# leoelm/Bayesian_inference_for_NN

Measured on AMD Instinct MI355X. Metric: posterior samples/sec (grad-steps/sec) on MLP 784->200->10, batch 1024, higher is better.
Workload: dtype f32; 1 GPU; SGLD, MLP 784->200->10 (D=159010), synthetic MNIST-shaped 48000x784 fp32 resident in HBM, batch 1024 (last batch of an epoch 896), 1 chain per GPU, device-resident run replayed from hipGraphs; seed=2024, parallelism=independent chains x1 (replicas only, no data-path collective)

## Files before the change

bayesian_inference_for_nn_amd/_lib.py:

```python

from __future__ import annotations

import ctypes as C
import os

from . import _build

ACT = {"linear": 0, "relu": 1, "tanh": 2, "sigmoid": 3, "softmax": 4}
LOSS = {"scce": 0, "mse": 1, "bce": 2}
SWEEP = {"gauss_seidel": 0, "jacobi": 1}
GAMMA_MEDIAN = -1.0
MAX_LANES = 64

STREAM_SGLD, STREAM_BBB, STREAM_HMC, STREAM_INIT, STREAM_PREDICT, STREAM_VADAM, STREAM_BSAM, STREAM_CORRUPT = 0, 1, 2, 3, 4, 5, 6, 7
STREAM_PILCO = 8
STREAM_FSVI = 9
FSVI_MAX_N, FSVI_MAX_D = 1024, 2048
REWARD = {"Cart": 0, "Acb 2 factors": 1}
PILCO_KIND = {"dense": 0, "rbf": 1}


class PyzError(RuntimeError):
    def __init__(self, code, msg):
        super().__init__(f"pyz error {code}: {msg}")
        self.code = code


_p = C.c_void_p
_i32, _i64, _u32, _u64, _f = C.c_int32, C.c_int64, C.c_uint32, C.c_uint64, C.c_float

SIGNATURES = {
    "pyz_version": (C.c_int, []),
    "pyz_last_error": (C.c_char_p, []),
    "pyz_device_count": (C.c_int, []),
    "pyz_mlp_create": (C.c_int, [C.c_int, C.POINTER(_i32), C.POINTER(_i32), C.c_int, C.c_int, C.c_int, C.POINTER(_p)]),
    "pyz_mlp_destroy": (C.c_int, [_p]),
    "pyz_mlp_param_count": (_i64, [_p]),
    "pyz_mlp_workspace_bytes": (_i64, [_p]),
    "pyz_mlp_forward": (C.c_int, [_p, _p, C.c_int, _p, _p, C.c_int, _p, _p]),
    "pyz_mlp_loss_grad": (C.c_int, [_p, _p, C.c_int, _p, _p, _p, C.c_int, _p, _p, _p]),
    "pyz_sgd_step": (C.c_int, [_p, _p, _p, _p, _p, C.c_int, _f, _p, _p]),
    "pyz_swag_step": (C.c_int, [_p, _p, _p, _p, _p, _p, _p, _p, C.c_int, _f, _i64, C.c_int, _p, _p]),
    "pyz_adam_step": (C.c_int, [_p, _p, _p, _p, _p, _p, _p, C.c_int, _f, C.c_double, C.c_double, _i64, _f, _f, _p, _p]),
    "pyz_vadam_perturb": (C.c_int, [_p, _p, _p, _f, _f, _i64, _u64, _p, _p]),
    "pyz_bsam_step": (C.c_int, [_p, _p, _p, _p, _p, _p, _p, C.c_int, _f, C.c_double, C.c_double, _f, _f, _f, _f, _i64, _u64,
                              _p, _p, _p]),
    "pyz_sgld_step": (C.c_int, [_p, _p, _p, _p, _p, _p, _p, C.c_int, _f, _i64, _u64, _p, _p, _p]),
    "pyz_sgld_run": (C.c_int, [_p, _p, _p, _p, _p, _p, _p, C.POINTER(_i32), C.POINTER(_f), C.c_int, _i64, _i64, _u64,
                               _p, C.c_int, _p]),
    "pyz_sgld_chains_step": (C.c_int, [_p, _p, _p, _p, C.c_int, _p, _p, _p, C.c_int, _f, _i64, _u64, _p, _p, _p]),
    "pyz_sgld_chains_run": (C.c_int, [_p, _p, _p, _p, C.c_int, _p, _p, _p, C.POINTER(_i32), C.POINTER(_f), C.c_int, _i64,
                                      _i64, _u64, _p, C.c_int, _p]),
    "pyz_sgld_lanes_step": (C.c_int, [_p, _p, _p, _p, C.c_int, _p, _p, _p, C.c_int, C.POINTER(_f), _i64, _u64, C.c_int, _p, _p,
                                      _p]),
    "pyz_sgld_lanes_run": (C.c_int, [_p, _p, _p, _p, C.c_int, _p, _p, _p, C.POINTER(_i32), C.POINTER(_f), C.c_int, _i64,
                                     _i64, _u64, C.c_int, _p, _p]),
    "pyz_lane_scores": (C.c_int, [_p, _p, C.c_int, _p, _p, C.c_int, _p, _p, _p]),
    "pyz_sgd_run": (C.c_int, [_p, _p, _p, _p, _p, C.POINTER(_i32), C.POINTER(_f), C.c_int, _i64, _p, C.c_int, _p]),
    "pyz_swag_run": (C.c_int, [_p, _p, _p, _p, _p, C.c_int, C.c_int, _p, _p, _p, C.POINTER(_i32), C.POINTER(_f), C.c_int,
                               _i64, _i64, _p, C.c_int, _p]),
    "pyz_sgd_members_step": (C.c_int, [_p, _p, _p, C.c_int, _p, _p, _p, C.c_int, _f, _i64, C.c_int, _p, _p]),
    "pyz_sgd_members_run": (C.c_int, [_p, _p, _p, C.c_int, C.c_int, _p, _p, _p, C.POINTER(_i32), C.POINTER(_f), C.c_int, _i64,
                                      _i64, _p, C.c_int, _p]),
    "pyz_swag_members_step": (C.c_int, [_p, _p, _p, _p, _p, C.c_int, C.c_int, _p, _p, _p, C.c_int, _f, _i64, C.c_int, C.c_int,
                                        _p, _p]),
    "pyz_swag_members_run": (C.c_int, [_p, _p, _p, _p, _p, C.c_int, C.c_int, C.c_int, _p, _p, _p, C.POINTER(_i32),
                                       C.POINTER(_f), C.c_int, _i64, _i64, _p, C.c_int, _p]),
    "pyz_last_run_info": (C.c_int, [_p, C.POINTER(_i32), C.POINTER(_i32), C.POINTER(_i32)]),
    "pyz_sgld_run_info": (C.c_int, [_p, C.POINTER(_i32)]),
    "pyz_check_finite": (C.c_int, [_p, _p]),
    "pyz_probe_begin": (C.c_int, [C.c_int]),
    "pyz_probe_end": (C.c_int, [_p, C.POINTER(_f), C.c_char_p, C.c_int, C.POINTER(C.c_int)]),
    "pyz_bbb_step": (C.c_int, [_p, _p, _p, _p, _p, _p, _p, C.c_int, _f, _f, _f, _f, _p, _p, _i64, _u64, _p, _p, _p]),
    "pyz_bbb_run": (C.c_int, [_p, _p, _p, _p, _p, _p, _p, C.POINTER(_i32), C.POINTER(_f), C.c_int, _f, _f, _f, _p, _p, _i64,
                              _i64, _u64, _p, _p, _p, _p, C.c_int, _p, C.c_int, _p]),
    "pyz_adam_run": (C.c_int, [_p, _p, _p, _p, _p, _p, _p, C.POINTER(_i32), C.POINTER(_f), C.POINTER(_i64), C.c_int, C.c_double,
                               C.c_double, _f, _f, C.c_int, _f, _f, _i64, _i64, _u64, _p, C.c_int, _p]),
    "pyz_bsam_run": (C.c_int, [_p, _p, _p, _p, _p, _p, _p, C.POINTER(_i32), C.POINTER(_f), C.c_int, C.c_double, C.c_double,
                               _f, _f, _f, _f, _i64, _i64, _u64, _p, C.c_int, _p]),
    "pyz_adam_run_info": (C.c_int, [_p, C.POINTER(_i32)]),
    "pyz_hmc_step": (C.c_int, [_p, _p, C.c_int, _p, _p, C.c_int, C.c_int, _f, _f, _f, _f, _p, _p, C.c_int, C.POINTER(_f),
                               _i64, _u64, _p, _p, _p]),
    "pyz_hmc_run": (C.c_int, [_p, _p, C.c_int, _p, _p, C.c_int, C.c_int, _f, _f, _f, _f, _p, _p, C.POINTER(_f), C.c_int, C.c_int,
                              _i64, _i64, _u64, _p, _p, _p, _p, C.c_int, _p, C.c_int, _p]),
    "pyz_hmc_run_info": (C.c_int, [_p, C.POINTER(_i32)]),
    "pyz_svgd_step": (C.c_int, [_p, _p, C.c_int, _p, C.c_int, C.c_int, _p, _p, _p, _p, _p, C.c_int, _f, _f, _i64,
                                C.c_int, _p, _p]),
    "pyz_svgd_gradients": (C.c_int, [_p, _p, C.c_int, _p, _p, _p, C.c_int, _p]),
    "pyz_svgd_sweep": (C.c_int, [_p, _p, C.c_int, _p, C.c_int, C.c_int, _p, _p, _f, _f, _i64, C.c_int, _p, _p]),
    "pyz_svgd_kernel_matrix": (C.c_int, [_p, _p, C.c_int, C.c_int, C.c_int, _f, _p]),
    "pyz_svgd_gram_groups": (C.c_int, [_p, _p, C.c_int, C.c_int, C.c_int, _p, _p]),
    "pyz_svgd_kernel_matrix_groups": (C.c_int, [_p, _p, _p, C.c_int, C.c_int, C.c_int, _f, _p]),
    "pyz_svgd_combine": (C.c_int, [_p, _p, C.c_int, _p, C.c_int, C.c_int, _p, _p, _f, _f, _i64, _p, _p]),
    "pyz_fsvi_check": (C.c_int, [C.c_int, C.POINTER(_i32), C.POINTER(_i32), C.c_int, C.c_int, C.c_int, C.c_int]),
    "pyz_fsvi_step": (C.c_int, [_p, _p, _p, C.c_int, _p, _p, _p, _p, _p, C.c_int, C.c_int, _p, _p, _f, _i64, _u64, _p, _p, _p,
                                _p, _p, _p, _p, _p, _p, _p]),
    "pyz_spd_solve_f64": (C.c_int, [_p, _p, C.c_int, C.c_int, _p, _p]),
    "pyz_predict": (C.c_int, [_p, _p, C.c_int, _p, C.c_int, _p, _p, _p]),
    "pyz_predict_moments": (C.c_int, [_p, _p, C.c_int, _p, C.c_int, _p, _p, _p]),
    "pyz_grid_rows": (C.c_int, [_p, C.c_int, _f, _f, C.c_int, _f, _f, C.c_int, _i64, _i64, _p, _p]),
    "pyz_predict_surface": (C.c_int, [_p, _p, C.c_int, _p, C.c_int, C.c_int, _p, _p, _p, _p, _p, _p]),
    "pyz_input_grad": (C.c_int, [_p, _p, C.c_int, _p, _p, C.c_int, _f, _p, _f, _p, _p, _p]),
    "pyz_corrupt_rows": (C.c_int, [_p, _i64, C.c_int, C.c_int, C.c_int, C.c_int, C.POINTER(_i32), C.c_int, _f, C.c_int, _u64, _p, _p]),
    "pyz_score_rows": (C.c_int, [_p, C.c_int, _i64, C.c_int, _p, C.c_int, _p, _p]),
    "pyz_pilco_create": (C.c_int, [C.c_int, C.POINTER(_i32), C.POINTER(_i32), C.c_int, C.POINTER(_i32), C.POINTER(_i32), C.c_int,
                                   C.c_int, C.POINTER(_p)]),
    "pyz_pilco_create_layers": (C.c_int, [C.c_int, C.POINTER(_i32), C.POINTER(_i32), C.POINTER(_i32), C.POINTER(_f), C.c_int,
                                          C.POINTER(_i32), C.POINTER(_i32), C.c_int, C.c_int, C.POINTER(_p)]),
    "pyz_pilco_destroy": (C.c_int, [_p]),
    "pyz_pilco_workspace_bytes": (_i64, [_p]),
    "pyz_pilco_policy_step": (C.c_int, [_p, _p, _p, _p, _i64, _p, _p, _p, C.c_int, C.c_int, _f, C.c_int, _f, _p, _p, _p, _p,
                                        C.c_int, _p]),
    "pyz_pilco_act": (C.c_int, [_p, _p, _p, C.c_int, _p, _p]),
    "pyz_sample_normal_rows": (C.c_int, [_p, _i64, _i64, _i64, _i64, _p, _p, _u64, _u32, _u32, _p]),
    "pyz_sample_lowrank_rows": (C.c_int, [_p, _i64, _i64, _i64, _i64, _p, _p, _p, C.c_int, _f, _u64, _u32, _u32, _p]),
    "pyz_gather_rows": (C.c_int, [_p, _i64, _i64, _i64, _i64, _p, _i64, _p, _p]),
    "pyz_fill_normal": (C.c_int, [_p, _i64, _u64, _u32, _u32, _f, _f, _p]),
    "pyz_debug_stamps": (C.c_int, [C.POINTER(C.c_uint64), _i64]),
    "pyz_debug_mfma_f64_layout": (C.c_int, [C.POINTER(C.c_int32)]),
    "pyz_bench_dense_kernel": (C.c_int, [_p, C.c_int, C.c_int, _p, C.c_int, _p, _p, C.c_int, _p, C.c_int, _p]),
    "pyz_malloc": (C.c_int, [C.c_size_t, C.POINTER(_p)]),
    "pyz_free": (C.c_int, [_p]),
    "pyz_upload": (C.c_int, [_p, _p, C.c_size_t, _p]),
    "pyz_download": (C.c_int, [_p, _p, C.c_size_t, _p]),
    "pyz_sync": (C.c_int, [_p]),
    "pyz_wait_flags": (C.c_int, [_p, C.c_int, C.c_uint64, C.c_int, _p, _p]),
    "pyz_stem_create": (C.c_int, [C.c_int, C.c_int, C.c_int, C.c_int, C.POINTER(_i32), C.c_int, C.c_int, C.POINTER(_p)]),
    "pyz_stem_destroy": (C.c_int, [_p]),
    "pyz_stem_param_count": (_i64, [_p]),
    "pyz_stem_feature_count": (_i64, [_p]),
    "pyz_stem_workspace_bytes": (_i64, [_p]),
    "pyz_stem_forward": (C.c_int, [_p, _p, _i64, C.c_int, _p, _p, C.c_int, _p, _p]),
    "pyz_stem_backward": (C.c_int, [_p, _p, _i64, C.c_int, _p, _p, C.c_int, _p, _p, _i64, _p]),
    "pyz_convnet_forward": (C.c_int, [_p, _p, _p, C.c_int, _p, _p, C.c_int, _p, _p]),
    "pyz_convnet_loss_grad": (C.c_int, [_p, _p, _p, C.c_int, _p, _p, _p, C.c_int, _p, _p, _p]),
    "pyz_convnet_sgd_step": (C.c_int, [_p, _p, _p, _p, _p, _p, C.c_int, _f, _p, _p]),
    "pyz_convnet_swag_step": (C.c_int, [_p, _p, _p, _p, _p, _p, _p, _p, _p, C.c_int, _f, _i64, C.c_int, _p, _p]),
    "pyz_convnet_predict": (C.c_int, [_p, _p, _p, C.c_int, _p, C.c_int, _p, _p, _p, _p]),
}

E_NAN = -6
LOWRANK_MAX_K = 256


def header_version() -> int:
    import re
    text = open(os.path.join(os.path.dirname(os.path.abspath(__file__)), "..", "include", "pyz.h")).read()
    return int(re.search(r"#define\s+PYZ_VERSION\s+(\d+)", text).group(1))

_lib = None


# ... 42 lines not shown
```

bayesian_inference_for_nn_amd/csrc/pyz_api.hip:

```cpp

#include <algorithm>
#include <climits>
#include <cmath>
#include <cstring>
#include <vector>

#include "pyz_common.h"
#include "pyz_conv.h"
#include "pyz_corrupt.h"
#include "pyz_fsvi.h"
#include "pyz_fused.h"
#include "pyz_gemm.h"
#include "pyz_gemm_ring.h"
#include "pyz_hmc_fused.h"
#include "pyz_hmc_multi.h"
#include "pyz_input_grad.h"
#include "pyz_pilco.h"
#include "pyz_kernels.h"
#include "pyz_predict_moments.h"
#include "pyz_surface.h"
#include "pyz_rng.h"
#include "pyz_sgld_chains.h"
#include "pyz_sgld_lanes.h"
#include "pyz_members.h"
// ... 107 lines not shown
int need_grad2(pyz_mlp *m, int P) {
  return ensure_bytes((void **)&m->grad2, &full(m)->x.grad2_cap, sizeof(float) * (size_t)P * m->D + 64, m);
}
int need_qsave(pyz_mlp *m, int P) {
  return ensure_bytes((void **)&m->qsave, &full(m)->x.qsave_cap, sizeof(float) * (size_t)P * m->D + 64, m);
}
int need_part(pyz_mlp *m, size_t n_doubles) {
  return ensure_bytes((void **)&m->part, &full(m)->x.part_cap, sizeof(double) * n_doubles, m);
}
int need_part2(pyz_mlp *m, size_t n_doubles, bool keep_kernel_matrix = false) {
  if (!keep_kernel_matrix) m->km_valid = false;
  return ensure_bytes((void **)&full(m)->x.part2, &full(m)->x.part2_cap, sizeof(double) * n_doubles, m);
}

int check_call(const pyz_mlp *m, int P, int batch) {
  if (!m) return pyz_fail(PYZ_E_INVALID, "null plan");
  if (batch <= 0 || batch > m->max_batch)
    return pyz_fail(PYZ_E_SHAPE, "batch %d outside [1, %d] of the plan", batch, m->max_batch);
  if (P <= 0 || P > m->max_p)
    return pyz_fail(PYZ_E_SHAPE, "particle count %d outside [1, %d] of the plan", P, m->max_p);
  return PYZ_OK;
}

inline bool aligned16(const void *p) { return (reinterpret_cast<uintptr_t>(p) & 15u) == 0; }

int set_ctl(pyz_mlp *m, int slot, int batch, float lr, long long n, long long row_off, int i, hipStream_t st,
            int slot0 = 0, int n_run = 0) {
  m->pend_on = false;
  PYZ_LAUNCH(k_set_ctl, dim3(1), dim3(1), 0, st, m->ctl + slot, batch, lr, n, row_off, i, slot0, n_run);
  PYZ_LAUNCH_CHECK();
  return PYZ_OK;
}

void set_ctl_lazy(pyz_mlp *m, int batch, float lr, long long n) {
  m->pend = StepCtl{};
  m->pend.batch = batch;
  m->pend.lr = lr;
  m->pend.n = n;
  m->pend_on = true;
}

void flush_ctl(pyz_mlp *m, hipStream_t st) {
  if (!m->pend_on) return;
  m->pend_on = false;
  PYZ_LAUNCH(k_set_ctl, dim3(1), dim3(1), 0, st, m->ctl, m->pend.batch, m->pend.lr, m->pend.n, m->pend.row_off, m->pend.i,
                     m->pend.slot0, 0);
}

DenseArgs forward_args(pyz_mlp *m, int l, const float *theta, long long theta_ps, const float *x, const int32_t *row_idx,
                       const StepCtl *ctl, float *gather_out) {
  DenseArgs g{};
  g.K = m->dims[l];
  g.N = m->dims[l + 1];
  if (l == 0) {
    g.in = x;
    g.in_pstride = 0;
    g.row_idx = row_idx;
    g.gather_out = row_idx ? gather_out : nullptr;
  } else {
    g.in = m->act[l - 1];
    g.in_pstride = (long long)m->max_batch * g.K;
    g.row_idx = nullptr;
  }
  g.lda = g.K;
  g.theta = theta;
  g.theta_pstride = theta_ps;
  g.w_off = m->w_off[l];
  g.out = m->act[l];
  g.out_pstride = (long long)m->max_batch * g.N;
  g.act = m->acts[l];
  g.vec = (g.K % 8 == 0) && aligned16(g.in) ? 1 : 0;
  g.ctl = ctl;
  if (l == 0 && m->pend_on && ctl == m->ctl) {
    g.init = m->pend;
    g.init_on = 1;
    m->pend_on = false;
  }
  return g;
}

void launch_forward(pyz_mlp *m, const float *theta, long long theta_ps, int P, const float *x,
                    const int32_t *row_idx, int grid_batch, const StepCtl *ctl, hipStream_t st,
                    float *gather_out = nullptr, int l_end = -1, const StepCtl *gate = nullptr, int gate_mod = 0,
                    long long x_pstride = 0) {
  if (l_end < 0) l_end = m->L;
  for (int l = 0; l < l_end; ++l) {
    DenseArgs g = forward_args(m, l, theta, theta_ps, x, row_idx, ctl, gather_out);
    if (l == 0) g.in_pstride = x_pstride;
    g.wt = pyz_wt_for(P);
    g.gate = gate;
    g.gate_mod = gate_mod;
    if (pyz_launch_fwd_ring(g, grid_batch, P, st)) continue;
    if (!g.row_idx && !g.init_on && !g.gather_out) g.rows_cap = std::min(grid_batch, m->max_batch);
    pyz_launch_fwd(g, grid_batch, P, st);
  }
}

void launch_loss(pyz_mlp *m, int P, const void *y, const int32_t *row_idx, int grid_batch, const StepCtl *ctl,
                 bool want_delta, hipStream_t st) {
  LossArgs g{};
  const int C = m->dims[m->L];
  g.out_last = m->act[m->L - 1];
  g.pstride = (long long)m->max_batch * C;
  g.C = C;
  g.y = y;
  g.delta = want_delta ? m->delta[m->L - 1] : nullptr;
  g.part = m->part;
  g.nblk = cdiv(m->max_batch, 256);
  g.act_last = m->acts[m->L - 1];
  g.ctl = ctl;
  g.row_idx = row_idx;
  dim3 grid(cdiv(grid_batch, 256), P);
  if ((int)grid.x < g.nblk) g.nblk = grid.x;
  if (m->loss == PYZ_LOSS_SCCE)
    PYZ_LAUNCH(k_loss_scce, grid, dim3(256), 0, st, g);
  else
    PYZ_LAUNCH(k_loss_mse, grid, dim3(256), 0, st, g);
}

inline int loss_nblk(const pyz_mlp *m, int grid_batch) { return std::min(cdiv(m->max_batch, 256), cdiv(grid_batch, 256)); }

struct TailOf {
  long long x_pstride;
  long long grad_pstride;
  float *dfeat;
  int act_feat;
};

void launch_backward(pyz_mlp *m, const float *theta, long long theta_ps, int P, const float *x,
                     const int32_t *row_idx, int grid_batch, const StepCtl *ctl, float *grad, hipStream_t st,
                     float *grad_sq = nullptr, const TailOf *tail = nullptr) {
  for (int l = m->L - 1; l >= 0; --l) {
    const int K = m->dims[l], N = m->dims[l + 1];
    if (l > 0 || tail) {
      DenseArgs g{};
      g.K = K;
      g.N = N;
      g.in = m->delta[l];
      g.in_pstride = (long long)m->max_batch * N;
      g.lda = N;
      g.theta = theta;
      g.theta_pstride = theta_ps;
      g.w_off = m->w_off[l];
      g.out = l > 0 ? m->delta[l - 1] : tail->dfeat;
      g.out_pstride = l > 0 ? (long long)m->max_batch * K : tail->x_pstride;
      g.aux = l > 0 ? m->act[l - 1] : x;
      g.aux_pstride = g.out_pstride;
      g.act = l > 0 ? m->acts[l - 1] : tail->act_feat;
      g.vec = (N % 8 == 0) && (m->w_off[l] % 4 == 0) && (P == 1 || theta_ps % 4 == 0) && aligned16(theta) ? 1 : 0;
      g.ctl = ctl;
      pyz_launch_bwd_data(g, grid_batch, P, st);
    }
    DenseArgs g{};
    g.K = K;
    g.N = N;
    if (l == 0) {
      g.in = x;
      g.in_pstride = tail ? tail->x_pstride : 0;
      g.row_idx = row_idx;
    } else {
      g.in = m->act[l - 1];
      g.in_pstride = (long long)m->max_batch * K;
    }
    g.lda = K;
    g.aux = m->delta[l];
    g.aux_pstride = (long long)m->max_batch * N;
    g.out = grad;
    g.out_pstride = tail ? tail->grad_pstride : m->D;
    g.w_off = m->w_off[l];
// ... 93 lines not shown
                            const StepCtl *ctl, hipStream_t st) {
  for (int l = m->L - 2; l >= 1; --l) {
    const int K = m->dims[l], N = m->dims[l + 1];
    DenseArgs g{};
    g.K = K;
    g.N = N;
    g.in = m->delta[l];
    g.in_pstride = (long long)m->max_batch * N;
    g.lda = N;
    g.theta = theta;
    g.theta_pstride = theta_ps;
    g.w_off = m->w_off[l];
    g.out = m->delta[l - 1];
    g.out_pstride = (long long)m->max_batch * K;
    g.aux = m->act[l - 1];
    g.aux_pstride = (long long)m->max_batch * K;
    g.act = m->acts[l - 1];
    g.vec = (N % 8 == 0) && (m->w_off[l] % 4 == 0) && (P == 1 || theta_ps % 4 == 0) && aligned16(theta) ? 1 : 0;
    g.ctl = ctl;
    pyz_launch_bwd_data(g, grid_batch, P, st);
  }
}

inline int wgrad_tiles(const pyz_mlp *m) {
  int tiles = 0;
  for (int l = 0; l < m->L; ++l) tiles += ((m->dims[l] + 1 + 31) / 32) * ((m->dims[l + 1] + 31) / 32);
  return tiles;
}

int wgrad_layers(pyz_mlp *m, int P, const float *x, const int32_t *row_idx, const StepCtl *ctl, WgradArgs &a,
                 const float *gathered) {
  int tiles = 0;
  a.L = m->L;
  for (int l = 0; l < m->L; ++l) {
    WgradLayer &ly = a.lay[l];
    ly.K = m->dims[l];
    ly.N = m->dims[l + 1];
    if (l == 0) {
      ly.in = (row_idx && gathered) ? gathered : x;
      ly.in_pstride = 0;
      ly.gather = (row_idx && !gathered) ? 1 : 0;
    } else {
      ly.in = m->act[l - 1];
      ly.in_pstride = (long long)m->max_batch * ly.K;
      ly.gather = 0;
    }
    ly.lda = ly.K;
    ly.delta = m->delta[l];
    ly.delta_pstride = (long long)m->max_batch * ly.N;
    ly.w_off = m->w_off[l];
    ly.tile0 = tiles;
    a.tile0[l] = tiles;
    tiles += ((ly.K + 1 + 31) / 32) * ((ly.N + 31) / 32);
  }
  for (int l = m->L; l < PYZ_MAX_LAYERS; ++l) a.tile0[l] = INT_MAX;
  a.row_idx = row_idx;
  a.ctl = ctl;
  a.part = m->part;
  a.nblk = m->cur_nblk;
  a.tiles = tiles;
  a.nonfinite = m->nonfinite;
  a.wt = pyz_wt_for(P);
  return tiles;
}

void launch_wgrad_all(pyz_mlp *m, int P, const float *x, const int32_t *row_idx, int grid_batch, const StepCtl *ctl,
                      WgradArgs &a, hipStream_t st, const float *gathered) {
  const int tiles = wgrad_layers(m, P, x, row_idx, ctl, a, gathered);
  const int S = pyz_pick_waves((long long)tiles * P, (grid_batch + 1) / 2);
  dim3 grid(pyz_pad8((long long)tiles + 1, P), P);
  if (a.prep.src && P == 1) grid.x = (unsigned)(tiles + 1 + std::max(pyz_cu_count() - tiles - 1, 24));
  switch (S) {
    case 1:
      if (a.mode == PYZ_UPD_NONE) PYZ_LAUNCH((k_wgrad_all<1, true>), grid, dim3(64), 0, st, a);
      else PYZ_LAUNCH(k_wgrad_all<1>, grid, dim3(64), 0, st, a);
      break;
    case 2: PYZ_LAUNCH(k_wgrad_all<2>, grid, dim3(128), 2 * 4096, st, a); break;
    case 4: PYZ_LAUNCH(k_wgrad_all<4>, grid, dim3(256), 4 * 4096, st, a); break;
    case 8: PYZ_LAUNCH(k_wgrad_all<8>, grid, dim3(512), 8 * 4096, st, a); break;
    default: PYZ_LAUNCH(k_wgrad_all<16>, grid, dim3(1024), 16 * 4096, st, a); break;
  }
}

void launch_wgrad_adam(pyz_mlp *m, const float *x, const int32_t *row_idx, int grid_batch, const StepCtl *ctl, AdamArgs &a,
                       hipStream_t st, const float *gathered) {
  const int tiles = wgrad_layers(m, 1, x, row_idx, ctl, a.w, gathered);
  const int S = pyz_pick_waves(tiles, (grid_batch + 1) / 2);
  const dim3 grid(tiles + 1);
  switch (S) {
    case 1: PYZ_LAUNCH(k_wgrad_adam<1>, grid, dim3(64), 0, st, a); break;
    case 2: PYZ_LAUNCH(k_wgrad_adam<2>, grid, dim3(128), 2 * 4096, st, a); break;
    case 4: PYZ_LAUNCH(k_wgrad_adam<4>, grid, dim3(256), 4 * 4096, st, a); break;
    case 8: PYZ_LAUNCH(k_wgrad_adam<8>, grid, dim3(512), 8 * 4096, st, a); break;
    default: PYZ_LAUNCH(k_wgrad_adam<16>, grid, dim3(1024), 16 * 4096, st, a); break;
  }
}

void launch_wgrad_bsam(pyz_mlp *m, const float *x, const int32_t *row_idx, int grid_batch, const StepCtl *ctl, int phase,
                       BsamArgs &a, hipStream_t st, const float *gathered) {
  const int tiles = wgrad_layers(m, 1, x, row_idx, ctl, a.w, gathered);
  const int S = pyz_pick_waves(tiles, (grid_batch + 1) / 2);
  const dim3 grid(tiles + 1);
#define PYZ_BSAM_CASE(W, LDS)                                                           \
  if (phase == 0) PYZ_LAUNCH((k_wgrad_bsam<W, 0>), grid, dim3(64 * W), LDS, st, a);     \
  else PYZ_LAUNCH((k_wgrad_bsam<W, 1>), grid, dim3(64 * W), LDS, st, a);                \
  break
  switch (S) {
    case 1: PYZ_BSAM_CASE(1, 0);
    case 2: PYZ_BSAM_CASE(2, 2 * 4096);
    case 4: PYZ_BSAM_CASE(4, 4 * 4096);
    case 8: PYZ_BSAM_CASE(8, 8 * 4096);
    default: PYZ_BSAM_CASE(16, 16 * 4096);
  }
#undef PYZ_BSAM_CASE
}

inline float *batch_buf(pyz_mlp *m, int slot) { return m->xb + (size_t)slot * m->max_batch * m->dims[0]; }

inline bool batch_ahead(const pyz_mlp *m, const int32_t *row_idx) {
  static const int on = pyz_env_int("PYZ_BATCH_AHEAD", 1);
  if (!on || !can_fuse(m) || m->L <= 1 || row_idx == nullptr) return false;
  return on == 2 || wgrad_tiles(m) + 24 <= pyz_cu_count();
}

PrepArgs prep_args(pyz_mlp *m, const float *x, const int32_t *row_idx, int grid_batch, long long row_stride, int dst_slot) {
  PrepArgs p{};
  p.src = x;
  p.dst = batch_buf(m, dst_slot);
  p.row_idx = row_idx;
  p.tab_bs = m->tab_bs;
  p.row_stride = row_stride;
  p.K = p.lda = m->dims[0];
  p.fwd_tiles_n = (m->dims[1] + 31) / 32;
  p.fwd_tiles = ((grid_batch + 31) / 32) * p.fwd_tiles_n;
  return p;
}

int ksplit_for(pyz_mlp *m, const float *theta, long long theta_ps, int P, const float *xc, int grid_batch, const StepCtl *ctl) {
  const int ks_env = pyz_env_int("PYZ_FWD_KSPLIT", 0);
  if (ks_env < 2 || ks_env > 8 || m->L != 2 || P != 1) return 0;
  const int UT = m->dims[1] <= 64 ? 1 : m->dims[1] <= 256 ? 4 : 0, NPc = m->dims[2];
  if (!UT || NPc > 16 || !pyz_env_int("PYZ_HEAD_ROWS", 1)) return 0;
  DenseArgs g = forward_args(m, 0, theta, theta_ps, xc, nullptr, ctl, nullptr);
  if (!pyz_fwd_ring_ksplit_ok(g, grid_batch, P)) return 0;
  if ((long long)((grid_batch + 31) / 32) * ks_env > 2 * pyz_cu_count()) return 0;
  const size_t need = sizeof(float) * (size_t)ks_env * m->max_batch * m->dims[1];
  if (!full(m)->x.fwd_part || full(m)->x.fwd_part_cap < need) return 0;
  return ks_env;
}

void launch_loss_backward(pyz_mlp *m, const float *theta, long long theta_ps, int P, const float *x, const void *y,
                          const int32_t *row_idx, int grid_batch, const StepCtl *ctl, bool want_grad, WgradArgs &upd,
                          hipStream_t st, int ahead_slot = -1, AdamArgs *adam = nullptr) {
  if (can_fuse(m)) {
    if (ahead_slot >= 0) {
      const float *xc = batch_buf(m, ahead_slot);
      const int ks = ksplit_for(m, theta, theta_ps, P, xc, grid_batch, ctl);
      if (ks > 1) {
        DenseArgs g = forward_args(m, 0, theta, theta_ps, xc, nullptr, ctl, nullptr);
        g.wt = pyz_wt_for(P);
        g.k_split = ks;
        g.part_out = static_cast<float *>(full(m)->x.fwd_part);
        g.part_stride = (long long)m->max_batch * g.N;
        pyz_launch_fwd_ring_ksplit(g, grid_batch, st);
      } else {
        launch_forward(m, theta, theta_ps, P, xc, nullptr, grid_batch, ctl, st, nullptr, m->L - 1);
      }
      launch_head(m, theta, theta_ps, P, x, y, row_idx, grid_batch, ctl, want_grad, st, nullptr, 0, ks);
      launch_bwd_data_hidden(m, theta, theta_ps, P, grid_batch, ctl, st);
      launch_wgrad_all(m, P, x, row_idx, grid_batch, ctl, upd, st, xc);
      return;
    }
    static const int use_xb = pyz_env_int("PYZ_GATHER_COPY", 1);
    float *xb = (use_xb && want_grad && row_idx && m->L > 1) ? m->xb : nullptr;
    launch_forward(m, theta, theta_ps, P, x, row_idx, grid_batch, ctl, st, xb, m->L - 1);
    launch_head(m, theta, theta_ps, P, x, y, row_idx, grid_batch, ctl, want_grad, st);
    if (want_grad) {
      launch_bwd_data_hidden(m, theta, theta_ps, P, grid_batch, ctl, st);
      if (adam) launch_wgrad_adam(m, x, row_idx, grid_batch, ctl, *adam, st, xb);
      else launch_wgrad_all(m, P, x, row_idx, grid_batch, ctl, upd, st, xb);
    }
    return;
  }
  flush_ctl(m, st);
  launch_forward(m, theta, theta_ps, P, x, row_idx, grid_batch, ctl, st);
  launch_loss(m, P, y, row_idx, grid_batch, ctl, want_grad, st);
  m->cur_nblk = loss_nblk(m, grid_batch);
  if (want_grad) launch_backward(m, theta, theta_ps, P, x, row_idx, grid_batch, ctl, upd.grad, st, adam ? m->grad2 : nullptr);
}

void launch_bsam_pass(pyz_mlp *m, const float *theta, const float *x, const void *y, const int32_t *row_idx, int grid_batch,
                      int phase, BsamArgs &a, hipStream_t st) {
  static const int use_xb = pyz_env_int("PYZ_GATHER_COPY", 1);
  float *xb = (use_xb && row_idx && m->L > 1) ? m->xb : nullptr;
  launch_forward(m, theta, m->D, 1, x, row_idx, grid_batch, m->ctl, st, xb, m->L - 1);
  launch_head(m, theta, m->D, 1, x, y, row_idx, grid_batch, m->ctl, true, st);
  launch_bwd_data_hidden(m, theta, m->D, 1, grid_batch, m->ctl, st);
  launch_wgrad_bsam(m, x, row_idx, grid_batch, m->ctl, phase, a, st, xb);
}

int check_loss_combo(const pyz_mlp *m) {
  const int last = m->acts[m->L - 1];
  if (m->loss == PYZ_LOSS_SCCE && last != PYZ_ACT_SOFTMAX)
    return pyz_fail(PYZ_E_INVALID, "SparseCategoricalCrossentropy needs a softmax last layer");
  if (m->loss == PYZ_LOSS_MSE && last == PYZ_ACT_SOFTMAX)
    return pyz_fail(PYZ_E_INVALID, "MeanSquaredError on a softmax last layer is not supported");
  if (m->loss == PYZ_LOSS_BCE && (m->dims[m->L] != 1 || last != PYZ_ACT_SIGMOID))
    return pyz_fail(PYZ_E_INVALID, "BinaryCrossentropy needs a last layer of exactly one sigmoid unit");
  return PYZ_OK;
}

AdamScal adam_scalars(float lr, double beta_1, double beta_2, long long epoch, float denom_eps, float decay) {
  AdamScal a;
  a.lr = lr;
  a.b1 = (float)beta_1;
  a.c1 = (float)(1.0 - beta_1);
  a.b2 = (float)beta_2;
  a.c2 = (float)(1.0 - beta_2);
  a.bc1 = (float)(1.0 - std::pow(beta_1, (double)epoch));
  a.bc2 = (float)(1.0 - std::pow(beta_2, (double)epoch));
  a.eps = denom_eps;
  a.decay = decay;
  return a;
}

void launch_delta0(pyz_mlp *m, const float *theta, int P, const float *x, const void *y, int n, hipStream_t st) {
  if (can_fuse(m)) {
    launch_forward(m, theta, m->D, P, x, nullptr, n, m->ctl, st, nullptr, m->L - 1);
    launch_head(m, theta, m->D, P, x, y, nullptr, n, m->ctl, true, st);
    launch_bwd_data_hidden(m, theta, m->D, P, n, m->ctl, st);
    return;
  }
  launch_forward(m, theta, m->D, P, x, nullptr, n, m->ctl, st);
  launch_loss(m, P, y, nullptr, n, m->ctl, true, st);
  m->cur_nblk = loss_nblk(m, n);
  if (m->L > 1) {
    const int l = m->L - 1, K = m->dims[l], N = m->dims[l + 1];
// ... 251 lines not shown
  return for_draw_chunks(net, d_weights, n_samples, d_x, n, m->max_p, st, [&](int s0, int S, const float *) {
    g.S = S;
    g.accumulate = s0 > 0 ? 1 : 0;
    if (!pyz_launch_predict_moments(g, st))
      return pyz_fail(PYZ_E_SHAPE, "a row of %d outputs does not fit the moments kernel's LDS", g.C);
    return PYZ_OK;
  });
}

}

extern "C" {

int pyz_version(void) { return PYZ_VERSION; }

const char *pyz_last_error(void) { return pyz_err_slot().c_str(); }

int pyz_device_count(void) {
  int n = 0;
  if (hipGetDeviceCount(&n) != hipSuccess) return 0;
  return n;
}

int pyz_mlp_create(int n_layers, const int32_t *h_dims, const int32_t *h_acts, int loss, int max_batch,
                   int max_particles, pyz_mlp **out) {
  if (!out || !h_dims || !h_acts) return pyz_fail(PYZ_E_INVALID, "null argument");
  *out = nullptr;
  if (n_layers < 1 || n_layers > PYZ_MAX_LAYERS) return pyz_fail(PYZ_E_INVALID, "n_layers %d outside [1, %d]", n_layers, PYZ_MAX_LAYERS);
  if (max_batch < 1 || max_particles < 1) return pyz_fail(PYZ_E_INVALID, "max_batch and max_particles must be >= 1");
  if (max_particles > 65535) return pyz_fail(PYZ_E_INVALID, "max_particles %d > 65535", max_particles);
  if (loss != PYZ_LOSS_SCCE && loss != PYZ_LOSS_MSE && loss != PYZ_LOSS_BCE) return pyz_fail(PYZ_E_INVALID, "unknown loss %d", loss);
  int ndev = 0;
  if (hipGetDeviceCount(&ndev) != hipSuccess || ndev < 1) return pyz_fail(PYZ_E_NODEV, "no HIP device visible");
  pyz_mlp_full *m = new pyz_mlp_full();
  m->L = n_layers;
  m->loss = loss;
  m->max_batch = max_batch;
  m->max_p = max_particles;
  long long off = 0;
  for (int l = 0; l <= n_layers; ++l) {
    if (h_dims[l] < 1) {
      delete m;
      return pyz_fail(PYZ_E_INVALID, "dims[%d] = %d", l, h_dims[l]);
    }
    m->dims[l] = h_dims[l];
  }
  for (int l = 0; l < n_layers; ++l) {
    const int a = h_acts[l];
    if (a < PYZ_ACT_LINEAR || a > PYZ_ACT_SOFTMAX || (a == PYZ_ACT_SOFTMAX && l != n_layers - 1)) {
      delete m;
      return pyz_fail(PYZ_E_INVALID, "activation %d at layer %d is not supported", a, l);
    }
    m->acts[l] = a;
    m->w_off[l] = off;
    off += (long long)(m->dims[l] + 1) * m->dims[l + 1];
  }
  m->D = off;
  if (loss == PYZ_LOSS_BCE) {
    const int rc = check_loss_combo(m);
    if (rc != PYZ_OK) {
      delete m;
      return rc;
    }
  }
  {
    long long widest = 0;
    for (int l = 0; l <= n_layers; ++l) widest = std::max<long long>(widest, m->dims[l]);
    if ((long long)max_batch * widest * 4 >= (1LL << 31) || off * 4 >= (1LL << 31)) {
      delete m;
      return pyz_fail(PYZ_E_INVALID, "max_batch x widest layer, or the parameter vector, exceeds 2 GiB");
    }
  }
  auto fail = [&](int rc) {
    pyz_mlp_destroy(m);
    return rc;
  };
  for (int l = 0; l < n_layers; ++l) {
    const size_t bytes = sizeof(float) * (size_t)max_particles * max_batch * m->dims[l + 1] + 64;
    if (hipMalloc((void **)&m->act[l], bytes) != hipSuccess || hipMalloc((void **)&m->delta[l], bytes) != hipSuccess)
      return fail(pyz_fail(PYZ_E_OOM, "workspace allocation of %zu bytes failed", bytes));
    m->ws_bytes += 2 * bytes;
  }
  {
    const size_t bytes = 2 * sizeof(float) * (size_t)max_batch * m->dims[0] + 64;
    if (hipMalloc((void **)&m->xb, bytes) != hipSuccess) return fail(pyz_fail(PYZ_E_OOM, "workspace allocation of %zu bytes failed", bytes));
    m->ws_bytes += bytes;
  }
  if (hipMalloc((void **)&m->nonfinite, 64) != hipSuccess || hipMemset(m->nonfinite, 0, 64) != hipSuccess)
    return fail(pyz_fail(PYZ_E_OOM, "counter allocation failed"));
  if (hipMalloc((void **)&m->ctl, 2 * sizeof(StepCtl)) != hipSuccess) return fail(pyz_fail(PYZ_E_OOM, "ctl allocation failed"));
  if (hipMemset(m->ctl, 0, 2 * sizeof(StepCtl)) != hipSuccess) return fail(pyz_fail(PYZ_E_HIP, "ctl memset failed"));
  const size_t scal = sizeof(float) * (size_t)(max_particles * 16 + 64);
  if (hipMalloc((void **)&m->scal, scal) != hipSuccess) return fail(pyz_fail(PYZ_E_OOM, "scalar allocation failed"));
  m->ws_bytes += scal;
  {
    const int rc = need_part(m, (size_t)max_particles * max_batch + 8);
    if (rc != PYZ_OK) return fail(rc);
  }
  if (m->L == 2 && m->dims[1] > 192 && m->dims[1] <= 200 && pyz_env_int("PYZ_FWD_KSPLIT", 0) >= 2) {
    const int rc = ensure_bytes(&m->x.fwd_part, &m->x.fwd_part_cap, sizeof(float) * (size_t)8 * max_batch * m->dims[1], m);
    if (rc != PYZ_OK) return fail(rc);
  }
  {
    const int gs_lds = (int)pyz_svgd_gs_lds_bytes();
    if (hipFuncSetAttribute(reinterpret_cast<const void *>(k_svgd_gs<false>), hipFuncAttributeMaxDynamicSharedMemorySize, gs_lds) != hipSuccess ||
        hipFuncSetAttribute(reinterpret_cast<const void *>(k_svgd_gs<true>), hipFuncAttributeMaxDynamicSharedMemorySize, gs_lds) != hipSuccess)
      return fail(pyz_fail(PYZ_E_HIP, "hipFuncSetAttribute(k_svgd_gs) failed"));
    if (hipFuncSetAttribute(reinterpret_cast<const void *>(k_svgd_gs_resident), hipFuncAttributeMaxDynamicSharedMemorySize,
                            (int)pyz_svgd_gs_res_lds_bytes()) != hipSuccess)
      return fail(pyz_fail(PYZ_E_HIP, "hipFuncSetAttribute(k_svgd_gs_resident) failed"));
    if (hipFuncSetAttribute(reinterpret_cast<const void *>(k_svgd_gs_resident2), hipFuncAttributeMaxDynamicSharedMemorySize,
                            (int)pyz_svgd_gs_res_lds_bytes()) != hipSuccess)
      return fail(pyz_fail(PYZ_E_HIP, "hipFuncSetAttribute(k_svgd_gs_resident2) failed"));
    const int gr_lds = (int)pyz_svgd_gram_lds_bytes();
    if (hipFuncSetAttribute(reinterpret_cast<const void *>(k_svgd_gram_tile<1, false>), hipFuncAttributeMaxDynamicSharedMemorySize, gr_lds) != hipSuccess ||
        hipFuncSetAttribute(reinterpret_cast<const void *>(k_svgd_gram_tile<2, false>), hipFuncAttributeMaxDynamicSharedMemorySize, gr_lds) != hipSuccess ||
        hipFuncSetAttribute(reinterpret_cast<const void *>(k_svgd_gram_tile<4, true>), hipFuncAttributeMaxDynamicSharedMemorySize, gr_lds) != hipSuccess)
      return fail(pyz_fail(PYZ_E_HIP, "hipFuncSetAttribute(k_svgd_gram_tile) failed"));
  }
  *out = m;
  return PYZ_OK;
}

int pyz_mlp_destroy(pyz_mlp *mm) {
  if (!mm) return PYZ_OK;
  pyz_mlp_full *m = full(mm);
  m->graphs.drop();
  m->x.hm_graphs.drop();
  m->x.hmc_run_graphs.drop();
  m->x.adam_graphs.drop();
  for (int l = 0; l < PYZ_MAX_LAYERS; ++l) {
    if (m->act[l]) (void)hipFree(m->act[l]);
    if (m->delta[l]) (void)hipFree(m->delta[l]);
  }
  void *ptrs[] = {m->grad, m->grad2, m->qsave, m->part, m->x.part2, m->scal, m->ctl, m->tab_bs, m->xb, m->x.hm_buf, m->x.hm_res_buf, m->x.gs_res_buf, m->x.fwd_part, m->nonfinite, m->x.hr_buf, m->x.hr_tab, m->x.tab_bc, m->x.fsvi_buf};
  for (void *p : ptrs)
    if (p) (void)hipFree(p);
  if (m->x.tab_host) {
    (void)hipHostFree(m->x.tab_host);
    for (auto &e : m->x.tab_ev) (void)hipEventDestroy(e);
  }
  if (m->x.up_host) {
    (void)hipHostFree(m->x.up_host);
    for (auto &e : m->x.up_ev) (void)hipEventDestroy(e);
  }
  if (m->x.hr_host) {
    (void)hipHostFree(m->x.hr_host);
    for (auto &e : m->x.hr_ev) (void)hipEventDestroy(e);
  }
  if (m->h_pinned) (void)hipHostFree(m->h_pinned);
  delete m;
  return PYZ_OK;
}

int64_t pyz_mlp_param_count(const pyz_mlp *m) { return m ? m->D : -1; }
int64_t pyz_mlp_workspace_bytes(const pyz_mlp *m) { return m ? (int64_t)m->ws_bytes : -1; }

int pyz_mlp_forward(pyz_mlp *m, const float *d_theta, int P, const float *d_x, const int32_t *d_row_idx, int batch,
                    float *d_out, void *stream) {
  int rc = check_call(m, P, batch);
  if (rc) return rc;
  return net_forward(Net{nullptr, m}, d_theta, P, d_x, d_row_idx, batch, d_out, stream);
}

int pyz_mlp_loss_grad(pyz_mlp *m, const float *d_theta, int P, const float *d_x, const void *d_y,
                      const int32_t *d_row_idx, int batch, float *d_grad, float *d_loss, void *stream) {
  int rc = check_call(m, P, batch);
// ... 333 lines not shown
  } else {
    u.mode = PYZ_UPD_NONE;
    u.grad = m->grad;
    u.grad_pstride = m->D;
  }
  launch_loss_backward(m, d_theta, m->D, 1, d_x, d_y, d_row_idx, batch, m->ctl, true, u, st);
  if (!fused)
    PYZ_LAUNCH(k_swag_update, dim3(cdiv(m->D, 256)), dim3(256), 0, st, d_theta, d_mean, d_sq_mean, d_dev_row,
                       m->grad, m->D, update_moments ? 1 : 0, m->ctl, m->part, m->cur_nblk, d_loss, m->nonfinite);
  PYZ_LAUNCH_CHECK();
  return PYZ_OK;
}

struct SwagChain {
  float *dev;
  int k, freq;
};

struct BbbChain {
  float *rho, *w;
  float *w2;
  float alpha, prior_mean, prior_rho;
  const float *pm_vec, *pr_vec;
  pyz_mlp *val;
  const float *val_x;
  const void *val_y;
  int n_val;
  float *val_losses;
};

static int ensure_run_tables(pyz_mlp *m, size_t n_tab, size_t host_entry_bytes, hipStream_t st) {
  pyz_mlp_full *f = full(m);
  if (m->tab_cap < (int)n_tab) {
    const size_t cap = std::max<size_t>(n_tab, 65536);
    if (m->tab_bs) PYZ_HIP(hipFree(m->tab_bs));
    m->tab_bs = nullptr;
    m->tab_lr = nullptr;
    PYZ_HIP(hipMalloc((void **)&m->tab_bs, 8 * cap));
    m->tab_lr = reinterpret_cast<float *>(m->tab_bs + cap);
    m->tab_cap = (int)cap;
    m->graphs.drop();
  }
  if (f->x.tab_host_cap < host_entry_bytes * n_tab) {
    if (f->x.tab_host) {
      PYZ_HIP(hipStreamSynchronize(st));
      PYZ_HIP(hipHostFree(f->x.tab_host));
      f->x.tab_host = nullptr;
    } else {
      for (auto &e : f->x.tab_ev) PYZ_HIP(hipEventCreateWithFlags(&e, hipEventDisableTiming));
    }
    const size_t cap = std::max<size_t>(host_entry_bytes * n_tab, host_entry_bytes * 4096);
    PYZ_HIP(hipHostMalloc(&f->x.tab_host, 2 * cap));
    f->x.tab_host_cap = cap;
    f->x.tab_count = 0;
  }
  return PYZ_OK;
}

static int check_run(const pyz_mlp *m, int n_steps, int64_t slot0, const int32_t *h_batch_sizes, const int64_t *h_epochs = nullptr) {
  if (n_steps <= 0) return pyz_fail(PYZ_E_INVALID, "n_steps must be positive");
  if (slot0 < 0 || slot0 + n_steps > 0x7fffffff) return pyz_fail(PYZ_E_INVALID, "slot0 out of range");
  int bmax = 0;
  for (int s = 0; h_batch_sizes && s < n_steps; ++s) {
    if (h_batch_sizes[s] <= 0 || h_batch_sizes[s] > m->max_batch)
      return pyz_fail(PYZ_E_SHAPE, "batch size %d of step %d outside [1, %d]", h_batch_sizes[s], s, m->max_batch);
    if (h_epochs && h_epochs[s] < 1) return pyz_fail(PYZ_E_INVALID, "epoch %lld of step %d < 1", (long long)h_epochs[s], s);
    bmax = std::max(bmax, h_batch_sizes[s]);
  }
  return bmax;
}

struct RunBc {
  double beta_1, beta_2;
  const int64_t *h_epochs;
  float2 of(int s) const {
    const AdamScal a = adam_scalars(0.0f, beta_1, beta_2, h_epochs[s], 0.0f, 0.0f);
    return make_float2(a.bc1, a.bc2);
  }
};

static int upload_run_tables(pyz_mlp *m, const int32_t *h_batch_sizes, const float *h_lr, int n_steps, int64_t n0, int64_t slot0,
                             const RunBc *bc, const float *d_x, const int32_t *d_row_idx, int ahead_batch, hipStream_t st) {
  Extra &x = full(m)->x;
  int rc;
  const size_t n_tab = (size_t)n_steps + 1;
  if ((rc = ensure_run_tables(m, n_tab, bc ? 16 : 8, st))) return rc;
  if (bc && x.tab_bc_cap < m->tab_cap) {
    if (x.tab_bc) PYZ_HIP(hipFree(x.tab_bc));
    x.tab_bc = nullptr;
    x.tab_bc_cap = 0;
    PYZ_HIP(hipMalloc((void **)&x.tab_bc, sizeof(float2) * (size_t)m->tab_cap));
    x.tab_bc_cap = m->tab_cap;
  }
  const long long row_stride = m->max_batch;
  m->pend_on = false;
  if (n_steps <= PYZ_INLINE_TAB) {
    InlineTabs tabs{};
    InlineBc ibc{};
    for (int s = 0; s < n_steps; ++s) {
      tabs.bs[s] = h_batch_sizes[s];
      tabs.lr[s] = h_lr[s];
    }
    tabs.bs[n_steps] = h_batch_sizes[n_steps - 1];
    tabs.lr[n_steps] = h_lr[n_steps - 1];
    tabs.n = n_steps + 1;
    for (int s = 0; bc && s <= n_steps; ++s) ibc.bc[s] = bc->of(std::min(s, n_steps - 1));
    if (ahead_batch) {
      const PrepArgs pa = prep_args(m, d_x, d_row_idx, ahead_batch, row_stride, 0);
      if (bc) PYZ_LAUNCH(k_run_start_bc, dim3(256), dim3(256), 0, st, m->ctl, tabs, ibc, m->tab_bs, m->tab_lr, x.tab_bc, (long long)n0, slot0 * row_stride, (int)slot0, pa);
      else PYZ_LAUNCH(k_run_start, dim3(256), dim3(256), 0, st, m->ctl, tabs, m->tab_bs, m->tab_lr, (long long)n0, slot0 * row_stride, (int)slot0, pa);
    } else {
      if (bc) PYZ_LAUNCH(k_set_ctl_tabs_bc, dim3(1), dim3(64), 0, st, m->ctl, tabs, ibc, m->tab_bs, m->tab_lr, x.tab_bc, (long long)n0, slot0 * row_stride, (int)slot0);
      else PYZ_LAUNCH(k_set_ctl_tabs, dim3(1), dim3(64), 0, st, m->ctl, tabs, m->tab_bs, m->tab_lr, (long long)n0, slot0 * row_stride, (int)slot0);
    }
    return PYZ_OK;
  }
  const unsigned slot = (unsigned)(x.tab_count & 1);
  if (x.tab_count >= 2) PYZ_HIP(hipEventSynchronize(x.tab_ev[slot]));
  ++x.tab_count;
  int32_t *hb = reinterpret_cast<int32_t *>(static_cast<unsigned char *>(x.tab_host) + slot * x.tab_host_cap);
  float *hl = reinterpret_cast<float *>(hb + n_tab);
  float2 *hc = reinterpret_cast<float2 *>(hl + n_tab);
  std::memcpy(hb, h_batch_sizes, sizeof(int32_t) * n_steps);
  std::memcpy(hl, h_lr, sizeof(float) * n_steps);
  hb[n_steps] = h_batch_sizes[n_steps - 1];
  hl[n_steps] = h_lr[n_steps - 1];
  for (int s = 0; bc && s <= n_steps; ++s) hc[s] = bc->of(std::min(s, n_steps - 1));
  PYZ_HIP(hipMemcpyAsync(m->tab_bs, hb, sizeof(int32_t) * n_tab, hipMemcpyHostToDevice, st));
  PYZ_HIP(hipMemcpyAsync(m->tab_lr, hl, sizeof(float) * n_tab, hipMemcpyHostToDevice, st));
  if (bc) PYZ_HIP(hipMemcpyAsync(x.tab_bc, hc, sizeof(float2) * n_tab, hipMemcpyHostToDevice, st));
  PYZ_HIP(hipEventRecord(x.tab_ev[slot], st));
  if ((rc = set_ctl(m, 0, h_batch_sizes[0], h_lr[0], n0, slot0 * row_stride, 0, st, (int)slot0, n_steps))) return rc;
  if (ahead_batch)
    PYZ_LAUNCH(k_prep_batch, dim3(256), dim3(256), 0, st, prep_args(m, d_x, d_row_idx, ahead_batch, row_stride, 0), m->ctl);
  return PYZ_OK;
}

static void launch_sgld_step(pyz_mlp *m, float *theta, float *mean, float *sq, const float *x, const void *y,
                             const int32_t *row_idx, int grid_batch, int slot, bool chained, long long row_stride,
                             uint64_t seed, const float *unit_noise, float *loss, hipStream_t st, int mode = PYZ_UPD_SGLD,
                             const SwagChain *swag = nullptr, const BbbChain *bbb = nullptr, bool first = true) {
  const StepCtl *ctl = m->ctl + slot;
  if (bbb) {
    const int nblk_sample = cdiv(cdiv(m->D, 4), 256), tiles = wgrad_tiles(m);
    const bool fuse = bbb->w2 != nullptr;
    const size_t kl_stride = (size_t)std::max(nblk_sample, tiles);
    double *kl_cur = full(m)->x.part2 + (fuse ? (size_t)slot * kl_stride : 0);
    double *kl_next = full(m)->x.part2 + (size_t)(slot ^ 1) * kl_stride;
    float *w_cur = (fuse && slot) ? bbb->w2 : bbb->w, *w_next = slot ? bbb->w : bbb->w2;
    const bool sample = !fuse || first;
    if (sample) {
      BbbArgs a{};
      a.mu = theta;
      a.rho = bbb->rho;
      a.w = w_cur;
      a.D = m->D;
      a.alpha = bbb->alpha;
      a.prior_mean = bbb->prior_mean;
      a.prior_rho = bbb->prior_rho;
      a.pm_vec = bbb->pm_vec;
      a.pr_vec = bbb->pr_vec;
      a.seed = seed;
      a.part_kl = kl_cur;
      a.nblk_kl = nblk_sample;
      a.ctl = ctl;
      a.chained = 1;
      PYZ_LAUNCH(k_bbb_sample, dim3(nblk_sample), dim3(256), 0, st, a);
    }
    WgradArgs u{};
    u.mode = PYZ_UPD_BBB;
    u.theta = theta;
    u.mean = bbb->rho;
    u.sq_mean = w_cur;
    u.seed = seed;
    u.alpha = bbb->alpha;
    u.prior_mean = bbb->prior_mean;
    u.prior_rho = bbb->prior_rho;
    u.pm_vec = bbb->pm_vec;
    u.pr_vec = bbb->pr_vec;
    u.bbb_chained = 1;
    u.part_kl = kl_cur;
    u.nblk_kl = sample ? nblk_sample : tiles;
    if (fuse) {
      u.w_next = w_next;
      u.part_kl_next = kl_next;
    }
    u.cost = loss;
    u.next = chained ? m->ctl + (slot ^ 1) : nullptr;
    u.tab_bs = m->tab_bs;
    u.tab_lr = m->tab_lr;
    u.row_stride = row_stride;
    const bool ahead = chained && batch_ahead(m, row_idx);
    if (ahead) u.prep = prep_args(m, x, row_idx, grid_batch, row_stride, slot ^ 1);
    launch_loss_backward(m, w_cur, m->D, 1, x, y, row_idx, grid_batch, ctl, true, u, st, ahead ? slot : -1);
    if (bbb->val) {
      pyz_mlp *v = bbb->val;
      launch_forward(v, w_cur, v->D, 1, bbb->val_x, nullptr, bbb->n_val, v->ctl, st, nullptr, v->L - 1, ctl, 10);
      launch_head(v, w_cur, v->D, 1, bbb->val_x, bbb->val_y, nullptr, bbb->n_val, v->ctl, false, st, ctl, 10);
      PYZ_LAUNCH(k_loss_finalize_gated, dim3(1), dim3(64), 0, st, v->part, v->cur_nblk, v->ctl, bbb->val_losses, v->nonfinite, ctl, 10);
    }
    return;
  }
  if (can_fuse(m)) {
    WgradArgs u{};
    u.mode = mode;
    if (swag) {
      u.swag_freq = swag->freq;
      u.swag_k = swag->k;
      u.dev_base = swag->dev;
      u.dev_stride = m->D;
    }
    u.theta = theta;
    u.mean = mean;
    u.sq_mean = sq;
    u.seed = seed;
    u.unit_noise = unit_noise;
    u.loss = loss;
    u.loss_indexed = chained ? 1 : 0;
    u.next = chained ? m->ctl + (slot ^ 1) : nullptr;
    u.tab_bs = m->tab_bs;
    u.tab_lr = m->tab_lr;
    u.row_stride = row_stride;
    const bool ahead = chained && batch_ahead(m, row_idx);
    if (ahead) u.prep = prep_args(m, x, row_idx, grid_batch, row_stride, slot ^ 1);
    launch_loss_backward(m, theta, m->D, 1, x, y, row_idx, grid_batch, ctl, true, u, st, ahead ? slot : -1);
    return;
  }
  WgradArgs u{};
  u.mode = PYZ_UPD_NONE;
  u.grad = m->grad;
  u.grad_pstride = m->D;
  launch_loss_backward(m, theta, m->D, 1, x, y, row_idx, grid_batch, ctl, true, u, st);
  SgldArgs a{};
  a.theta = theta;
  a.mean = mean;
  a.sq_mean = sq;
  a.grad = m->grad;
  a.D = m->D;
  a.ctl = ctl;
  a.next = chained ? m->ctl + (slot ^ 1) : nullptr;
  a.tab_bs = m->tab_bs;
  a.tab_lr = m->tab_lr;
  a.row_stride = row_stride;
  a.seed = seed;
  a.unit_noise = unit_noise;
  a.part = m->part;
  a.nblk = m->cur_nblk;
  a.loss = loss;
  a.loss_indexed = chained ? 1 : 0;
  a.nonfinite = m->nonfinite;
  PYZ_LAUNCH(k_sgld_update, dim3(cdiv(cdiv(m->D, 4), 256)), dim3(256), 0, st, a);
}

int pyz_sgld_step(pyz_mlp *m, float *d_theta, float *d_mean, float *d_sq_mean, const float *d_x, const void *d_y,
                  const int32_t *d_row_idx, int batch, float lr, int64_t n, uint64_t seed, const float *d_unit_noise,
                  float *d_loss, void *stream) {
  int rc = check_call(m, 1, batch);
  if (rc) return rc;
  if ((rc = check_loss_combo(m))) return rc;
  if (!d_theta || !d_mean || !d_sq_mean || !d_x || !d_y || !d_loss) return pyz_fail(PYZ_E_INVALID, "null device pointer");
  if (n < 0) return pyz_fail(PYZ_E_INVALID, "negative step count");
  if (!can_fuse(m) && (rc = need_grad(m, 1))) return rc;
  hipStream_t st = as_stream(stream);
  set_ctl_lazy(m, batch, lr, n);
  launch_sgld_step(m, d_theta, d_mean, d_sq_mean, d_x, d_y, d_row_idx, batch, 0, false, 0, seed, d_unit_noise, d_loss, st);
  PYZ_LAUNCH_CHECK();
  return PYZ_OK;
}

static int sgld_run_impl(pyz_mlp *m, float *d_theta, float *d_mean, float *d_sq_mean, const float *d_x, const void *d_y,
                         const int32_t *d_row_idx, const int32_t *h_batch_sizes, const float *h_lr, int n_steps,
                         int64_t n0, int64_t slot0, uint64_t seed, float *d_losses, int use_graph, void *stream,
                         int mode = PYZ_UPD_SGLD, const SwagChain *swag = nullptr, const BbbChain *bbb = nullptr) {
  if (!m) return pyz_fail(PYZ_E_INVALID, "null plan");
  if (mode != PYZ_UPD_SGLD && !can_fuse(m))
    return pyz_fail(PYZ_E_INVALID, "the chained SGD / SWAG runs need a last layer of at most 32 units");
  if (mode == PYZ_UPD_SGD) d_mean = d_sq_mean = d_theta;
  int rc = check_loss_combo(m);
  if (rc) return rc;
  if ((rc = check_run(m, n_steps, slot0, nullptr)) < 0) return rc;
  if (!d_theta || !d_mean || !d_sq_mean || !d_x || !d_y || !d_row_idx || !h_batch_sizes || !h_lr || !d_losses)
    return pyz_fail(PYZ_E_INVALID, "null pointer");
  const int bmax = check_run(m, n_steps, slot0, h_batch_sizes);
  if (bmax < 0) return bmax;
  if (!can_fuse(m) && (rc = need_grad(m, 1))) return rc;
  hipStream_t st = as_stream(stream);
  BbbChain bbb_local{};
  if (bbb) {
    static const int fuse_sample = pyz_env_int("PYZ_BBB_FUSE_SAMPLE", 1);
    if ((rc = need_part2(m, 2 * (size_t)std::max(cdiv(cdiv(m->D, 4), 256), wgrad_tiles(m))))) return rc;
    if (fuse_sample) {
      if ((rc = need_grad(m, 1))) return rc;
      bbb_local = *bbb;
      bbb_local.w2 = m->grad;
      bbb = &bbb_local;
    }
    if (bbb->val) {
      pyz_mlp *v = bbb->val;
      if (v->D != m->D || !can_fuse(v) || bbb->n_val < 1 || bbb->n_val > v->max_batch || !bbb->val_x || !bbb->val_y || !bbb->val_losses)
        return pyz_fail(PYZ_E_INVALID, "validation plan / split does not fit the model");
      if ((rc = set_ctl(v, 0, bbb->n_val, 0.0f, 0, 0, 0, st))) return rc;
    }
  }
  const long long row_stride = m->max_batch;
  if ((rc = upload_run_tables(m, h_batch_sizes, h_lr, n_steps, n0, slot0, nullptr, d_x, d_row_idx,
                              batch_ahead(m, d_row_idx) ? bmax : 0, st)))
    return rc;

  int s = 0;
  m->run_graph_steps = m->run_eager_steps = m->run_graph_launches = 0;
  m->graphs.begin_call();
  static const int G = std::min(128, std::max(2, pyz_env_int("PYZ_GRAPH_STEPS", 32) & ~1));
  if (use_graph && st != nullptr && !pyz_probe().on) {
    unsigned long long key = 1469598103934665603ull;
    auto mix = [&](unsigned long long v) { key = (key ^ v) * 1099511628211ull; };
    mix((unsigned long long)(uintptr_t)d_theta); mix((unsigned long long)(uintptr_t)d_mean);
    mix((unsigned long long)(uintptr_t)d_sq_mean); mix((unsigned long long)(uintptr_t)d_x);
    mix((unsigned long long)(uintptr_t)d_y); mix((unsigned long long)(uintptr_t)d_row_idx);
    mix((unsigned long long)(uintptr_t)d_losses); mix(seed); mix((unsigned long long)bmax);
    mix((unsigned long long)(uintptr_t)m->tab_bs); mix((unsigned long long)G); mix((unsigned long long)mode);
    if (swag) { mix((unsigned long long)(uintptr_t)swag->dev); mix((unsigned long long)swag->k); mix((unsigned long long)swag->freq); }
    if (bbb) {
      unsigned fb[3];
      memcpy(&fb[0], &bbb->alpha, 4); memcpy(&fb[1], &bbb->prior_mean, 4); memcpy(&fb[2], &bbb->prior_rho, 4);
      for (unsigned b : fb) mix(b);
      mix((unsigned long long)(uintptr_t)bbb->pm_vec); mix((unsigned long long)(uintptr_t)bbb->pr_vec);
      mix((unsigned long long)(uintptr_t)bbb->val); mix((unsigned long long)(uintptr_t)bbb->val_x); mix((unsigned long long)(uintptr_t)bbb->val_y);
      mix((unsigned long long)bbb->n_val); mix((unsigned long long)(uintptr_t)bbb->val_losses);
      mix((unsigned long long)(uintptr_t)bbb->w2); mix((unsigned long long)(uintptr_t)bbb->rho); mix((unsigned long long)(uintptr_t)full(m)->x.part2);
    }
    m->graphs.rekey(key);
    while (s < n_steps) {
      const int len = std::min(G, n_steps - s);
      const bool rest = len < G;
      rc = m->graphs.launch(len, 0, rest ? 1 : 0, rest ? PYZ_GRAPH_CHUNKS : 1, st, [&] {
        for (int k = 0; k < len; ++k)
          launch_sgld_step(m, d_theta, d_mean, d_sq_mean, d_x, d_y, d_row_idx, bmax, k & 1, true, row_stride, seed,
                           nullptr, d_losses, st, mode, swag, bbb, k == 0);
        return PYZ_OK;
      });
      if (rc) return rc;
      s += len;
      m->run_graph_steps += len;
      ++m->run_graph_launches;
    }
  }
  for (; s < n_steps; ++s) {
    launch_sgld_step(m, d_theta, d_mean, d_sq_mean, d_x, d_y, d_row_idx, bmax, s & 1, true, row_stride, seed, nullptr,
                     d_losses, st, mode, swag, bbb, s == 0);
    ++m->run_eager_steps;
  }
  if (bbb && bbb->w2 && ((n_steps - 1) & 1))
    PYZ_HIP(hipMemcpyAsync(bbb->w, bbb->w2, sizeof(float) * (size_t)m->D, hipMemcpyDeviceToDevice, st));
  PYZ_LAUNCH_CHECK();
  return PYZ_OK;
}

int pyz_sgld_run(pyz_mlp *m, float *d_theta, float *d_mean, float *d_sq_mean, const float *d_x, const void *d_y,
                 const int32_t *d_row_idx, const int32_t *h_batch_sizes, const float *h_lr, int n_steps, int64_t n0,
                 int64_t slot0, uint64_t seed, float *d_losses, int use_graph, void *stream) {
  return sgld_run_impl(m, d_theta, d_mean, d_sq_mean, d_x, d_y, d_row_idx, h_batch_sizes, h_lr, n_steps, n0, slot0, seed,
                       d_losses, use_graph, stream);
}

static int sgld_rows_check(const pyz_mlp *m, bool lanes, const void *theta, const void *mean, const void *sq, int P,
                           const void *x, const void *y, const void *h_lr, const void *losses, int64_t n, int seed_stride,
                           const char *row = nullptr) {
  if (!row) row = lanes ? "lane" : "chain";
  if (P < 1) return pyz_fail(PYZ_E_INVALID, "n_%ss %d: at least one %s", row, P, row);
  if (n < 0) return pyz_fail(PYZ_E_INVALID, "negative step count");
  if (lanes && seed_stride != 0 && seed_stride != 1)
    return pyz_fail(PYZ_E_INVALID, "seed_stride %d: 0 (one noise stream for every lane) or 1 (seed + lane)", seed_stride);
  if (!theta || !mean || !sq || !x || !y || (lanes && !h_lr) || !losses)
    return pyz_fail(PYZ_E_INVALID, lanes ? "null pointer" : "null device pointer");
  if (!m) return pyz_fail(PYZ_E_INVALID, "null plan");
  const int most = lanes ? std::min(m->max_p, PYZ_MAX_LANES) : m->max_p;
  if (P > most)
    return pyz_fail(PYZ_E_SHAPE, "n_%ss %d outside [1, %d] of the plan%s", row, P, most, lanes ? " and the library" : "");
  return check_loss_combo(m);
}

static dim3 sgld_rows_grid(long long groups, int P) {
  const long long per_row = std::max<long long>(1, 8LL * pyz_cu_count() / P);
  return dim3((unsigned)std::min<long long>(cdiv(groups, 256), per_row), (unsigned)P);
}

struct MembersUpdate {
  bool swag;
  float *dev;
  int k;
  int freq;
  int hit, col;
};

static void launch_sgld_rows_step(pyz_mlp *m, float *theta, float *mean, float *sq, int P, const float *x, const void *y,
                                  const int32_t *row_idx, int grid_batch, int slot, bool chained, long long row_stride,
                                  uint64_t seed, const float *lane_lr, int seed_stride, const float *unit_noise, float *loss,
                                  hipStream_t st, const MembersUpdate *members = nullptr) {
  const StepCtl *ctl = m->ctl + slot;
  WgradArgs u{};
  u.mode = PYZ_UPD_NONE;
  u.grad = m->grad;
  u.grad_pstride = m->D;
// ... 1789 lines not shown
    g.out = m->delta[layer - 1];
    g.out_pstride = (long long)m->max_batch * K;
    g.aux = m->act[layer - 1];
    g.aux_pstride = (long long)m->max_batch * K;
    g.act = m->acts[layer - 1];
    g.vec = (N % 8 == 0) && (m->w_off[layer] % 4 == 0) && (P == 1 || m->D % 4 == 0) && aligned16(d_theta) ? 1 : 0;
  } else if (kind == 0) {
    if (layer == 0) {
      g.in = d_x;
      g.in_pstride = 0;
      g.row_idx = d_row_idx;
    } else {
      g.in = m->act[layer - 1];
      g.in_pstride = (long long)m->max_batch * K;
    }
    g.lda = K;
    g.out = m->act[layer];
    g.out_pstride = (long long)m->max_batch * N;
    g.act = m->acts[layer];
    g.vec = (K % 8 == 0) && aligned16(g.in) ? 1 : 0;
  }
  WgradArgs u{};
  u.mode = PYZ_UPD_NONE;
  u.grad = d_grad;
  u.grad_pstride = m->D;
  for (int i = 0; i < iters; ++i) {
    if (kind == 0) {
      if (!pyz_launch_fwd_ring(g, batch, P, st)) pyz_launch_fwd(g, batch, P, st);
    }
    else if (kind == 1) pyz_launch_bwd_data(g, batch, P, st);
    else launch_wgrad_all(m, P, d_x, d_row_idx, batch, m->ctl, u, st, nullptr);
  }
  PYZ_LAUNCH_CHECK();
  return PYZ_OK;
}

int pyz_probe_begin(int max_launches) {
  if (max_launches < 1 || max_launches > (1 << 20)) return pyz_fail(PYZ_E_INVALID, "max_launches outside [1, 2^20]");
  PyzProbe &p = pyz_probe();
  if (p.on) return pyz_fail(PYZ_E_INVALID, "a probe is already open on this thread");
  while ((int)p.ev.size() < 2 * max_launches) {
    hipEvent_t e = nullptr;
    PYZ_HIP(hipEventCreate(&e));
    p.ev.push_back(e);
  }
  p.name.assign((size_t)max_launches, nullptr);
  p.cap = max_launches;
  p.n = 0;
  p.on = true;
  return PYZ_OK;
}

int pyz_probe_end(void *stream, float *h_us, char *h_names, int name_stride, int *h_n) {
  PyzProbe &p = pyz_probe();
  if (!p.on) return pyz_fail(PYZ_E_INVALID, "no probe open on this thread");
  p.on = false;
  if (!h_us || !h_n) return pyz_fail(PYZ_E_INVALID, "null pointer");
  PYZ_HIP(hipStreamSynchronize(as_stream(stream)));
  for (int i = 0; i < p.n; ++i) {
    float ms = 0.0f;
    PYZ_HIP(hipEventElapsedTime(&ms, p.ev[2 * i], p.ev[2 * i + 1]));
    h_us[i] = ms * 1e3f;
    if (h_names && name_stride > 1) {
      const char *nm = p.name[i] ? p.name[i] : "";
      const bool wrapped = nm[0] == '(';
      char *dst = h_names + (size_t)i * name_stride;
      std::snprintf(dst, (size_t)name_stride, "%s", nm + (wrapped ? 1 : 0));
      const size_t len = std::strlen(dst);
      if (wrapped && len > 0 && dst[len - 1] == ')') dst[len - 1] = '\0';
    }
  }
  *h_n = p.n;
  return PYZ_OK;
}

int pyz_last_run_info(const pyz_mlp *m, int32_t *h_graph_steps, int32_t *h_eager_steps, int32_t *h_graph_launches) {
  if (!m) return pyz_fail(PYZ_E_INVALID, "null plan");
  if (h_graph_steps) *h_graph_steps = m->run_graph_steps;
  if (h_eager_steps) *h_eager_steps = m->run_eager_steps;
  if (h_graph_launches) *h_graph_launches = m->run_graph_launches;
  return PYZ_OK;
}

int pyz_sgld_run_info(const pyz_mlp *m, int32_t *h_captures) {
  if (!m) return pyz_fail(PYZ_E_INVALID, "null plan");
  if (h_captures) *h_captures = m->graphs.captures;
  return PYZ_OK;
}

int pyz_check_finite(pyz_mlp *m, void *stream) {
  if (!m) return pyz_fail(PYZ_E_INVALID, "null plan");
  hipStream_t st = as_stream(stream);
  int n = 0;
  PYZ_HIP(hipMemcpyAsync(&n, m->nonfinite, sizeof n, hipMemcpyDeviceToHost, st));
  PYZ_HIP(hipMemsetAsync(m->nonfinite, 0, sizeof n, st));
  PYZ_HIP(hipStreamSynchronize(st));
  if (n > 0) return pyz_fail(PYZ_E_NAN, "%d step(s) since the last check produced a NaN / Inf loss", n);
  return PYZ_OK;
}

int pyz_malloc(size_t bytes, void **d_out) {
  if (!d_out || bytes == 0) return pyz_fail(PYZ_E_INVALID, "bad allocation request");
  *d_out = nullptr;
  PYZ_HIP(hipMalloc(d_out, bytes));
  return PYZ_OK;
}

int pyz_free(void *d_ptr) {
  if (d_ptr) PYZ_HIP(hipFree(d_ptr));
  return PYZ_OK;
}

int pyz_upload(void *d_dst, const void *h_src, size_t bytes, void *stream) {
  if (!d_dst || !h_src) return pyz_fail(PYZ_E_INVALID, "null pointer");
  PYZ_HIP(hipMemcpyAsync(d_dst, h_src, bytes, hipMemcpyHostToDevice, as_stream(stream)));
  PYZ_HIP(hipStreamSynchronize(as_stream(stream)));
  return PYZ_OK;
}

int pyz_download(void *h_dst, const void *d_src, size_t bytes, void *stream) {
  if (!h_dst || !d_src) return pyz_fail(PYZ_E_INVALID, "null pointer");
  PYZ_HIP(hipMemcpyAsync(h_dst, d_src, bytes, hipMemcpyDeviceToHost, as_stream(stream)));
  PYZ_HIP(hipStreamSynchronize(as_stream(stream)));
  return PYZ_OK;
}

int pyz_wait_flags(const uint64_t *d_flags, int n, uint64_t value, int spin_limit, int *d_fail, void *stream) {
  if (!d_flags) return pyz_fail(PYZ_E_INVALID, "null device pointer");
  if (n < 1 || n > 64) return pyz_fail(PYZ_E_INVALID, "flag count %d outside [1, 64]", n);
  PYZ_LAUNCH(k_wait_flags, dim3(1), dim3(64), 0, as_stream(stream), reinterpret_cast<const unsigned long long *>(d_flags), n,
             (unsigned long long)value, spin_limit, d_fail);
  PYZ_LAUNCH_CHECK();
  return PYZ_OK;
}

int pyz_sync(void *stream) {
  PYZ_HIP(hipStreamSynchronize(as_stream(stream)));
  return PYZ_OK;
}

int pyz_debug_mfma_f64_layout(int32_t *h_out512) {
  if (!h_out512) return pyz_fail(PYZ_E_INVALID, "null pointer");
  int *d = nullptr;
  PYZ_HIP(hipMalloc((void **)&d, 512 * sizeof(int)));
  PYZ_LAUNCH(k_probe_mfma_f64, dim3(1), dim3(64), 0, nullptr, d);
  const hipError_t e = hipMemcpy(h_out512, d, 512 * sizeof(int), hipMemcpyDeviceToHost);
  (void)hipFree(d);
  PYZ_HIP(e);
  return PYZ_OK;
}

int pyz_debug_stamps(uint64_t *h_out, int64_t n_words) {
#ifdef PYZ_STAMPS
  const int64_t total = (int64_t)PYZ_STAMP_KERNELS * PYZ_STAMP_BLOCKS * PYZ_STAMP_WAVES * PYZ_STAMP_SLOTS * 2;
  if (!h_out || n_words < total) return pyz_fail(PYZ_E_INVALID, "need %lld words", (long long)total);
  PYZ_HIP(hipDeviceSynchronize());
  PYZ_HIP(hipMemcpyFromSymbol(h_out, HIP_SYMBOL(pyz_dbg_buf), sizeof(unsigned long long) * total));
  return PYZ_OK;
#else
  (void)h_out;
  (void)n_words;
  return pyz_fail(PYZ_E_INVALID, "not a PYZ_STAMPS build");
#endif
}

int pyz_stem_destroy(pyz_stem *s) {
// ... 217 lines not shown
```

bayesian_inference_for_nn_amd/csrc/pyz_common.h:

```cpp
#pragma once

#include <hip/hip_runtime.h>
#include <hip/hip_ext.h>

#include <cstdarg>
#include <cstdint>
#include <cstdio>
#include <string>
#include <vector>

#include "../../include/pyz.h"

#define PYZ_MAX_LAYERS 16

typedef float f32x16 __attribute__((ext_vector_type(16)));
typedef float f32x4 __attribute__((ext_vector_type(4)));

struct StepCtl {
  int32_t batch;
  float lr;
  long long n;
  long long row_off;
  int32_t i;
  int32_t slot0;
// ... 53 lines not shown
  long long n = raw.n, ro = raw.row_off;
  asm volatile("; step scalars" : "+v"(b), "+v"(lr), "+v"(n), "+v"(ro));
  PyzCtlHot c;
  c.batch = __builtin_amdgcn_readfirstlane(b);
  c.lr = __builtin_bit_cast(float, __builtin_amdgcn_readfirstlane(__builtin_bit_cast(int, lr)));
  const unsigned nl = __builtin_amdgcn_readfirstlane((int)(unsigned)n), nh = __builtin_amdgcn_readfirstlane((int)(n >> 32));
  const unsigned rl = __builtin_amdgcn_readfirstlane((int)(unsigned)ro), rh = __builtin_amdgcn_readfirstlane((int)(ro >> 32));
  c.n = (long long)(((unsigned long long)nh << 32) | nl);
  c.row_off = (long long)(((unsigned long long)rh << 32) | rl);
  return c;
}

__device__ __forceinline__ StepCtl pyz_ctl_first(const StepCtl *ctl, const StepCtl &init, const int on) {
  if (on && blockIdx.x == 0 && blockIdx.y == 0 && threadIdx.x == 0) *const_cast<StepCtl *>(ctl) = init;
  int ib = init.batch, ii = init.i, is0 = init.slot0, inr = init.n_run;
  float il = init.lr;
  long long in_ = init.n, iro = init.row_off;
  asm volatile("" : "+s"(ib), "+s"(ii), "+s"(is0), "+s"(il), "+s"(in_), "+s"(iro), "+s"(inr));
  StepCtl c;
  c.batch = on ? ib : ctl->batch;
  c.lr = on ? il : ctl->lr;
  c.n = on ? in_ : ctl->n;
  c.row_off = on ? iro : ctl->row_off;
  c.i = on ? ii : ctl->i;
  c.slot0 = on ? is0 : ctl->slot0;
  c.n_run = on ? inr : ctl->n_run;
  return c;
}

__device__ __forceinline__ void pyz_st(float *p, const float v, const int wt) {
  if (wt)
    asm volatile("global_store_dword %0, %1, off sc1" ::"v"(p), "v"(v) : "memory");
  else
    *p = v;
}

inline std::string &pyz_err_slot() {
  static thread_local std::string s;
  return s;
}

inline int pyz_fail(int code, const char *fmt, ...) {
  char buf[512];
  va_list ap;
  va_start(ap, fmt);
  vsnprintf(buf, sizeof buf, fmt, ap);
  va_end(ap);
  pyz_err_slot() = buf;
  return code;
}

#define PYZ_HIP(call)                                                                        \
  do {                                                                                       \
    hipError_t e_ = (call);                                                                  \
    if (e_ != hipSuccess)                                                                    \
      return pyz_fail(e_ == hipErrorOutOfMemory ? PYZ_E_OOM : PYZ_E_HIP, "%s failed: %s (%s:%d)", \
                      #call, hipGetErrorString(e_), __FILE__, __LINE__);                     \
  } while (0)

#define PYZ_LAUNCH_CHECK()                                                                    \
  do {                                                                                        \
    hipError_t e_ = hipGetLastError();                                                        \
    if (e_ != hipSuccess)                                                                     \
      return pyz_fail(PYZ_E_HIP, "kernel launch failed: %s (%s:%d)", hipGetErrorString(e_),   \
                      __FILE__, __LINE__);                                                    \
  } while (0)

struct PyzProbe {
  std::vector<hipEvent_t> ev;
  std::vector<const char *> name;
  int n = 0, cap = 0;
  bool on = false;
};
inline PyzProbe &pyz_probe() {
  static thread_local PyzProbe p;
  return p;
}
#define PYZ_LAUNCH(kern, grid, block, lds, st, ...)                                                              \
  do {                                                                                                           \
    PyzProbe &pp_ = pyz_probe();                                                                                 \
    if (pp_.on && pp_.n < pp_.cap) {                                                                             \
      hipExtLaunchKernelGGL(kern, grid, block, lds, st, pp_.ev[2 * pp_.n], pp_.ev[2 * pp_.n + 1], 0, __VA_ARGS__); \
      pp_.name[pp_.n++] = #kern;                                                                                 \
    } else {                                                                                                     \
      hipLaunchKernelGGL(kern, grid, block, lds, st, __VA_ARGS__);                                               \
    }                                                                                                            \
  } while (0)

template <int N>
struct PyzGraphCache {
  hipGraph_t graph[N] = {};
  hipGraphExec_t exec[N] = {};
  int len[N] = {};
  unsigned long long sig[N] = {}, use[N] = {};
  unsigned long long clock = 0, key = 0;
  unsigned long long call_clock = 0;
  int captures = 0;

  void drop_slot(int c) {
    if (exec[c]) (void)hipGraphExecDestroy(exec[c]);
    if (graph[c]) (void)hipGraphDestroy(graph[c]);
    exec[c] = nullptr;
    graph[c] = nullptr;
    len[c] = 0;
  }
  void drop() {
    for (int c = 0; c < N; ++c) drop_slot(c);
  }
  void rekey(unsigned long long k) {
    if (key != k) {
      drop();
      key = k;
    }
  }
  void begin_call() {
    captures = 0;
    call_clock = clock;
  }
  template <class Steps>
  int launch(int n, unsigned long long s, int lo, int hi, hipStream_t st, Steps &&steps) {
    int ci = -1, free_slot = -1, lru = -1;
    for (int c = lo; c < hi; ++c) {
      if (!exec[c]) {
        if (free_slot < 0) free_slot = c;
        continue;
      }
      if (len[c] == n && sig[c] == s) ci = c;
      if (lru < 0 || use[c] < use[lru]) lru = c;
    }
    if (ci < 0) {
      ci = free_slot >= 0 ? free_slot : lru;
      if (exec[ci] && use[ci] > call_clock) PYZ_HIP(hipStreamSynchronize(st));
      drop_slot(ci);
      PYZ_HIP(hipStreamBeginCapture(st, hipStreamCaptureModeRelaxed));
      const int rc = steps();
      hipGraph_t gr = nullptr;
      const hipError_t ce = hipStreamEndCapture(st, &gr);
      if (rc || ce != hipSuccess) {
        if (gr) (void)hipGraphDestroy(gr);
        return rc ? rc : pyz_fail(PYZ_E_HIP, "hipStreamEndCapture failed: %s", hipGetErrorString(ce));
      }
      graph[ci] = gr;
      PYZ_HIP(hipGraphInstantiate(&exec[ci], gr, nullptr, nullptr, 0));
      len[ci] = n;
      sig[ci] = s;
      ++captures;
    }
    use[ci] = ++clock;
    PYZ_HIP(hipGraphLaunch(exec[ci], st));
    return PYZ_OK;
  }
};

#define PYZ_GRAPH_CHUNKS 8
struct pyz_mlp {
  int L = 0;
  int dims[PYZ_MAX_LAYERS + 1] = {0};
  int acts[PYZ_MAX_LAYERS] = {0};
  long long w_off[PYZ_MAX_LAYERS] = {0};
  int loss = 0;
  int max_batch = 0, max_p = 0;
  long long D = 0;
  size_t ws_bytes = 0;
  float *act[PYZ_MAX_LAYERS] = {nullptr};
  float *delta[PYZ_MAX_LAYERS] = {nullptr};
  float *xb = nullptr;
  float *grad = nullptr;
  float *grad2 = nullptr;
  float *qsave = nullptr;
  double *part = nullptr;
  int part_len = 0;
  int cur_nblk = 0;
  float *scal = nullptr;
  StepCtl *ctl = nullptr;
  StepCtl pend{};
  bool pend_on = false;
  int32_t *tab_bs = nullptr;
  float *tab_lr = nullptr;
  int tab_cap = 0;
  float *h_pinned = nullptr;
  PyzGraphCache<PYZ_GRAPH_CHUNKS> graphs;
  int run_graph_steps = 0, run_eager_steps = 0, run_graph_launches = 0;
  int *nonfinite = nullptr;
  int grad_owner = 0;
  int grad_rows = 0;
  bool km_valid = false;
  const float *km_all = nullptr;
  int km_total = 0, km_row0 = 0, km_local = 0;
  float km_gamma = 0.0f;
};
```

bayesian_inference_for_nn_amd/csrc/pyz_fused.h:

```cpp
#pragma once

#include <type_traits>

#include "pyz_common.h"
#include "pyz_gemm.h"
#include "pyz_kernels.h"

struct HeadArgs {
  const float *hin;
  long long hin_pstride;
  const float *theta;
  long long theta_pstride;
  long long w_off;
  const StepCtl *ctl;
  const int32_t *row_idx;
  const StepCtl *gate;
  const void *y;
  double *part;
  int lda;
  int K, N;
  int loss;
  int gather_hin;
  int gate_mod;
  int init_on;
// ... 383 lines not shown
        d2[c] = c < N ? sc * e * pyz_act_grad(o, act) : 0.0f;
        outv[c] = o;
      }
      lm = a / (float)N;
    }
#pragma unroll
    for (int c = 0; c < NP; ++c) {
      my_d = (l == c) ? d2[c] : my_d;
      my_o = (l == c) ? outv[c] : my_o;
    }
  }
  PYZ_STAMP(1, 3);
  if (l < N) {
    if (g.out_last) pyz_st(g.out_last + p * g.last_pstride + (long long)m * N + l, my_o, g.wt);
    if (g.delta_last) pyz_st(g.delta_last + p * g.last_pstride + (long long)m * N + l, my_d, g.wt);
  }
  if (l == 0) g.part[p * g.nblk + m] = (double)lm;
  PYZ_STAMP(1, 4);
  if (!g.delta_prev) return;
  float *op = g.delta_prev + p * g.prev_pstride + (long long)m * K;
  const int actp = g.act_prev;
#pragma unroll
  for (int t = 0; t < UT; ++t) {
    const int u = l + 64 * t;
    float a = 0.0f;
#pragma unroll
    for (int c = 0; c < NP; ++c) a = fmaf(d2[c], wv[t][c], a);
    if (u < K) pyz_st(op + u, a * pyz_act_grad(hv[t], actp), g.wt);
  }
  PYZ_STAMP(1, 5);
}

template <int UT, int NP, int RW = 1, bool HP = false>
__global__ void __launch_bounds__(256) k_head_rows(HeadArgs g) {
  PYZ_STAMP(1, 0);
  const int w = pyz_wave_id(), l = threadIdx.x & 63;
  asm volatile("; arguments in one trip" ::"s"(g.hin), "s"(g.hin_pstride), "s"(g.theta), "s"(g.theta_pstride), "s"(g.w_off),
               "s"(g.ctl), "s"(g.row_idx), "s"(g.gate), "s"(g.y), "s"(g.part), "s"(g.lda), "s"(g.K), "s"(g.N), "s"(g.loss),
               "s"(g.gather_hin), "s"(g.gate_mod), "s"(g.init_on), "s"(g.nblk), "s"(g.act_last), "s"(g.act_prev), "s"(g.vec),
               "s"(g.wt));
  if (g.gate && g.gate->n % g.gate_mod == 0) return;
  StepCtl ctl;
  if (g.init_on) {
    asm volatile("; the step scalars by value" ::: "memory");
    ctl = pyz_ctl_first(g.ctl, g.init, 1);
  } else {
    const PyzCtlHot c = pyz_ctl_arrived(pyz_ctl_request(g.ctl));
    ctl.batch = c.batch;
    ctl.row_off = c.row_off;
  }
  const int batch = ctl.batch, p = blockIdx.y;
  const int m0 = (blockIdx.x * 4 + w) * RW;
  if (m0 >= batch) {
    if (l < RW && m0 + l < g.nblk) g.part[p * g.nblk + m0 + l] = 0.0;
    return;
  }
  PyzHeadW<UT, NP> W;
  if (RW == 1) {
    pyz_head_row<UT, NP, false, HP>(g, batch, ctl.row_off, p, m0, l, W);
    return;
  }
  pyz_head_load_w<UT, NP>(g, p, l, W);
#pragma unroll 1
  for (int rr = 0; rr < RW; ++rr) {
    const int m = m0 + rr;
    if (m >= batch) {
      if (l == 0 && m < g.nblk) g.part[p * g.nblk + m] = 0.0;
      continue;
    }
    pyz_head_row<UT, NP, true>(g, batch, ctl.row_off, p, m, l, W);
  }
}

struct PrepArgs {
  const float *src;
  float *dst;
  const int32_t *row_idx;
  const int32_t *tab_bs;
  long long row_stride;
  int K, lda;
  int fwd_tiles, fwd_tiles_n;
};

__device__ __forceinline__ void pyz_copy_rows(const PrepArgs &g, const int32_t *idx, const int ra, const int rb) {
  const int K = g.K, nt = blockDim.x, t = threadIdx.x;
  if (ra >= rb) return;
  if ((K & 3) == 0 && (g.lda & 3) == 0 && ((reinterpret_cast<uintptr_t>(g.src) | reinterpret_cast<uintptr_t>(g.dst)) & 15) == 0) {
    const int K4 = K >> 2, total = (rb - ra) * K4;
    for (int e0 = t; e0 < total; e0 += 4 * nt) {
      float4 v[4];
#pragma unroll
      for (int u = 0; u < 4; ++u) {
        const int e = min(e0 + u * nt, total - 1), m = ra + e / K4, c = e % K4;
        v[u] = *reinterpret_cast<const float4 *>(g.src + (long long)idx[m] * g.lda + 4 * c);
      }
#pragma unroll
      for (int u = 0; u < 4; ++u) {
        const int e = e0 + u * nt;
        if (e < total) {
          float *d = g.dst + (long long)(ra + e / K4) * K + 4 * (e % K4);
          const f32x4 vv = {v[u].x, v[u].y, v[u].z, v[u].w};
          asm volatile("global_store_dwordx4 %0, %1, off sc1" ::"v"(d), "v"(vv) : "memory");
        }
      }
    }
    return;
  }
  const int total = (rb - ra) * K;
  for (int e = t; e < total; e += nt) {
    const int m = ra + e / K, c = e % K;
    g.dst[(long long)m * K + c] = g.src[(long long)idx[m] * g.lda + c];
  }
}

__device__ __forceinline__ void pyz_prep_rows(const PrepArgs &g, const int32_t *idx, const int nb, const int j, const int cnt,
                                              const int bid) {
  int ra, rb;
  if (cnt >= 8 && g.fwd_tiles >= 8) {
    const int x = bid & 7, q = g.fwd_tiles >> 3, r = g.fwd_tiles & 7;
    const int t0 = x < r ? x * (q + 1) : r * (q + 1) + (x - r) * q, t1 = t0 + (x < r ? q + 1 : q);
    const int b0 = (t0 + g.fwd_tiles_n - 1) / g.fwd_tiles_n, b1 = (t1 + g.fwd_tiles_n - 1) / g.fwd_tiles_n;
    const int r0 = min(32 * b0, nb), r1 = x == 7 ? nb : min(32 * b1, nb);
    const int id0 = bid - j;
    const int first = id0 + ((x - (id0 & 7)) & 7);
    const int mine = (bid - first) >> 3, all = (id0 + cnt - 1 - first) / 8 + 1;
    const int per = (r1 - r0 + all - 1) / all;
    ra = r0 + mine * per;
    rb = min(ra + per, r1);
  } else {
    const int per = (nb + cnt - 1) / cnt;
    ra = j * per;
    rb = min(ra + per, nb);
  }
  pyz_copy_rows(g, idx, ra, rb);
}

__global__ void k_prep_batch(PrepArgs g, const StepCtl *ctl) {
  pyz_prep_rows(g, g.row_idx + ctl->row_off, ctl->batch, (int)blockIdx.x, (int)gridDim.x, (int)blockIdx.x);
}

__global__ void k_run_start(StepCtl *ctl, InlineTabs t, int32_t *tab_bs, float *tab_lr, long long n, long long row_off,
                            int slot0, PrepArgs g) {
  if (blockIdx.x == 0) {
    const int e = threadIdx.x;
    if (e < t.n) {
      tab_bs[e] = t.bs[e];
      tab_lr[e] = t.lr[e];
    }
    if (e == 0) {
      ctl->batch = t.bs[0];
      ctl->lr = t.lr[0];
      ctl->n = n;
      ctl->row_off = row_off;
      ctl->i = 0;
      ctl->slot0 = slot0;
      ctl->n_run = t.n - 1;
    }
  }
  pyz_prep_rows(g, g.row_idx + row_off, t.bs[0], (int)blockIdx.x, (int)gridDim.x, (int)blockIdx.x);
}

__global__ void k_run_start_bc(StepCtl *ctl, InlineTabs t, InlineBc b, int32_t *tab_bs, float *tab_lr, float2 *tab_bc,
                               long long n, long long row_off, int slot0, PrepArgs g) {
  if (blockIdx.x == 0) {
    const int e = threadIdx.x;
    if (e < t.n) {
      tab_bs[e] = t.bs[e];
      tab_lr[e] = t.lr[e];
      tab_bc[e] = b.bc[e];
    }
    if (e == 0) {
      ctl->batch = t.bs[0];
      ctl->lr = t.lr[0];
      ctl->n = n;
      ctl->row_off = row_off;
      ctl->i = 0;
      ctl->slot0 = slot0;
      ctl->n_run = t.n - 1;
    }
  }
  pyz_prep_rows(g, g.row_idx + row_off, t.bs[0], (int)blockIdx.x, (int)gridDim.x, (int)blockIdx.x);
}

struct WgradLayer {
  const float *in;
  long long in_pstride;
  const float *delta;
  long long delta_pstride;
  long long w_off;
  int lda, K, N;
  int tile0;
  int gather;
};

#define PYZ_UPD_NONE 0
#define PYZ_UPD_SGD 1
#define PYZ_UPD_SGLD 2
#define PYZ_UPD_BBB 3
#define PYZ_UPD_SWAG 4

struct WgradArgs {
  int tiles;
  int L;
  int mode;
  int wt;
  const StepCtl *ctl;
  const int32_t *row_idx;
  float *theta, *mean, *sq_mean;
  const float *unit_noise;
  uint64_t seed;
  int tile0[PYZ_MAX_LAYERS];
  const double *part;
  int nblk;
  int loss_indexed;
  float *loss;
  StepCtl *next;
  const int32_t *tab_bs;
  const float *tab_lr;
  int *nonfinite;
  WgradLayer lay[PYZ_MAX_LAYERS];
  float *grad;
  long long grad_pstride;
  float *dev_row;
  int swag_update;
  int swag_freq, swag_k;
  float *dev_base;
  long long dev_stride;
  float alpha, prior_mean, prior_rho, bbb_lr;
  const float *pm_vec, *pr_vec;
  uint32_t bbb_step;
  int bbb_chained;
  const double *part_kl;
  int nblk_kl;
  float *cost;
  float *w_next;
  double *part_kl_next;
  long long row_stride;
  float *ploss;
  PrepArgs prep;
};

static_assert(offsetof(WgradArgs, lay) % 64 == 0 && sizeof(WgradLayer) == 64, "a layer's entry is one 64-byte line");
// ... 42 lines not shown
    o.th = mu - blr * (g_mu + g_w);
    o.mu = rho - blr * (zz * sig * g_w + g_rho);
    o.wr_mu = true;
  } else if (mode == PYZ_UPD_SGLD) {
#pragma clang fp contract(off)
    const float fn = (float)nstep, fn1 = fn + 1.0f;
    const float gn = __builtin_fmaf(lr, zz, gv);
    const float th = __builtin_fmaf(-lr, gn, th0);
    o.th = th;
    o.mu = (mu0 * fn + th) / fn1;
    o.sq = __builtin_fmaf(th, th, sq0 * fn) / fn1;
    o.wr_mu = o.wr_sq = true;
  }
  return o;
}

__device__ __forceinline__ void pyz_update_store(const WgradArgs &g, const int mode, const long long e, const int p,
                                                 const float gv, const PyzUpdOut &o) {
  if (mode == PYZ_UPD_NONE) {
    g.grad[p * g.grad_pstride + e] = gv;
    return;
  }
  pyz_st(g.theta + e, o.th, g.wt);
  if (o.wr_mu) pyz_st(g.mean + e, o.mu, g.wt);
  if (o.wr_sq) pyz_st(g.sq_mean + e, o.sq, g.wt);
  if (o.wr_dev) o.dev_row[e] = o.dev;
}

__device__ __forceinline__ void pyz_step_duties(const WgradArgs &g, const int l) {
  const int batch = g.ctl->batch;
  if (g.loss) {
    const double v = pyz_sum_partials(g.part, g.nblk);
    if (l == 0) {
      float *lo = g.loss + (g.loss_indexed ? g.ctl->slot0 + g.ctl->i : 0);
      lo[0] = (float)(v / (double)batch);
      pyz_note_loss(g.nonfinite, lo[0]);
      if (g.next) pyz_prepare_next(g.ctl, g.next, g.tab_bs, g.tab_lr, g.row_stride);
    }
  }
  if (g.mode == PYZ_UPD_BBB) {
    const double v = pyz_sum_partials(g.part, g.nblk), k = pyz_sum_partials(g.part_kl, g.nblk_kl);
    if (l == 0) {
      const float loss = (float)(v / (double)batch), kl = (float)k;
      float *co = g.cost + (g.bbb_chained ? 4 * (g.ctl->slot0 + g.ctl->i) : 0);
      co[0] = loss + g.alpha * kl;
      pyz_note_loss(g.nonfinite, co[0]);
      co[1] = loss;
      co[2] = kl;
      if (g.bbb_chained && g.next) pyz_prepare_next(g.ctl, g.next, g.tab_bs, g.tab_lr, g.row_stride);
    }
  }
}


template <class H>
__device__ __forceinline__ void pyz_wgrad_accumulate(f32x16 &acc, const float *abase, const int ic, const float *dbase,
                                                     const int n, const int lda, const int N, const int batch, int s,
                                                     const int se, const int h, const bool is_w, const bool is_b, H hook) {
  const float bconst = is_b ? 1.0f : 0.0f;
  const unsigned a_lane = ((unsigned)h * (unsigned)lda + (unsigned)ic) * 4u;
  const unsigned d_lane = ((unsigned)h * (unsigned)N + (unsigned)n) * 4u;
  const unsigned a_row2 = 8u * (unsigned)lda, d_row2 = 8u * (unsigned)N;
  const __amdgpu_buffer_rsrc_t ra =
      __builtin_amdgcn_make_buffer_rsrc(const_cast<float *>(abase), 0, (int)((unsigned)batch * (unsigned)lda * 4u), 0x00020000);
  const __amdgpu_buffer_rsrc_t rd =
      __builtin_amdgcn_make_buffer_rsrc(const_cast<float *>(dbase), 0, (int)((unsigned)batch * (unsigned)N * 4u), 0x00020000);
  const int full = batch >> 1;
  pyz_steps1_all(
      s, min(se, full), acc,
      [&](int st, float &a, float &d) {
        a = pyz_buf_load(ra, a_lane, (unsigned)PYZ_HOT(st, batch) * a_row2);
        d = pyz_buf_load(rd, d_lane, (unsigned)PYZ_HOT(st, batch) * d_row2);
      },
      [&](int, float &a, float &) { a = is_w ? a : bconst; }, hook);
  if (se > full) {
    const int b = batch - 1;
    float a = abase[(size_t)b * lda + ic], d = dbase[(size_t)b * N + n];
    a = h == 0 ? (is_w ? a : bconst) : 0.0f;
    d = h == 0 ? d : 0.0f;
    acc = pyz_mfma(a, d, acc);
  }
}

template <int S, bool PLAIN, int MODE>
__device__ __forceinline__ void pyz_wgrad_tile(const WgradArgs &g, float *red) {
  constexpr int EPT = 16 / S;
  const int w = pyz_wave_id(), l = threadIdx.x & 63;
  const int r = l & 31, h = l >> 5;
  const int tile = pyz_xcd_remap(blockIdx.x, g.tiles);
  int li = 0;
#pragma unroll
  for (int j = 1; j < PYZ_MAX_LAYERS; ++j) li += tile >= g.tile0[j] ? 1 : 0;
  li = __builtin_amdgcn_readfirstlane(li);
  const WgradLayer &ly = g.lay[li];
  const PyzCtlHot ctl_raw = pyz_ctl_request(g.ctl);
  asm volatile("; the layer in one trip" ::"s"(ly.in), "s"(ly.in_pstride), "s"(ly.delta), "s"(ly.delta_pstride), "s"(ly.w_off),
               "s"(ly.lda), "s"(ly.K), "s"(ly.N), "s"(ly.tile0), "s"(ly.gather));
  const PyzCtlHot ctl = pyz_ctl_arrived(ctl_raw);
  const int batch = ctl.batch;
  const int K = ly.K, N = ly.N;
  const int tiles_n = (N + 31) >> 5;
  const int t = tile - ly.tile0;
  const int i0 = (t / tiles_n) * 32, n0 = (t % tiles_n) * 32;
  const int p = blockIdx.y;
  const long long w_off = ly.w_off;
  constexpr int mode = PLAIN ? PYZ_UPD_NONE : MODE;
  const long long nstep = ctl.n;
  const float lr = ctl.lr;

  long long ee[EPT];
  bool ev[EPT];
  float th0[PLAIN ? 1 : EPT], mu0[PLAIN ? 1 : EPT], sq0[PLAIN ? 1 : EPT], zz[PLAIN ? 1 : EPT];
  float zg[PLAIN ? 1 : EPT];
  float zn[PLAIN ? 1 : EPT];
  const bool fuse_next = !PLAIN && mode == PYZ_UPD_BBB && g.w_next != nullptr;
  auto prefetch = [&]() {
#pragma unroll
    for (int q = 0; q < EPT; ++q) {
      int ro, co;
      if (S == 1) {
        ro = (q & 3) + 8 * (q >> 2) + 4 * h;
        co = r;
      } else {
        const int e = threadIdx.x + q * 64 * S;
        ro = e >> 5;
        co = e & 31;
      }
      const int ii = i0 + ro, nn = n0 + co;
      ev[q] = ii <= K && nn < N;
      ee[q] = w_off + (long long)min(ii, K) * N + min(nn, N - 1);
      if (PLAIN) continue;
      th0[q] = mu0[q] = sq0[q] = zz[q] = zg[q] = 0.0f;
      if (mode != PYZ_UPD_NONE) th0[q] = g.theta[ee[q]];
      if (mode == PYZ_UPD_SGLD || mode == PYZ_UPD_BBB || mode == PYZ_UPD_SWAG) {
        mu0[q] = g.mean[ee[q]];
        sq0[q] = g.sq_mean[ee[q]];
        if (g.unit_noise && mode != PYZ_UPD_SWAG) zz[q] = g.unit_noise[ee[q]];
      }
    }
    if (!PLAIN && (mode == PYZ_UPD_SGLD || mode == PYZ_UPD_BBB) && !g.unit_noise) {
#pragma unroll
      for (int q = 0; q < EPT; ++q) {
        zg[q] = mode == PYZ_UPD_SGLD ? pyz_normal1(g.seed, PYZ_STREAM_SGLD, (uint32_t)nstep, (uint64_t)ee[q])
                                     : pyz_normal1(g.seed, PYZ_STREAM_BBB, g.bbb_chained ? (uint32_t)nstep : g.bbb_step, (uint64_t)ee[q]);
      }
    }
    if (!PLAIN && fuse_next) {
#pragma unroll
      for (int q = 0; q < EPT; ++q) zn[q] = pyz_normal1(g.seed, PYZ_STREAM_BBB, (uint32_t)(nstep + 1), (uint64_t)ee[q]);
    }
  };

  const int i = i0 + r, n = min(n0 + r, N - 1);
  const int ic = min(i, K - 1);
  const bool is_w = i < K, is_b = i == K;
  const float *ap = ly.in + p * ly.in_pstride + ic;
  const float *dp = ly.delta + p * ly.delta_pstride + n;
  const int32_t *idx = (ly.gather && g.row_idx) ? g.row_idx + ctl.row_off : nullptr;
  f32x16 acc = {0};
  const int steps = (batch + 1) >> 1;
  int s = (steps * w) / S;
  const int se = (steps * (w + 1)) / S;
  PYZ_STAMP(2, 1);
  if (idx) {
    prefetch();
    for (int s0 = s; s0 < se; s0 += 32) {
      const int idxv = idx[min(2 * s0 + l, batch - 1)];
      const int lda = ly.lda;
      pyz_steps1_all(
          s0, min(s0 + 32, se), acc,
          [&](int st, float &a, float &d) {
            const int bc = PYZ_HOT(min(2 * st + h, batch - 1), batch);
            const long long row = PYZ_HOT(__shfl(idxv, 2 * (st - s0) + h, 64), batch);
            a = ap[row * lda];
            d = dp[(long long)bc * N];
          },
          [&](int st, float &a, float &d) {
            const bool vb = 2 * st + h < batch;
            a = vb ? (is_w ? a : (is_b ? 1.0f : 0.0f)) : 0.0f;
            d = vb ? d : 0.0f;
          });
    }
  } else {
    pyz_wgrad_accumulate(acc, ly.in + p * ly.in_pstride, ic, ly.delta + p * ly.delta_pstride, n, ly.lda, N, batch, s, se, h,
                         is_w, is_b, prefetch);
  }
  PYZ_STAMP(2, 2);
  float gv[EPT];
  if (S == 1) {
#pragma unroll
    for (int q = 0; q < EPT; ++q) gv[q] = acc[q];
  } else {
    float *my = red + w * 1024;
#pragma unroll
    for (int q = 0; q < 16; ++q) my[((q & 3) + 8 * (q >> 2) + 4 * h) * 32 + r] = acc[q];
    __syncthreads();
#pragma unroll
    for (int q = 0; q < EPT; ++q) {
      const int e = threadIdx.x + q * 64 * S;
      float v = red[e];
#pragma unroll
      for (int ww = 1; ww < S; ++ww) v += red[ww * 1024 + e];
      gv[q] = v;
    }
  }
  PYZ_STAMP(2, 4);
  double klp = 0.0;
  float sp_s = 1.0f, lsp_s = 0.0f;
  if (!PLAIN && fuse_next) {
    sp_s = pyz_softplus(g.prior_rho);
    lsp_s = logf(sp_s);
  }
#pragma unroll
  for (int q = 0; q < EPT; ++q) {
    if (!ev[q]) continue;
    if (PLAIN) {
      pyz_st(g.grad + p * g.grad_pstride + ee[q], gv[q], g.wt);
      continue;
    }
    const PyzUpdOut o = pyz_update_math(g, mode, ee[q], gv[q], th0[q], mu0[q], sq0[q],
                                        PLAIN ? 0.0f : (g.unit_noise ? zz[q] : zg[q]), lr, nstep);
    pyz_update_store(g, mode, ee[q], p, gv[q], o);
    if (fuse_next) {
      const long long e = ee[q];
      const float pmean = g.pm_vec ? g.pm_vec[e] : g.prior_mean;
      float sp = sp_s, lsp = lsp_s;
      if (g.pr_vec) {
        sp = pyz_softplus(g.pr_vec[e]);
        lsp = logf(sp);
      }
      const float mu = o.th, sg = pyz_softplus(o.mu);
      const float wn = zn[q] * sg + mu;
      pyz_st(g.w_next + e, wn, g.wt);
      const float a = (wn - mu) / sg, b = (wn - pmean) / sp;
      const float lq = -0.5f * a * a - logf(sg) - PYZ_LOG_SQRT_2PI;
      const float lp = -0.5f * b * b - lsp - PYZ_LOG_SQRT_2PI;
      klp += (double)lq - (double)lp;
    }
  }
  if (!PLAIN && fuse_next) {
    double tot = pyz_wave_sum(klp);
    if (S > 1) {
      double *sm = reinterpret_cast<double *>(red);
      __syncthreads();
      if (l == 0) sm[w] = tot;
      __syncthreads();
      tot = 0.0;
      if (threadIdx.x == 0)
        for (int ww = 0; ww < S; ++ww) tot += sm[ww];
    }
    if (threadIdx.x == 0) g.part_kl_next[blockIdx.x] = tot;
  }
  PYZ_STAMP(2, 3);
}

template <int S, bool PLAIN = false>
__global__ void __launch_bounds__(64 * S) k_wgrad_all(WgradArgs g) {
  extern __shared__ float red[];
  PYZ_STAMP(2, 0);
  const int w = pyz_wave_id(), l = threadIdx.x & 63;
  asm volatile("; arguments in one trip" ::"s"(g.tiles), "s"(g.mode), "s"(g.ctl), "s"(g.row_idx), "s"(g.tile0[1]),
               "s"(g.tile0[2]), "s"(g.tile0[3]), "s"(g.tile0[4]), "s"(g.tile0[5]), "s"(g.tile0[6]), "s"(g.tile0[7]),
               "s"(g.tile0[8]), "s"(g.tile0[9]), "s"(g.tile0[10]), "s"(g.tile0[11]), "s"(g.tile0[12]), "s"(g.tile0[13]),
               "s"(g.tile0[14]), "s"(g.tile0[15]));
  if (blockIdx.x >= (unsigned)g.tiles) {
    if (blockIdx.x == (unsigned)g.tiles && blockIdx.y == 0 && w == 0) pyz_step_duties(g, l);
    if (blockIdx.x == (unsigned)g.tiles && w == 0 && g.ploss) {
      const double tot = pyz_sum_partials(g.part + (long long)blockIdx.y * g.nblk, g.nblk);
      if (l == 0) {
        g.ploss[blockIdx.y] = (float)(tot / (double)g.ctl->batch);
        pyz_note_loss(g.nonfinite, g.ploss[blockIdx.y]);
      }
    }
    if (!PLAIN && blockIdx.x > (unsigned)g.tiles && blockIdx.y == 0 && g.prep.src) {
      const int i2 = g.ctl->i + 1;
      if (i2 < g.ctl->n_run)
        pyz_prep_rows(g.prep, g.prep.row_idx + g.ctl->row_off + g.prep.row_stride, g.prep.tab_bs[i2],
                      (int)blockIdx.x - g.tiles - 1, (int)gridDim.x - g.tiles - 1, (int)blockIdx.x);
      PYZ_STAMP(2, 3);
    }
    return;
  }
  if constexpr (PLAIN) {
    pyz_wgrad_tile<S, true, PYZ_UPD_NONE>(g, red);
  } else {
    switch (g.mode) {
      case PYZ_UPD_SGLD: pyz_wgrad_tile<S, false, PYZ_UPD_SGLD>(g, red); break;
      case PYZ_UPD_SGD: pyz_wgrad_tile<S, false, PYZ_UPD_SGD>(g, red); break;
      case PYZ_UPD_SWAG: pyz_wgrad_tile<S, false, PYZ_UPD_SWAG>(g, red); break;
      case PYZ_UPD_BBB: pyz_wgrad_tile<S, false, PYZ_UPD_BBB>(g, red); break;
      default: pyz_wgrad_tile<S, false, PYZ_UPD_NONE>(g, red); break;
    }
  }
}

template <class H>
__device__ __forceinline__ void pyz_wgrad_accumulate_sq(f32x16 &acc, f32x16 &acc2, const float fb, const float *abase,
                                                        const int ic, const float *dbase, const int n, const int lda,
                                                        const int N, const int batch, int s, const int se, const int h,
                                                        const bool is_w, const bool is_b, H hook) {
  const float bconst = is_b ? 1.0f : 0.0f;
  const unsigned a_lane = ((unsigned)h * (unsigned)lda + (unsigned)ic) * 4u;
  const unsigned d_lane = ((unsigned)h * (unsigned)N + (unsigned)n) * 4u;
  const unsigned a_row2 = 8u * (unsigned)lda, d_row2 = 8u * (unsigned)N;
  const __amdgpu_buffer_rsrc_t ra =
      __builtin_amdgcn_make_buffer_rsrc(const_cast<float *>(abase), 0, (int)((unsigned)batch * (unsigned)lda * 4u), 0x00020000);
  const __amdgpu_buffer_rsrc_t rd =
      __builtin_amdgcn_make_buffer_rsrc(const_cast<float *>(dbase), 0, (int)((unsigned)batch * (unsigned)N * 4u), 0x00020000);
  const int full = batch >> 1;
  pyz_steps1_all(
      s, min(se, full), acc,
      [&](int st, float &a, float &d) {
        a = pyz_buf_load(ra, a_lane, (unsigned)PYZ_HOT(st, batch) * a_row2);
        d = pyz_buf_load(rd, d_lane, (unsigned)PYZ_HOT(st, batch) * d_row2);
      },
      [&](int, float &a, float &d) {
        a = is_w ? a : bconst;
        const float gd = d * fb;
        acc2 = pyz_mfma(a * a, gd * gd, acc2);
      },
      hook);
  if (se > full) {
    const int b = batch - 1;
    float a = abase[(size_t)b * lda + ic], d = dbase[(size_t)b * N + n];
    a = h == 0 ? (is_w ? a : bconst) : 0.0f;
    d = h == 0 ? d : 0.0f;
    const float gd = d * fb;
    acc2 = pyz_mfma(a * a, gd * gd, acc2);
    acc = pyz_mfma(a, d, acc);
  }
}

struct AdamArgs {
  WgradArgs w;
  float *m, *v;
  AdamScal a;
};

struct RunChain {
  const float2 *tab_bc;
  int perturb;
  float lam, num_data;
};

__device__ __forceinline__ void pyz_run_duties(const WgradArgs &g, const int l, const int stride, const int off,
                                               const bool advance) {
  const double v = pyz_sum_partials(g.part, g.nblk);
  if (l == 0) {
    float *lo = g.loss + (long long)stride * (g.ctl->slot0 + g.ctl->i) + off;
    lo[0] = (float)(v / (double)g.ctl->batch);
    pyz_note_loss(g.nonfinite, lo[0]);
    if (advance) pyz_prepare_next(g.ctl, g.next, g.tab_bs, g.tab_lr, g.row_stride);
  }
}

__device__ __forceinline__ void pyz_run_prep(const WgradArgs &g) {
  if (blockIdx.x > (unsigned)g.tiles && g.prep.src) {
    const int i2 = g.ctl->i + 1;
    if (i2 < g.ctl->n_run)
      pyz_prep_rows(g.prep, g.prep.row_idx + g.ctl->row_off + g.prep.row_stride, g.prep.tab_bs[i2],
                    (int)blockIdx.x - g.tiles - 1, (int)gridDim.x - g.tiles - 1, (int)blockIdx.x);
  }
}

struct AdamRunArgs : AdamArgs {
  RunChain c;
};

template <int S, bool CHAIN = false>
__global__ void __launch_bounds__(64 * S) k_wgrad_adam(std::conditional_t<CHAIN, AdamRunArgs, AdamArgs> A) {
  extern __shared__ float red[];
  const WgradArgs &g = A.w;
  constexpr int EPT = 16 / S;
  const int w = pyz_wave_id(), l = threadIdx.x & 63;
  const int r = l & 31, h = l >> 5;
// ... 300 lines not shown
```

bayesian_inference_for_nn_amd/csrc/pyz_gemm.h:

```cpp
#pragma once

#include <cstdlib>

#include "pyz_common.h"

struct DenseArgs {
  const float *in;
  long long in_pstride;
  const float *theta;
  long long theta_pstride;
  long long w_off;
  int lda;
  int K, N;
  int vec;
  int rows_cap;
  int gate_mod;
  float *out;
  long long out_pstride;
  const StepCtl *ctl;
  const int32_t *row_idx;
  float *gather_out;
  const StepCtl *gate;
  int act;
  int wt;
// ... 107 lines not shown
__device__ __forceinline__ void pyz_pipe1(int s, const int se, f32x16 &acc, L load, F fix, H hook = H()) {
  if (s >= se) {
    hook();
    return;
  }
  float an[G], bn[G], a[G], b[G];
  const int last = se - 1;
#pragma unroll
  for (int u = 0; u < G; ++u) load(min(s + u, last), an[u], bn[u]);
  __builtin_amdgcn_sched_barrier(0);
  hook();
  __builtin_amdgcn_sched_barrier(0);
  for (;;) {
#pragma unroll
    for (int u = 0; u < G; ++u) {
      a[u] = an[u];
      b[u] = bn[u];
    }
    const int sn = s + G;
    if (sn < se) {
#pragma unroll
      for (int u = 0; u < G; ++u) load(min(sn + u, last), an[u], bn[u]);
    }
    __builtin_amdgcn_sched_barrier(0);
#pragma unroll
    for (int u = 0; u < G; ++u)
      if (s + u < se) {
        fix(s + u, a[u], b[u]);
        acc = pyz_mfma(a[u], b[u], acc);
      }
    __builtin_amdgcn_sched_barrier(0);
    s = sn;
    if (s >= se) break;
  }
}

#define PYZ_MFMA4(A, B)              \
  acc = pyz_mfma((A).x, (B).x, acc); \
  acc = pyz_mfma((A).y, (B).y, acc); \
  acc = pyz_mfma((A).z, (B).z, acc); \
  acc = pyz_mfma((A).w, (B).w, acc);

struct PyzNoUse4 {
  __device__ __forceinline__ void operator()(int, const float4 &) const {}
};

template <int G, class L, class U, class H = PyzNoHook>
__device__ __forceinline__ void pyz_pipe4(int c, const int ce, f32x16 &acc, L load, U use, H hook = H()) {
  if (c >= ce) {
    hook();
    return;
  }
  float4 an[G], bn[G], a[G], b[G];
  const int last = ce - 1;
#pragma unroll
  for (int u = 0; u < G; ++u) load(min(c + u, last), an[u], bn[u]);
  __builtin_amdgcn_sched_barrier(0);
  hook();
  __builtin_amdgcn_sched_barrier(0);
  for (;;) {
#pragma unroll
    for (int u = 0; u < G; ++u) {
      a[u] = an[u];
      b[u] = bn[u];
    }
    const int cn = c + G;
    if (cn < ce) {
#pragma unroll
      for (int u = 0; u < G; ++u) load(min(cn + u, last), an[u], bn[u]);
    }
    __builtin_amdgcn_sched_barrier(0);
#pragma unroll
    for (int u = 0; u < G; ++u)
      if (c + u < ce) {
        use(c + u, a[u]);
        PYZ_MFMA4(a[u], b[u])
      }
    __builtin_amdgcn_sched_barrier(0);
    c = cn;
    if (c >= ce) break;
  }
}

template <class L, class U, class H = PyzNoHook>
__device__ __forceinline__ void pyz_steps4_all(int c, const int ce, f32x16 &acc, L load, U use, H hook = H()) {
  pyz_pipe4<2>(c, ce, acc, load, use, hook);
}
template <class L, class F, class H = PyzNoHook>
__device__ __forceinline__ void pyz_steps1_all(int s, const int se, f32x16 &acc, L load, F fix, H hook = H()) {
  pyz_pipe1<8>(s, se, acc, load, fix, hook);
}

__device__ __forceinline__ float pyz_buf_load(const __amdgpu_buffer_rsrc_t rsrc, const unsigned voff, const unsigned soff) {
  return __builtin_bit_cast(float, __builtin_amdgcn_raw_buffer_load_b32(rsrc, (int)voff, (int)soff, 0));
}

template <class H = PyzNoHook>
__device__ __forceinline__ void pyz_fwd_accumulate(f32x16 &acc, const float *ap, const float *wl, const int n, const int K,
                                                   const int N, const int vec, const int w, const int S, const int h,
                                                   float *gp = nullptr, const int copy_mod = 1, const int copy_rem = 0,
                                                   H hook = H()) {
  const __amdgpu_buffer_rsrc_t rw =
      __builtin_amdgcn_make_buffer_rsrc(const_cast<float *>(wl), 0, (int)((unsigned)(K + 1) * (unsigned)N * 4u), 0x00020000);
  const unsigned n4 = 4u * (unsigned)n, N4 = 4u * (unsigned)N;
  const float bias = pyz_buf_load(rw, n4, (unsigned)K * N4);
  const int c8 = vec ? (K >> 3) : 0;
  const unsigned v0 = (4u * h) * N4 + n4, v1 = v0 + N4, v2 = v1 + N4, v3 = v2 + N4;
  pyz_steps4_all(
      0, (c8 - w + S - 1) / S, acc,
      [&](int u, float4 &a4, float4 &b4) {
        const int c = PYZ_HOT(w + S * u, K);
        a4 = *reinterpret_cast<const float4 *>(ap + 8 * c + 4 * h);
        const unsigned so = 8u * (unsigned)c * N4;
        b4 = make_float4(pyz_buf_load(rw, v0, so), pyz_buf_load(rw, v1, so), pyz_buf_load(rw, v2, so), pyz_buf_load(rw, v3, so));
      },
      [&](int u, const float4 &a4) {
        const int c = w + S * u;
        if (gp && c % copy_mod == copy_rem) {
#ifdef PYZ_COPY_NT
          typedef float pyz_f4 __attribute__((ext_vector_type(4)));
          pyz_f4 v = {a4.x, a4.y, a4.z, a4.w};
          __builtin_nontemporal_store(v, reinterpret_cast<pyz_f4 *>(gp + 8 * c + 4 * h));
#else
          *reinterpret_cast<float4 *>(gp + 8 * c + 4 * h) = a4;
#endif
        }
      },
      hook);
  const int t0 = 8 * c8, steps = (K - t0 + 1) >> 1;
  const unsigned vt = (unsigned)h * N4 + n4;
  pyz_steps1_all(
      0, (steps - w + S - 1) / S, acc,
      [&](int u, float &a, float &b) {
        const int kb = t0 + 2 * (w + S * u);
        const int kk = kb + h;
        a = ap[kk < K ? kk : 0];
        b = pyz_buf_load(rw, vt, (unsigned)kb * N4);
      },
      [&](int u, float &a, float &b) {
        const int kk = t0 + 2 * (w + S * u) + h;
        const bool vk = kk < K;
        if (gp && vk && copy_rem == 0) gp[kk] = a;
        a = vk ? a : 0.0f;
        b = vk ? b : 0.0f;
      });
  if (w == 0) {
    acc = pyz_mfma(h == 0 ? 1.0f : 0.0f, h == 0 ? bias : 0.0f, acc);
  }
}

__global__ void k_dense_fwd(DenseArgs g) {
  extern __shared__ float red[];
  PYZ_STAMP(0, 0);
  const int S = blockDim.x >> 6, w = pyz_wave_id(), l = threadIdx.x & 63;
  const int r = l & 31, h = l >> 5;
  const int tiles_n = (g.N + 31) >> 5;
  asm volatile("; arguments in one trip" ::"s"(g.in), "s"(g.in_pstride), "s"(g.theta), "s"(g.theta_pstride), "s"(g.w_off),
               "s"(g.lda), "s"(g.K), "s"(g.N), "s"(g.vec), "s"(g.rows_cap), "s"(g.gate_mod), "s"(g.out), "s"(g.out_pstride),
               "s"(g.ctl), "s"(g.row_idx), "s"(g.gather_out), "s"(g.gate), "s"(g.act), "s"(g.wt), "s"((int)gridDim.x),
               "s"((int)blockDim.x));
  if (g.gate && g.gate->n % g.gate_mod == 0) return;
  const int tile = pyz_xcd_remap(blockIdx.x, gridDim.x);
  const int m0 = (tile / tiles_n) * 32, n0 = (tile % tiles_n) * 32;
  int cap = g.rows_cap;
  long long row_off = 0;
  if (cap <= 0) {
    asm volatile("; the step scalars are needed here" ::: "memory");
    const StepCtl ctl = pyz_ctl_first(g.ctl, g.init, g.init_on);
    cap = __builtin_amdgcn_readfirstlane(ctl.batch);
    row_off = ctl.row_off;
  }
  if (m0 >= cap) return;
  const int p = blockIdx.y;
  const int K = g.K, N = g.N;
  const int m = min(m0 + r, cap - 1), n = min(n0 + r, N - 1);
  long long row = m;
  if (g.row_idx) row = g.row_idx[row_off + m];
  const float *ap = g.in + p * g.in_pstride + row * g.lda;
  const float *wl = g.theta + p * g.theta_pstride + g.w_off;
  f32x16 acc = {0};
  PYZ_STAMP(0, 1);
  float *gp = (g.gather_out && p == 0) ? g.gather_out + (long long)m * K : nullptr;
  int batch = 0;
  const int32_t *ctl_batch = &g.ctl->batch;
  pyz_fwd_accumulate(acc, ap, wl, n, K, N, g.vec, w, S, h, gp, tiles_n, tile % tiles_n,
                     [&]() { batch = __hip_atomic_load(ctl_batch, __ATOMIC_RELAXED, __HIP_MEMORY_SCOPE_AGENT); });
  batch = g.rows_cap > 0 ? __builtin_amdgcn_readfirstlane(batch) : cap;
  PYZ_STAMP(0, 2);
  float *op = g.out + p * g.out_pstride;
  const int act = g.act, wt = g.wt;
  pyz_tile_epilogue(acc, red, [&](int ro, int co, float v) {
    const int mm = m0 + ro, nn = n0 + co;
    if (mm < batch && nn < N) pyz_st(op + (long long)mm * N + nn, pyz_act(v, act), wt);
  });
  PYZ_STAMP(0, 3);
}

template <int NT>
__global__ void __launch_bounds__(256) k_dense_fwd_lds(DenseArgs g) {
  constexpr int BN = 32 * NT, BM = 128, BK = 16;
  constexpr int AS = BM + 32;
  constexpr int BS = (BN % 64 == 0) ? BN + 32 : BN;
  constexpr int BJ = NT;
  __shared__ __attribute__((aligned(16))) float As[2][BK][AS];
  __shared__ __attribute__((aligned(16))) float Bs[2][BK][BS];
  const int t = threadIdx.x, w = pyz_wave_id(), l = t & 63, r = l & 31, h = l >> 5;
  const StepCtl ctl = pyz_ctl_first(g.ctl, g.init, g.init_on);
  const int batch = ctl.batch;
  const int K = g.K, N = g.N;
  const int tiles_n = (N + BN - 1) / BN;
  const int tile = pyz_xcd_remap(blockIdx.x, gridDim.x);
  const int m0 = (tile / tiles_n) * BM, n0 = (tile % tiles_n) * BN;
  if (m0 >= batch) return;
  const int p = blockIdx.y;
  const int ra = t >> 1, ka = 8 * (t & 1);
  const int ma = min(m0 + ra, batch - 1);
  long long rowa = ma;
  if (g.row_idx) rowa = g.row_idx[ctl.row_off + ma];
  const float *ap = g.in + p * g.in_pstride + rowa * g.lda + ka;
  const float *wl = g.theta + p * g.theta_pstride + g.w_off;
  float *gp = (g.gather_out && p == 0 && n0 == 0 && m0 + ra < batch) ? g.gather_out + (long long)ma * K + ka : nullptr;
  float4 va[2];
  float2 vb[BJ];
  auto fetch = [&](const int k0) {
#pragma unroll
    for (int j = 0; j < 2; ++j) {
      const int k = k0 + ka + 4 * j;
      va[j] = k < K ? *reinterpret_cast<const float4 *>(ap + k0 + 4 * j) : make_float4(0.f, 0.f, 0.f, 0.f);
    }
#pragma unroll
    for (int j = 0; j < BJ; ++j) {
      const int idx = t + 256 * j, kr = idx / (BN / 2), c2 = idx % (BN / 2);
      const int k = k0 + kr, n = n0 + 2 * c2;
      vb[j] = (k < K && n < N) ? *reinterpret_cast<const float2 *>(wl + (long long)k * N + n) : make_float2(0.f, 0.f);
    }
  };
  auto stage = [&](const int buf, const int k0) {
#pragma unroll
    for (int j = 0; j < 2; ++j) {
      const int kk = ka + 4 * j;
      As[buf][kk + 0][ra] = va[j].x;
      As[buf][kk + 1][ra] = va[j].y;
      As[buf][kk + 2][ra] = va[j].z;
      As[buf][kk + 3][ra] = va[j].w;
      if (gp && k0 + kk < K) *reinterpret_cast<float4 *>(gp + k0 + 4 * j) = va[j];
    }
#pragma unroll
    for (int j = 0; j < BJ; ++j) {
      const int idx = t + 256 * j, kr = idx / (BN / 2), c2 = idx % (BN / 2);
      *reinterpret_cast<float2 *>(&Bs[buf][kr][2 * c2]) = vb[j];
    }
  };
  f32x16 acc[NT];
#pragma unroll
  for (int nt = 0; nt < NT; ++nt) acc[nt] = f32x16{0};
  const int ns = (K + BK - 1) / BK;
  PYZ_STAMP(0, 0);
  fetch(0);
  stage(0, 0);
  __syncthreads();
  PYZ_STAMP(0, 1);
  for (int s = 0; s < ns; ++s) {
    const int buf = s & 1;
    if (s == 24) PYZ_STAMP(0, 2);
    if (s + 1 < ns) fetch((s + 1) * BK);
#pragma unroll
    for (int kp = 0; kp < BK / 2; ++kp) {
      const float a = As[buf][2 * kp + h][32 * w + r];
#pragma unroll
      for (int nt = 0; nt < NT; ++nt) acc[nt] = pyz_mfma(a, Bs[buf][2 * kp + h][32 * nt + r], acc[nt]);
    }
    if (s == 24) PYZ_STAMP(0, 3);
// ... 192 lines not shown
  f32x16 acc = {0}, acc2 = {0};
  const int steps = (batch + 1) >> 1;
  int s = (steps * w) / S;
  const int se = (steps * (w + 1)) / S;
  if (idx) {
    pyz_wgrad_steps<16, true, true>(s, se, acc, ap, dp, idx, g.lda, N, batch, h, r, is_w, is_b, &acc2, fb);
    pyz_wgrad_steps<4, true, true>(s, se, acc, ap, dp, idx, g.lda, N, batch, h, r, is_w, is_b, &acc2, fb);
    pyz_wgrad_steps<1, true, true>(s, se, acc, ap, dp, idx, g.lda, N, batch, h, r, is_w, is_b, &acc2, fb);
  } else {
    pyz_wgrad_steps<16, false, true>(s, se, acc, ap, dp, idx, g.lda, N, batch, h, r, is_w, is_b, &acc2, fb);
    pyz_wgrad_steps<4, false, true>(s, se, acc, ap, dp, idx, g.lda, N, batch, h, r, is_w, is_b, &acc2, fb);
    pyz_wgrad_steps<1, false, true>(s, se, acc, ap, dp, idx, g.lda, N, batch, h, r, is_w, is_b, &acc2, fb);
  }
  float *op = g.out + g.w_off, *op2 = out2 + g.w_off;
  pyz_tile_epilogue(acc, red, [&](int ro, int co, float v) {
    const int ii = i0 + ro, nn = n0 + co;
    if (ii <= K && nn < N) op[(long long)ii * N + nn] = v;
  });
  __syncthreads();
  pyz_tile_epilogue(acc2, red, [&](int ro, int co, float v) {
    const int ii = i0 + ro, nn = n0 + co;
    if (ii <= K && nn < N) op2[(long long)ii * N + nn] = v / fb;
  });
}

static inline int pyz_env_int(const char *name, int dflt) {
  const char *v = getenv(name);
  return v && *v ? atoi(v) : dflt;
}

static inline int pyz_cu_count() {
  static const int n = [] {
    int dev = 0, v = 0;
    if (hipGetDevice(&dev) != hipSuccess || hipDeviceGetAttribute(&v, hipDeviceAttributeMultiprocessorCount, dev) != hipSuccess || v <= 0)
      v = 256;
    return v;
  }();
  return n;
}

static inline int pyz_wt_for(int P) {
  static const int on = pyz_env_int("PYZ_WT", 1);
  return (on == 2 || (on && P == 1)) ? 1 : 0;
}

static inline int pyz_pick_waves(long long tiles, long long mfma_steps) {
  static const int target = pyz_env_int("PYZ_WAVES_TARGET", 3072);
  static const int min_steps = pyz_env_int("PYZ_MIN_STEPS", 8);
  int S = 1;
  while (S < 16 && tiles * S < target && mfma_steps / (2 * S) >= min_steps) S *= 2;
  return S;
}

static inline unsigned pyz_pad8(long long n, int P) { return (unsigned)(P > 1 ? (n + 7) / 8 * 8 : n); }

static inline bool pyz_fwd_takes_lds(const DenseArgs &g, int grid_batch, int P, int S) {
  const int lds_on = pyz_env_int("PYZ_FWD_LDS", 1);
  const bool lds_ok = g.K % 4 == 0 && g.N % 2 == 0 && g.lda % 4 == 0 && g.w_off % 2 == 0 && (P == 1 || g.theta_pstride % 2 == 0) &&
                      (P == 1 || g.in_pstride % 4 == 0) && (reinterpret_cast<uintptr_t>(g.theta) & 7) == 0 &&
                      (reinterpret_cast<uintptr_t>(g.in) & 15) == 0 &&
                      (!g.gather_out || (reinterpret_cast<uintptr_t>(g.gather_out) & 15) == 0);
  const int lds_max_rows = pyz_env_int("PYZ_FWD_LDS_MAXROWS", 2048);
  const int NT = g.N <= 64 ? 2 : (g.N <= 128 ? 4 : 7);
  const long long wg128 = (long long)((grid_batch + 127) / 128) * ((g.N + 32 * NT - 1) / (32 * NT)) * P;
  return S == 1 && !g.gate && lds_on && lds_ok && g.N >= 48 && grid_batch >= 128 && (grid_batch <= lds_max_rows || P >= 8) &&
         wg128 >= pyz_env_int("PYZ_FWD_LDS_MINWG", 256);
}

static inline void pyz_launch_fwd(const DenseArgs &g, int grid_batch, int P, hipStream_t st) {
  const long long tiles = (long long)((grid_batch + 31) / 32) * ((g.N + 31) / 32);
  const int S = pyz_pick_waves(tiles * P, (g.K + 1) / 2 + 1);
  if (pyz_fwd_takes_lds(g, grid_batch, P, S)) {
    const int NT = g.N <= 64 ? 2 : (g.N <= 128 ? 4 : 7);
    const long long tl = (long long)((grid_batch + 127) / 128) * ((g.N + 32 * NT - 1) / (32 * NT));
    const dim3 grid(pyz_pad8(tl, P), P), block(256);
    if (NT == 2) PYZ_LAUNCH(k_dense_fwd_lds<2>, grid, block, 0, st, g);
    else if (NT == 4) PYZ_LAUNCH(k_dense_fwd_lds<4>, grid, block, 0, st, g);
    else PYZ_LAUNCH(k_dense_fwd_lds<7>, grid, block, 0, st, g);
    return;
  }
  PYZ_LAUNCH(k_dense_fwd, dim3(pyz_pad8(tiles, P), P), dim3(64 * S), S > 1 ? S * 4096 : 0, st, g);
}

static inline void pyz_launch_bwd_data(const DenseArgs &g, int grid_batch, int P, hipStream_t st) {
  const long long tiles = (long long)((grid_batch + 31) / 32) * ((g.K + 31) / 32);
  const int S = pyz_pick_waves(tiles * P, (g.N + 1) / 2);
  PYZ_LAUNCH(k_dense_bwd_data, dim3(pyz_pad8(tiles, P), P), dim3(64 * S), S > 1 ? S * 4096 : 0, st, g);
}

static inline void pyz_launch_bwd_weight(const DenseArgs &g, int grid_batch, int P, hipStream_t st) {
  const long long tiles = (long long)((g.K + 1 + 31) / 32) * ((g.N + 31) / 32);
  const int S = pyz_pick_waves(tiles * P, (grid_batch + 1) / 2);
  PYZ_LAUNCH(k_dense_bwd_weight, dim3((unsigned)tiles, P), dim3(64 * S), S > 1 ? S * 4096 : 0, st, g);
}

static inline void pyz_launch_bwd_weight_sq(const DenseArgs &g, float *out2, int grid_batch, hipStream_t st) {
  const long long tiles = (long long)((g.K + 1 + 31) / 32) * ((g.N + 31) / 32);
  const int S = pyz_pick_waves(tiles, (grid_batch + 1) / 2);
  PYZ_LAUNCH(k_dense_bwd_weight_sq, dim3((unsigned)tiles), dim3(64 * S), S > 1 ? S * 4096 : 0, st, g, out2);
}
```

bayesian_inference_for_nn_amd/engine.py:

```python

from __future__ import annotations

import ctypes as C
from dataclasses import dataclass
from typing import Optional, Sequence, Tuple

import numpy as np
import torch

from . import _lib
from ._lib import ACT, LOSS, SWEEP, check, ptr

SVGD_GROUPS = 8


@dataclass(frozen=True)
class MLPSpec:
    dims: Tuple[int, ...]
    acts: Tuple[str, ...]
    loss: str = "scce"

    @property
    def n_layers(self):
        return len(self.acts)
# ... 344 lines not shown
        return P

    def sgld_lanes_step(self, theta, mean, sq_mean, x, y, lrs, n, seed, loss_out, seed_stride=0, batch=None, row_idx=None,
                        unit_noise=None):
        P = self._check_lanes(theta, mean, sq_mean, seed_stride)
        lr = self._lane_rates(lrs, (P,))
        batch = self._check_rows_step(P, x, y, loss_out, batch, row_idx, unit_noise)
        check(self.lib.pyz_sgld_lanes_step(self.h, ptr(theta), ptr(mean), ptr(sq_mean), P, ptr(x), ptr(y), ptr(row_idx), batch,
                                           lr.ctypes.data_as(C.POINTER(C.c_float)), int(n), int(seed), int(seed_stride),
                                           ptr(unit_noise), ptr(loss_out), _stream()))

    def sgld_lanes_run(self, theta, mean, sq_mean, x, y, row_idx, batch_sizes: Sequence[int], lrs, n0, seed, losses_out,
                       seed_stride=0, slot0=0):
        P = self._check_lanes(theta, mean, sq_mean, seed_stride)
        n_steps = len(batch_sizes)
        if n_steps < 1:
            raise ValueError("at least one step")
        lr = self._lane_rates(lrs, (n_steps, P))
        bs = self._check_rows_run(P, "n_lanes", x, y, row_idx, batch_sizes, losses_out, slot0)
        check(self.lib.pyz_sgld_lanes_run(self.h, ptr(theta), ptr(mean), ptr(sq_mean), P, ptr(x), ptr(y), ptr(row_idx), bs,
                                          lr.ctypes.data_as(C.POINTER(C.c_float)), n_steps, int(n0), int(slot0), int(seed),
                                          int(seed_stride), ptr(losses_out), _stream()))

    def lane_scores(self, weights, x, y, want_errors=True):
        _f32(weights, name="weights")
        if weights.dim() != 2 or weights.shape[1] != self.D or weights.shape[0] < 1:
            raise ValueError(f"weights must be (n_lanes, {self.D})")
        n = int(x.shape[0])
        self._check_xy(x, y, None, n)
        S = int(weights.shape[0])
        loss_sum = torch.empty((S,), dtype=torch.float64, device=self.device)
        errors = torch.empty((S,), dtype=torch.int64, device=self.device) if want_errors else None
        check(self.lib.pyz_lane_scores(self.h, ptr(weights), S, ptr(x), ptr(y), n, ptr(loss_sum), ptr(errors), _stream()))
        return loss_sum, errors

    def sgd_run(self, theta, x, y, row_idx, batch_sizes, lrs, losses_out, use_graph=True, slot0=0):
        n_steps = len(batch_sizes)
        assert len(lrs) == n_steps and n_steps > 0
        _f32(theta, (self.D,), "theta")
        self._check_xy(x, y, row_idx, 1)
        if slot0 < 0 or row_idx.numel() < (slot0 + n_steps) * self.max_batch or losses_out.numel() < slot0 + n_steps:
            raise ValueError("row_idx / losses_out too small")
        if any(int(b) < 1 or int(b) > self.max_batch for b in batch_sizes):
            raise ValueError("batch size outside the plan")
        bs = (C.c_int32 * n_steps)(*[int(b) for b in batch_sizes])
        lr = (C.c_float * n_steps)(*[float(v) for v in lrs])
        check(self.lib.pyz_sgd_run(self.h, ptr(theta), ptr(x), ptr(y), ptr(row_idx), bs, lr, n_steps, int(slot0),
                                   ptr(losses_out), 1 if use_graph else 0, _stream()))

    def swag_run(self, theta, mean, sq_mean, dev, frequency, x, y, row_idx, batch_sizes, lrs, n0, losses_out,
                 use_graph=True, slot0=0):
        n_steps = len(batch_sizes)
        assert len(lrs) == n_steps and n_steps > 0
        for t, nm in ((theta, "theta"), (mean, "mean"), (sq_mean, "sq_mean")):
            _f32(t, (self.D,), nm)
        _f32(dev, name="dev")
        assert dev.dim() == 2 and dev.shape[1] == self.D
        self._check_xy(x, y, row_idx, 1)
        if slot0 < 0 or row_idx.numel() < (slot0 + n_steps) * self.max_batch or losses_out.numel() < slot0 + n_steps:
            raise ValueError("row_idx / losses_out too small")
        if any(int(b) < 1 or int(b) > self.max_batch for b in batch_sizes):
            raise ValueError("batch size outside the plan")
        bs = (C.c_int32 * n_steps)(*[int(b) for b in batch_sizes])
        lr = (C.c_float * n_steps)(*[float(v) for v in lrs])
        check(self.lib.pyz_swag_run(self.h, ptr(theta), ptr(mean), ptr(sq_mean), ptr(dev), int(dev.shape[0]), int(frequency),
                                    ptr(x), ptr(y), ptr(row_idx), bs, lr, n_steps, int(n0), int(slot0), ptr(losses_out),
                                    1 if use_graph else 0, _stream()))

    def last_run_path(self):
        g, e, n = C.c_int32(), C.c_int32(), C.c_int32()
        check(self.lib.pyz_last_run_info(self.h, C.byref(g), C.byref(e), C.byref(n)))
        kind = "graph" if e.value == 0 else ("eager" if g.value == 0 else "mixed")
        return kind, g.value + e.value

    def last_run_graph_launches(self) -> int:
        n = C.c_int32()
        check(self.lib.pyz_last_run_info(self.h, None, None, C.byref(n)))
        return n.value

    def sgld_run_captures(self) -> int:
        n = C.c_int32()
        check(self.lib.pyz_sgld_run_info(self.h, C.byref(n)))
        return n.value

    def check_finite(self):
        check(self.lib.pyz_check_finite(self.h, _stream()))

    def bbb_step(self, mu, rho, w, x, y, lr, alpha, prior_mean, prior_rho, step, seed, cost_out, batch=None,
                 row_idx=None, eps=None, prior_mean_vec=None, prior_rho_vec=None):
        for t, nm in ((mu, "mu"), (rho, "rho"), (w, "w")):
            _f32(t, (self.D,), nm)
        for t, nm in ((eps, "eps"), (prior_mean_vec, "prior_mean_vec"), (prior_rho_vec, "prior_rho_vec")):
            if t is not None:
                _f32(t, (self.D,), nm)
        _f32(cost_out, name="cost_out")
        assert cost_out.numel() >= 3
        batch = int(batch if batch is not None else (row_idx.numel() if row_idx is not None else x.shape[0]))
        self._check_xy(x, y, row_idx, batch)
        check(self.lib.pyz_bbb_step(self.h, ptr(mu), ptr(rho), ptr(w), ptr(x), ptr(y), ptr(row_idx), batch, float(lr),
                                    float(alpha), float(prior_mean), float(prior_rho), ptr(prior_mean_vec),
                                    ptr(prior_rho_vec), int(step), int(seed), ptr(eps), ptr(cost_out), _stream()))

    def bbb_run(self, mu, rho, w, x, y, row_idx, batch_sizes, lrs, alpha, prior_mean, prior_rho, step0, seed, costs_out,
                use_graph=True, slot0=0, prior_mean_vec=None, prior_rho_vec=None, val_plan=None, val_x=None, val_y=None,
                val_losses_out=None):
        n_steps = len(batch_sizes)
        assert len(lrs) == n_steps and n_steps > 0
        for t, nm in ((mu, "mu"), (rho, "rho"), (w, "w")):
            _f32(t, (self.D,), nm)
        for t, nm in ((prior_mean_vec, "prior_mean_vec"), (prior_rho_vec, "prior_rho_vec")):
            if t is not None:
                _f32(t, (self.D,), nm)
        self._check_xy(x, y, row_idx, 1)
        _f32(costs_out, name="costs_out")
        if slot0 < 0 or row_idx.numel() < (slot0 + n_steps) * self.max_batch or costs_out.numel() < 4 * (slot0 + n_steps):
            raise ValueError("row_idx / costs_out too small")
        if any(int(b) < 1 or int(b) > self.max_batch for b in batch_sizes):
            raise ValueError("batch size outside the plan")
        n_val = 0
        if val_plan is not None:
            _f32(val_x, name="val_x")
            n_val = int(val_x.shape[0])
            if val_x.shape[1] != self.spec.dims[0] or n_val > val_plan.max_batch or val_plan.D != self.D:
                raise ValueError("validation split does not fit the validation plan")
            _f32(val_losses_out, name="val_losses_out")
            if val_losses_out.numel() < slot0 + n_steps:
                raise ValueError("val_losses_out too small")
        bs = (C.c_int32 * n_steps)(*[int(b) for b in batch_sizes])
        lr = (C.c_float * n_steps)(*[float(v) for v in lrs])
        check(self.lib.pyz_bbb_run(self.h, ptr(mu), ptr(rho), ptr(w), ptr(x), ptr(y), ptr(row_idx), bs, lr, n_steps, float(alpha),
                                   float(prior_mean), float(prior_rho), ptr(prior_mean_vec), ptr(prior_rho_vec), int(step0),
                                   int(slot0), int(seed), ptr(costs_out), val_plan.h if val_plan is not None else None,
                                   ptr(val_x), ptr(val_y), n_val, ptr(val_losses_out), 1 if use_graph else 0, _stream()))

    def _run_tables(self, row_idx, batch_sizes, lrs, losses_out, slot0, per_step=1):
        n_steps = len(batch_sizes)
        assert len(lrs) == n_steps and n_steps > 0
        _f32(losses_out, name="losses_out")
        if (slot0 < 0 or row_idx.numel() < (slot0 + n_steps) * self.max_batch
                or losses_out.numel() < per_step * (slot0 + n_steps)):
            raise ValueError("row_idx / losses_out too small")
        if any(int(b) < 1 or int(b) > self.max_batch for b in batch_sizes):
            raise ValueError("batch size outside the plan")
        return (C.c_int32 * n_steps)(*[int(b) for b in batch_sizes]), (C.c_float * n_steps)(*[float(v) for v in lrs])

    def adam_run(self, theta, m, v, x, y, row_idx, batch_sizes, lrs, epochs, beta_1, beta_2, losses_out, denom_eps=1e-3,
                 decay=0.0, perturb=False, lam=0.0, num_data=1.0, step0=0, seed=0, use_graph=True, slot0=0):
        for t, nm in ((theta, "theta"), (m, "m"), (v, "v")):
            _f32(t, (self.D,), nm)
        self._check_xy(x, y, row_idx, 1)
        bs, lr = self._run_tables(row_idx, batch_sizes, lrs, losses_out, slot0)
        n_steps = len(batch_sizes)
        if len(epochs) != n_steps:
            raise ValueError("one epoch count per step")
        ep = (C.c_int64 * n_steps)(*[int(e) for e in epochs])
        check(self.lib.pyz_adam_run(self.h, ptr(theta), ptr(m), ptr(v), ptr(x), ptr(y), ptr(row_idx), bs, lr, ep, n_steps,
                                    float(beta_1), float(beta_2), float(denom_eps), float(decay), 1 if perturb else 0,
                                    float(lam), float(num_data), int(step0), int(slot0), int(seed), ptr(losses_out),
                                    1 if use_graph else 0, _stream()))

    def bsam_run(self, theta, m, v, x, y, row_idx, batch_sizes, lrs, beta_1, beta_2, lam, rho, gam, num_data, step0, seed,
                 losses_out, use_graph=True, slot0=0):
        for t, nm in ((theta, "theta"), (m, "m"), (v, "v")):
            _f32(t, (self.D,), nm)
        self._check_xy(x, y, row_idx, 1)
        bs, lr = self._run_tables(row_idx, batch_sizes, lrs, losses_out, slot0, per_step=2)
# ... 620 lines not shown
```

include/pyz.h:

```cpp
#ifndef PYZ_H
#define PYZ_H

#include <stddef.h>
#include <stdint.h>

#ifdef __cplusplus
extern "C" {
#endif

#define PYZ_VERSION 302

#define PYZ_OK 0
#define PYZ_E_INVALID (-1)
#define PYZ_E_SHAPE (-2)
#define PYZ_E_HIP (-3)
#define PYZ_E_OOM (-4)
#define PYZ_E_NODEV (-5)
#define PYZ_E_NAN (-6)

#define PYZ_ACT_LINEAR 0
#define PYZ_ACT_RELU 1
#define PYZ_ACT_TANH 2
#define PYZ_ACT_SIGMOID 3
#define PYZ_ACT_SOFTMAX 4
// ... 30 lines not shown
                 const int32_t *d_row_idx, int batch, float lr, float *d_loss, void *stream);

int pyz_swag_step(pyz_mlp *mlp, float *d_theta, float *d_mean, float *d_sq_mean, float *d_dev_row,
                  const float *d_x, const void *d_y, const int32_t *d_row_idx, int batch, float lr,
                  int64_t n, int update_moments, float *d_loss, void *stream);

int pyz_adam_step(pyz_mlp *mlp, float *d_theta, float *d_m, float *d_v, const float *d_x, const void *d_y,
                  const int32_t *d_row_idx, int batch, float lr, double beta_1, double beta_2, int64_t epoch,
                  float denom_eps, float decay, float *d_loss, void *stream);

int pyz_vadam_perturb(pyz_mlp *mlp, float *d_theta, const float *d_v, float lam, float num_data, int64_t step,
                      uint64_t seed, const float *d_eps, void *stream);

int pyz_bsam_step(pyz_mlp *mlp, float *d_theta, float *d_m, float *d_v, const float *d_x, const void *d_y,
                  const int32_t *d_row_idx, int batch, float lr, double beta_1, double beta_2, float lam, float rho,
                  float gam, float num_data, int64_t step, uint64_t seed, const float *d_eps, float *d_loss,
                  void *stream);

int pyz_sgld_step(pyz_mlp *mlp, float *d_theta, float *d_mean, float *d_sq_mean, const float *d_x,
                  const void *d_y, const int32_t *d_row_idx, int batch, float lr, int64_t n,
                  uint64_t seed, const float *d_unit_noise, float *d_loss, void *stream);

int pyz_sgld_run(pyz_mlp *mlp, float *d_theta, float *d_mean, float *d_sq_mean, const float *d_x,
                 const void *d_y, const int32_t *d_row_idx, const int32_t *h_batch_sizes,
                 const float *h_lr, int n_steps, int64_t n0, int64_t slot0, uint64_t seed,
                 float *d_losses, int use_graph, void *stream);

int pyz_sgld_chains_step(pyz_mlp *mlp, float *d_theta, float *d_mean, float *d_sq_mean, int n_chains,
                         const float *d_x, const void *d_y, const int32_t *d_row_idx, int batch, float lr,
                         int64_t n, uint64_t seed, const float *d_unit_noise, float *d_loss ,
                         void *stream);

int pyz_sgld_chains_run(pyz_mlp *mlp, float *d_theta, float *d_mean, float *d_sq_mean, int n_chains,
                        const float *d_x, const void *d_y, const int32_t *d_row_idx,
                        const int32_t *h_batch_sizes, const float *h_lr, int n_steps, int64_t n0, int64_t slot0,
                        uint64_t seed, float *d_losses , int use_graph, void *stream);

#define PYZ_MAX_LANES 64
int pyz_sgld_lanes_step(pyz_mlp *mlp, float *d_theta, float *d_mean, float *d_sq_mean, int n_lanes, const float *d_x,
                        const void *d_y, const int32_t *d_row_idx, int batch, const float *h_lr ,
                        int64_t n, uint64_t seed, int seed_stride, const float *d_unit_noise,
                        float *d_loss , void *stream);

int pyz_sgld_lanes_run(pyz_mlp *mlp, float *d_theta, float *d_mean, float *d_sq_mean, int n_lanes, const float *d_x,
                       const void *d_y, const int32_t *d_row_idx, const int32_t *h_batch_sizes,
                       const float *h_lr , int n_steps, int64_t n0, int64_t slot0,
                       uint64_t seed, int seed_stride, float *d_losses , void *stream);

int pyz_lane_scores(pyz_mlp *mlp, const float *d_weights, int n_lanes, const float *d_x, const void *d_y, int n,
                    double *d_loss_sum , int64_t *d_errors , void *stream);

int pyz_sgd_run(pyz_mlp *mlp, float *d_theta, const float *d_x, const void *d_y,
                const int32_t *d_row_idx, const int32_t *h_batch_sizes, const float *h_lr,
                int n_steps, int64_t slot0, float *d_losses, int use_graph, void *stream);

int pyz_swag_run(pyz_mlp *mlp, float *d_theta, float *d_mean, float *d_sq_mean, float *d_dev, int k,
                 int frequency, const float *d_x, const void *d_y, const int32_t *d_row_idx,
                 const int32_t *h_batch_sizes, const float *h_lr, int n_steps, int64_t n0,
                 int64_t slot0, float *d_losses, int use_graph, void *stream);

int pyz_sgd_members_step(pyz_mlp *mlp, float *d_theta, float *d_mean, int n_members, const float *d_x,
                         const void *d_y, const int32_t *d_row_idx, int batch, float lr, int64_t n, int update_mean,
                         float *d_loss , void *stream);

int pyz_sgd_members_run(pyz_mlp *mlp, float *d_theta, float *d_mean, int n_members, int frequency, const float *d_x,
                        const void *d_y, const int32_t *d_row_idx, const int32_t *h_batch_sizes, const float *h_lr,
                        int n_steps, int64_t n0, int64_t slot0, float *d_losses ,
                        int use_graph, void *stream);

int pyz_swag_members_step(pyz_mlp *mlp, float *d_theta, float *d_mean, float *d_sq_mean, float *d_dev, int k,
                          int n_members, const float *d_x, const void *d_y, const int32_t *d_row_idx, int batch,
                          float lr, int64_t n, int update_moments, int dev_col, float *d_loss ,
                          void *stream);

int pyz_swag_members_run(pyz_mlp *mlp, float *d_theta, float *d_mean, float *d_sq_mean, float *d_dev, int k,
                         int frequency, int n_members, const float *d_x, const void *d_y, const int32_t *d_row_idx,
                         const int32_t *h_batch_sizes, const float *h_lr, int n_steps, int64_t n0, int64_t slot0,
                         float *d_losses , int use_graph, void *stream);

int pyz_last_run_info(const pyz_mlp *mlp, int32_t *h_graph_steps, int32_t *h_eager_steps,
                      int32_t *h_graph_launches);

int pyz_sgld_run_info(const pyz_mlp *mlp, int32_t *h_captures);

int pyz_check_finite(pyz_mlp *mlp, void *stream);

int pyz_probe_begin(int max_launches);
int pyz_probe_end(void *stream, float *h_us, char *h_names, int name_stride, int *h_n);

int pyz_bbb_step(pyz_mlp *mlp, float *d_mu, float *d_rho, float *d_w, const float *d_x,
                 const void *d_y, const int32_t *d_row_idx, int batch, float lr, float alpha,
                 float prior_mean, float prior_rho, const float *d_prior_mean_vec,
                 const float *d_prior_rho_vec, int64_t step, uint64_t seed,
                 const float *d_eps, float *d_cost, void *stream);

int pyz_bbb_run(pyz_mlp *mlp, float *d_mu, float *d_rho, float *d_w, const float *d_x, const void *d_y,
                const int32_t *d_row_idx, const int32_t *h_batch_sizes, const float *h_lr, int n_steps,
                float alpha, float prior_mean, float prior_rho, const float *d_prior_mean_vec,
                const float *d_prior_rho_vec, int64_t step0, int64_t slot0, uint64_t seed, float *d_costs,
                pyz_mlp *val_plan, const float *d_val_x, const void *d_val_y, int n_val,
                float *d_val_losses, int use_graph, void *stream);

int pyz_adam_run(pyz_mlp *mlp, float *d_theta, float *d_m, float *d_v, const float *d_x, const void *d_y,
                 const int32_t *d_row_idx, const int32_t *h_batch_sizes, const float *h_lr,
                 const int64_t *h_epochs, int n_steps, double beta_1, double beta_2, float denom_eps,
                 float decay, int perturb, float lam, float num_data, int64_t step0, int64_t slot0,
                 uint64_t seed, float *d_losses, int use_graph, void *stream);

int pyz_bsam_run(pyz_mlp *mlp, float *d_theta, float *d_m, float *d_v, const float *d_x, const void *d_y,
                 const int32_t *d_row_idx, const int32_t *h_batch_sizes, const float *h_lr, int n_steps,
                 double beta_1, double beta_2, float lam, float rho, float gam, float num_data,
                 int64_t step0, int64_t slot0, uint64_t seed, float *d_losses, int use_graph, void *stream);

int pyz_adam_run_info(const pyz_mlp *mlp, int32_t *h_captures);

int pyz_hmc_step(pyz_mlp *mlp, float *d_q, int n_chains, const float *d_x, const void *d_y,
                 int n_rows, int L, float epsilon, float m, float prior_mean, float prior_sigma,
                 const float *d_prior_mean_vec, const float *d_prior_sigma_vec,
                 int burning, const float *h_uniform, int64_t step, uint64_t seed,
                 const float *d_unit_p, float *d_stats, void *stream);

int pyz_hmc_run(pyz_mlp *mlp, float *d_q, int n_chains, const float *d_x, const void *d_y, int n_rows, int L,
                float epsilon, float m, float prior_mean, float prior_sigma, const float *d_prior_mean_vec,
                const float *d_prior_sigma_vec, const float *h_uniform, int n_steps, int n_burn, int64_t step0,
                int64_t slot0, uint64_t seed, float *d_stats_all, float *d_samples, int32_t *d_freq,
                int32_t *d_count, int cap, int32_t *d_fail, int use_graph, void *stream);
int pyz_hmc_run_info(const pyz_mlp *mlp, int32_t *h_captures);

int pyz_svgd_step(pyz_mlp *mlp, float *d_particles, int n_local, const float *d_all, int n_total,
                  int row0, float *d_adam_m, float *d_adam_v, const float *d_x, const void *d_y,
                  const int32_t *d_row_idx, int batch, float lr, float gamma, int64_t t, int sweep,
                  float *d_loss, void *stream);

int pyz_svgd_gradients(pyz_mlp *mlp, const float *d_particles, int n_local, const float *d_x, const void *d_y,
                       const int32_t *d_row_idx, int batch, void *stream);
int pyz_svgd_sweep(pyz_mlp *mlp, float *d_particles, int n_local, const float *d_all, int n_total, int row0,
                   float *d_adam_m, float *d_adam_v, float lr, float gamma, int64_t t, int sweep, float *d_loss,
                   void *stream);

int pyz_svgd_kernel_matrix(pyz_mlp *mlp, const float *d_all, int n_total, int row0, int n_local, float gamma,
                           void *stream);
int pyz_svgd_combine(pyz_mlp *mlp, float *d_particles, int n_local, const float *d_all, int n_total, int row0,
                     float *d_adam_m, float *d_adam_v, float lr, float gamma, int64_t t, float *d_loss,
                     void *stream);

#define PYZ_SVGD_GROUPS 8
int pyz_svgd_gram_groups(pyz_mlp *mlp, const float *d_all, int n_total, int g_lo, int g_hi, double *d_groups, void *stream);
int pyz_svgd_kernel_matrix_groups(pyz_mlp *mlp, const double *d_groups, const float *d_all, int n_total, int row0,
                                  int n_local, float gamma, void *stream);

int pyz_fsvi_check(int n_layers, const int32_t *h_dims, const int32_t *h_acts, int loss, int k, int batch, int batch_size);
int pyz_fsvi_step(pyz_mlp *mlp, float *d_mu, float *d_particles, int k, float *d_adam_m, float *d_adam_v, const float *d_x,
                  const float *d_y, const int32_t *d_row_idx, int batch, int batch_size, const float *d_lo,
                  const float *d_hi, float lr, int64_t t, uint64_t seed, const float *d_xm, const float *d_noise,
                  const float *d_eps, double *d_alpha, float *d_stein, float *d_grad, float *d_xp, float *d_f,
                  float *d_loss, void *stream);

int pyz_spd_solve_f64(double *d_a, double *d_rhs, int n, int n_systems, int *d_fail, void *stream);

int pyz_predict(pyz_mlp *mlp, const float *d_weights, int n_samples, const float *d_x, int n,
                float *d_samples, float *d_mean, void *stream);

int pyz_predict_moments(pyz_mlp *mlp, const float *d_weights, int n_samples, const float *d_x, int n,
                        float *d_mean, float *d_m2, void *stream);

int pyz_grid_rows(const float *d_basis, int d, float a0, float da, int n1, float b0, float db, int n2, int64_t row0,
// ... 96 lines not shown
```

Before: 42740 grad-steps/s.

## Prefetch next batch into MFMA fragment layouts for forward and weight-grad

When the next minibatch is gathered ahead of time, the prep step now writes two pre-swizzled images of it: one in the forward GEMM's A-fragment order and one transposed into the weight-gradient kernel's fragment order. New forward and wgrad kernel variants read those images with single contiguous float4 loads instead of strided row loads, and the forward kernel no longer copies the input. This is meant to cut the uncoalesced and extra-copy traffic on the 784-wide first layer. In exchange the staging buffer grows and the prep writes two images, and the path is on by default behind PYZ_BATCH_FRAG with a fallback when its conditions are not met.

```diff
diff --git a/bayesian_inference_for_nn_amd/_lib.py b/bayesian_inference_for_nn_amd/_lib.py
--- a/bayesian_inference_for_nn_amd/_lib.py
+++ b/bayesian_inference_for_nn_amd/_lib.py
@@ -68,6 +68,7 @@
                                        C.POINTER(_f), C.c_int, _i64, _i64, _p, C.c_int, _p]),
     "pyz_last_run_info": (C.c_int, [_p, C.POINTER(_i32), C.POINTER(_i32), C.POINTER(_i32)]),
     "pyz_sgld_run_info": (C.c_int, [_p, C.POINTER(_i32)]),
+    "pyz_run_batch_form": (C.c_int, [_p, C.POINTER(_i32)]),
     "pyz_check_finite": (C.c_int, [_p, _p]),
     "pyz_probe_begin": (C.c_int, [C.c_int]),
     "pyz_probe_end": (C.c_int, [_p, C.POINTER(_f), C.c_char_p, C.c_int, C.POINTER(C.c_int)]),
diff --git a/bayesian_inference_for_nn_amd/csrc/pyz_api.hip b/bayesian_inference_for_nn_amd/csrc/pyz_api.hip
--- a/bayesian_inference_for_nn_amd/csrc/pyz_api.hip
+++ b/bayesian_inference_for_nn_amd/csrc/pyz_api.hip
@@ -213,9 +213,9 @@
 void launch_forward(pyz_mlp *m, const float *theta, long long theta_ps, int P, const float *x,
                     const int32_t *row_idx, int grid_batch, const StepCtl *ctl, hipStream_t st,
                     float *gather_out = nullptr, int l_end = -1, const StepCtl *gate = nullptr, int gate_mod = 0,
-                    long long x_pstride = 0) {
+                    long long x_pstride = 0, int l_begin = 0) {
   if (l_end < 0) l_end = m->L;
-  for (int l = 0; l < l_end; ++l) {
+  for (int l = l_begin; l < l_end; ++l) {
     DenseArgs g = forward_args(m, l, theta, theta_ps, x, row_idx, ctl, gather_out);
     if (l == 0) g.in_pstride = x_pstride;
     g.wt = pyz_wt_for(P);
@@ -475,6 +475,22 @@
   }
 }
 
+void launch_wgrad_all_frag(pyz_mlp *m, const float *x, const int32_t *row_idx, int grid_batch, const StepCtl *ctl, WgradArgs &a,
+                           hipStream_t st, const float *wimg) {
+  const int tiles = wgrad_layers(m, 1, x, row_idx, ctl, a, wimg);
+  const int S = pyz_pick_waves(tiles, (grid_batch + 1) / 2);
+  dim3 grid((unsigned)tiles + 1);
+  if (a.prep.src) grid.x = (unsigned)(tiles + 1 + std::max(pyz_cu_count() - tiles - 1, 24));
+  a.lay[0].lda = 8 * ((m->max_batch + 7) / 8);
+  switch (S) {
+    case 1: PYZ_LAUNCH_AS(k_wgrad_all<1>, k_wgrad_all_frag<1>, grid, dim3(64), 0, st, a); break;
+    case 2: PYZ_LAUNCH_AS(k_wgrad_all<2>, k_wgrad_all_frag<2>, grid, dim3(128), 2 * 4096, st, a); break;
+    case 4: PYZ_LAUNCH_AS(k_wgrad_all<4>, k_wgrad_all_frag<4>, grid, dim3(256), 4 * 4096, st, a); break;
+    case 8: PYZ_LAUNCH_AS(k_wgrad_all<8>, k_wgrad_all_frag<8>, grid, dim3(512), 8 * 4096, st, a); break;
+    default: PYZ_LAUNCH_AS(k_wgrad_all<16>, k_wgrad_all_frag<16>, grid, dim3(1024), 16 * 4096, st, a); break;
+  }
+}
+
 void launch_wgrad_adam(pyz_mlp *m, const float *x, const int32_t *row_idx, int grid_batch, const StepCtl *ctl, AdamArgs &a,
                        hipStream_t st, const float *gathered) {
   const int tiles = wgrad_layers(m, 1, x, row_idx, ctl, a.w, gathered);
@@ -516,6 +532,23 @@
   return on == 2 || wgrad_tiles(m) + 24 <= pyz_cu_count();
 }
 
+inline size_t frag_fwd_floats(const pyz_mlp *m) { return (size_t)((m->max_batch + 31) / 32) * 32 * m->dims[0]; }
+inline size_t frag_slot_floats(const pyz_mlp *m) {
+  return frag_fwd_floats(m) + (size_t)((m->dims[0] + 31) / 32) * ((m->max_batch + 7) / 8) * 256;
+}
+inline float *frag_buf(pyz_mlp *m, int slot) { return m->xb + (size_t)slot * frag_slot_floats(m); }
+
+bool batch_frag(pyz_mlp *m, const float *theta, const float *x, const int32_t *row_idx, int grid_batch) {
+  if (!m->frag_on || !batch_ahead(m, row_idx)) return false;
+  const int K = m->dims[0];
+  if (K % 8 || !aligned16(x) || !aligned16(m->xb)) return false;
+  if (pyz_env_int("PYZ_FWD_KSPLIT", 0) >= 2) return false;
+  DenseArgs g = forward_args(m, 0, theta, m->D, frag_buf(m, 0), nullptr, nullptr, nullptr);
+  if (!g.vec || pyz_fwd_ring_variant(g, grid_batch, 1)) return false;
+  const long long tiles = (long long)((grid_batch + 31) / 32) * ((g.N + 31) / 32);
+  return !pyz_fwd_takes_lds(g, grid_batch, 1, pyz_pick_waves(tiles, (g.K + 1) / 2 + 1));
+}
+
 PrepArgs prep_args(pyz_mlp *m, const float *x, const int32_t *row_idx, int grid_batch, long long row_stride, int dst_slot) {
   PrepArgs p{};
   p.src = x;
@@ -529,6 +562,11 @@
   return p;
 }
 
+inline PrepArgs frag_prep(pyz_mlp *m, PrepArgs p, int dst_slot) {
+  p.dst = frag_buf(m, dst_slot);
+  return p;
+}
+
 int ksplit_for(pyz_mlp *m, const float *theta, long long theta_ps, int P, const float *xc, int grid_batch, const StepCtl *ctl) {
   const int ks_env = pyz_env_int("PYZ_FWD_KSPLIT", 0);
   if (ks_env < 2 || ks_env > 8 || m->L != 2 || P != 1) return 0;
@@ -544,8 +582,19 @@
 
 void launch_loss_backward(pyz_mlp *m, const float *theta, long long theta_ps, int P, const float *x, const void *y,
                           const int32_t *row_idx, int grid_batch, const StepCtl *ctl, bool want_grad, WgradArgs &upd,
-                          hipStream_t st, int ahead_slot = -1, AdamArgs *adam = nullptr) {
+                          hipStream_t st, int ahead_slot = -1, AdamArgs *adam = nullptr, bool frag = false) {
   if (can_fuse(m)) {
+    if (ahead_slot >= 0 && frag) {
+      DenseArgs g = forward_args(m, 0, theta, theta_ps, frag_buf(m, ahead_slot), nullptr, ctl, nullptr);
+      g.wt = pyz_wt_for(P);
+      g.rows_cap = std::min(grid_batch, m->max_batch);
+      pyz_launch_fwd_frag(g, grid_batch, st);
+      launch_forward(m, theta, theta_ps, P, nullptr, nullptr, grid_batch, ctl, st, nullptr, m->L - 1, nullptr, 0, 0, 1);
+      launch_head(m, theta, theta_ps, P, x, y, row_idx, grid_batch, ctl, want_grad, st);
+      launch_bwd_data_hidden(m, theta, theta_ps, P, grid_batch, ctl, st);
+      launch_wgrad_all_frag(m, x, row_idx, grid_batch, ctl, upd, st, frag_buf(m, ahead_slot) + frag_fwd_floats(m));
+      return;
+    }
     if (ahead_slot >= 0) {
       const float *xc = batch_buf(m, ahead_slot);
       const int ks = ksplit_for(m, theta, theta_ps, P, xc, grid_batch, ctl);
@@ -963,7 +1012,9 @@
     m->ws_bytes += 2 * bytes;
   }
   {
-    const size_t bytes = 2 * sizeof(float) * (size_t)max_batch * m->dims[0] + 64;
+    m->frag_on = pyz_env_int("PYZ_BATCH_FRAG", 1) != 0 && m->dims[0] % 8 == 0;
+    size_t bytes = 2 * sizeof(float) * (size_t)max_batch * m->dims[0] + 64;
+    if (m->frag_on) bytes = std::max(bytes, 2 * sizeof(float) * frag_slot_floats(m) + 64);
     if (hipMalloc((void **)&m->xb, bytes) != hipSuccess) return fail(pyz_fail(PYZ_E_OOM, "workspace allocation of %zu bytes failed", bytes));
     m->ws_bytes += bytes;
   }
@@ -1463,6 +1514,9 @@
 static int upload_run_tables(pyz_mlp *m, const int32_t *h_batch_sizes, const float *h_lr, int n_steps, int64_t n0, int64_t slot0,
                              const RunBc *bc, const float *d_x, const int32_t *d_row_idx, int ahead_batch, hipStream_t st) {
   Extra &x = full(m)->x;
+  const bool frag = m->frag_next && ahead_batch;
+  m->frag_next = false;
+  m->run_batch_form = ahead_batch ? (frag ? 2 : 1) : 0;
   int rc;
   const size_t n_tab = (size_t)n_steps + 1;
   if ((rc = ensure_run_tables(m, n_tab, bc ? 16 : 8, st))) return rc;
@@ -1488,7 +1542,8 @@
     for (int s = 0; bc && s <= n_steps; ++s) ibc.bc[s] = bc->of(std::min(s, n_steps - 1));
     if (ahead_batch) {
       const PrepArgs pa = prep_args(m, d_x, d_row_idx, ahead_batch, row_stride, 0);
-      if (bc) PYZ_LAUNCH(k_run_start_bc, dim3(256), dim3(256), 0, st, m->ctl, tabs, ibc, m->tab_bs, m->tab_lr, x.tab_bc, (long long)n0, slot0 * row_stride, (int)slot0, pa);
+      if (frag) PYZ_LAUNCH_AS(k_run_start, k_run_start_frag, dim3(256), dim3(256), 0, st, m->ctl, tabs, m->tab_bs, m->tab_lr, (long long)n0, slot0 * row_stride, (int)slot0, frag_prep(m, pa, 0));
+      else if (bc) PYZ_LAUNCH(k_run_start_bc, dim3(256), dim3(256), 0, st, m->ctl, tabs, ibc, m->tab_bs, m->tab_lr, x.tab_bc, (long long)n0, slot0 * row_stride, (int)slot0, pa);
       else PYZ_LAUNCH(k_run_start, dim3(256), dim3(256), 0, st, m->ctl, tabs, m->tab_bs, m->tab_lr, (long long)n0, slot0 * row_stride, (int)slot0, pa);
     } else {
       if (bc) PYZ_LAUNCH(k_set_ctl_tabs_bc, dim3(1), dim3(64), 0, st, m->ctl, tabs, ibc, m->tab_bs, m->tab_lr, x.tab_bc, (long long)n0, slot0 * row_stride, (int)slot0);
@@ -1512,6 +1567,10 @@
   if (bc) PYZ_HIP(hipMemcpyAsync(x.tab_bc, hc, sizeof(float2) * n_tab, hipMemcpyHostToDevice, st));
   PYZ_HIP(hipEventRecord(x.tab_ev[slot], st));
   if ((rc = set_ctl(m, 0, h_batch_sizes[0], h_lr[0], n0, slot0 * row_stride, 0, st, (int)slot0, n_steps))) return rc;
+  if (frag) {
+    PYZ_LAUNCH_AS(k_prep_batch, k_prep_batch_frag, dim3(256), dim3(256), 0, st, frag_prep(m, prep_args(m, d_x, d_row_idx, ahead_batch, row_stride, 0), 0), m->ctl);
+    return PYZ_OK;
+  }
   if (ahead_batch)
     PYZ_LAUNCH(k_prep_batch, dim3(256), dim3(256), 0, st, prep_args(m, d_x, d_row_idx, ahead_batch, row_stride, 0), m->ctl);
   return PYZ_OK;
@@ -1522,6 +1581,7 @@
                              uint64_t seed, const float *unit_noise, float *loss, hipStream_t st, int mode = PYZ_UPD_SGLD,
                              const SwagChain *swag = nullptr, const BbbChain *bbb = nullptr, bool first = true) {
   const StepCtl *ctl = m->ctl + slot;
+  const bool frag = chained && m->run_batch_form == 2;
   if (bbb) {
     const int nblk_sample = cdiv(cdiv(m->D, 4), 256), tiles = wgrad_tiles(m);
     const bool fuse = bbb->w2 != nullptr;
@@ -1573,7 +1633,8 @@
     u.row_stride = row_stride;
     const bool ahead = chained && batch_ahead(m, row_idx);
     if (ahead) u.prep = prep_args(m, x, row_idx, grid_batch, row_stride, slot ^ 1);
-    launch_loss_backward(m, w_cur, m->D, 1, x, y, row_idx, grid_batch, ctl, true, u, st, ahead ? slot : -1);
+    if (ahead && frag) u.prep.dst = frag_buf(m, slot ^ 1);
+    launch_loss_backward(m, w_cur, m->D, 1, x, y, row_idx, grid_batch, ctl, true, u, st, ahead ? slot : -1, nullptr, ahead && frag);
     if (bbb->val) {
       pyz_mlp *v = bbb->val;
       launch_forward(v, w_cur, v->D, 1, bbb->val_x, nullptr, bbb->n_val, v->ctl, st, nullptr, v->L - 1, ctl, 10);
@@ -1604,7 +1665,8 @@
     u.row_stride = row_stride;
     const bool ahead = chained && batch_ahead(m, row_idx);
     if (ahead) u.prep = prep_args(m, x, row_idx, grid_batch, row_stride, slot ^ 1);
-    launch_loss_backward(m, theta, m->D, 1, x, y, row_idx, grid_batch, ctl, true, u, st, ahead ? slot : -1);
+    if (ahead && frag) u.prep.dst = frag_buf(m, slot ^ 1);
+    launch_loss_backward(m, theta, m->D, 1, x, y, row_idx, grid_batch, ctl, true, u, st, ahead ? slot : -1, nullptr, ahead && frag);
     return;
   }
   WgradArgs u{};
@@ -1684,6 +1746,7 @@
     }
   }
   const long long row_stride = m->max_batch;
+  const bool frag = m->frag_next = batch_frag(m, d_theta, d_x, d_row_idx, bmax);
   if ((rc = upload_run_tables(m, h_batch_sizes, h_lr, n_steps, n0, slot0, nullptr, d_x, d_row_idx,
                               batch_ahead(m, d_row_idx) ? bmax : 0, st)))
     return rc;
@@ -1700,6 +1763,7 @@
     mix((unsigned long long)(uintptr_t)d_y); mix((unsigned long long)(uintptr_t)d_row_idx);
     mix((unsigned long long)(uintptr_t)d_losses); mix(seed); mix((unsigned long long)bmax);
     mix((unsigned long long)(uintptr_t)m->tab_bs); mix((unsigned long long)G); mix((unsigned long long)mode);
+    mix(frag ? 1ull : 0ull);
     if (swag) { mix((unsigned long long)(uintptr_t)swag->dev); mix((unsigned long long)swag->k); mix((unsigned long long)swag->freq); }
     if (bbb) {
       unsigned fb[3];
@@ -3655,6 +3719,12 @@
   return PYZ_OK;
 }
 
+int pyz_run_batch_form(const pyz_mlp *m, int32_t *h_form) {
+  if (!m) return pyz_fail(PYZ_E_INVALID, "null plan");
+  if (h_form) *h_form = m->run_batch_form;
+  return PYZ_OK;
+}
+
 int pyz_sgld_run_info(const pyz_mlp *m, int32_t *h_captures) {
   if (!m) return pyz_fail(PYZ_E_INVALID, "null plan");
   if (h_captures) *h_captures = m->graphs.captures;
diff --git a/bayesian_inference_for_nn_amd/csrc/pyz_common.h b/bayesian_inference_for_nn_amd/csrc/pyz_common.h
--- a/bayesian_inference_for_nn_amd/csrc/pyz_common.h
+++ b/bayesian_inference_for_nn_amd/csrc/pyz_common.h
@@ -159,6 +159,17 @@
     if (pp_.on && pp_.n < pp_.cap) {                                                                             \
       hipExtLaunchKernelGGL(kern, grid, block, lds, st, pp_.ev[2 * pp_.n], pp_.ev[2 * pp_.n + 1], 0, __VA_ARGS__); \
       pp_.name[pp_.n++] = #kern;                                                                                 \
+    } else {                                                                                                     \
+      hipLaunchKernelGGL(kern, grid, block, lds, st, __VA_ARGS__);                                               \
+    }                                                                                                            \
+  } while (0)
+
+#define PYZ_LAUNCH_AS(as, kern, grid, block, lds, st, ...)                                                       \
+  do {                                                                                                           \
+    PyzProbe &pp_ = pyz_probe();                                                                                 \
+    if (pp_.on && pp_.n < pp_.cap) {                                                                             \
+      hipExtLaunchKernelGGL(kern, grid, block, lds, st, pp_.ev[2 * pp_.n], pp_.ev[2 * pp_.n + 1], 0, __VA_ARGS__); \
+      pp_.name[pp_.n++] = #as;                                                                                   \
     } else {                                                                                                     \
       hipLaunchKernelGGL(kern, grid, block, lds, st, __VA_ARGS__);                                               \
     }                                                                                                            \
@@ -242,6 +253,9 @@
   float *act[PYZ_MAX_LAYERS] = {nullptr};
   float *delta[PYZ_MAX_LAYERS] = {nullptr};
   float *xb = nullptr;
+  bool frag_on = false;
+  int run_batch_form = 0;
+  bool frag_next = false;
   float *grad = nullptr;
   float *grad2 = nullptr;
   float *qsave = nullptr;
diff --git a/bayesian_inference_for_nn_amd/csrc/pyz_fused.h b/bayesian_inference_for_nn_amd/csrc/pyz_fused.h
--- a/bayesian_inference_for_nn_amd/csrc/pyz_fused.h
+++ b/bayesian_inference_for_nn_amd/csrc/pyz_fused.h
@@ -489,6 +489,55 @@
   int fwd_tiles, fwd_tiles_n;
 };
 
+__device__ __forceinline__ long long pyz_frag_fwd_floats(const int mb, const int K) { return (long long)((mb + 31) >> 5) * 32 * K; }
+
+__device__ __forceinline__ void pyz_copy_rows_frag(const PrepArgs &g, const int32_t *idx, const int ra, const int rb, const int nb) {
+  const int ga = (ra + 7) >> 3, gb = (rb + 7) >> 3;
+  if (ga >= gb) return;
+  const int K = g.K, K4 = K >> 2, C8 = K >> 3, KB = (K + 31) >> 5;
+  const int lane = threadIdx.x & 63, wv = threadIdx.x >> 6, nw = blockDim.x >> 6;
+  const int r8 = lane & 7, cl = lane >> 3, h = r8 & 1, qd = r8 >> 1;
+  const int mb = (int)g.row_stride, G = (mb + 7) >> 3;
+  float *fimg = g.dst, *wimg = g.dst + pyz_frag_fwd_floats(mb, K);
+  const int total = (gb - ga) * KB;
+  for (int u0 = wv; u0 < total; u0 += 4 * nw) {
+    float4 v[4];
+#pragma unroll
+    for (int u = 0; u < 4; ++u) {
+      const int unit = min(u0 + u * nw, total - 1), gi = ga + unit / KB, c4 = 8 * (unit % KB) + cl;
+      const int m = min(8 * gi + r8, nb - 1);
+      v[u] = *reinterpret_cast<const float4 *>(g.src + (long long)idx[m] * g.lda + 4 * min(c4, K4 - 1));
+    }
+#pragma unroll
+    for (int u = 0; u < 4; ++u) {
+      const int unit = u0 + u * nw;
+      if (unit >= total) break;
+      const int gi = ga + unit / KB, kb = unit % KB, c4 = 8 * kb + cl, m = 8 * gi + r8;
+      const bool vc = c4 < K4;
+      if (vc && m < nb) {
+        float *d = fimg + ((((long long)(m >> 5) * C8 + (c4 >> 1)) * 2 + (c4 & 1)) * 32 + (m & 31)) * 4;
+        const f32x4 vv = {v[u].x, v[u].y, v[u].z, v[u].w};
+        asm volatile("global_store_dwordx4 %0, %1, off sc1" ::"v"(d), "v"(vv) : "memory");
+      }
+      const float x0 = vc ? v[u].x : 0.0f, x1 = vc ? v[u].y : 0.0f, x2 = vc ? v[u].z : 0.0f, x3 = vc ? v[u].w : 0.0f;
+      float o0 = 0.0f, o1 = 0.0f, o2 = 0.0f, o3 = 0.0f;
+#pragma unroll
+      for (int k = 0; k < 4; ++k) {
+        const int js = (qd + k) & 3, qs = (qd - k) & 3;
+        const float send = js == 0 ? x0 : (js == 1 ? x1 : (js == 2 ? x2 : x3));
+        const float got = __shfl(send, (cl << 3) | (2 * qs + h), 64);
+        o0 = qs == 0 ? got : o0;
+        o1 = qs == 1 ? got : o1;
+        o2 = qs == 2 ? got : o2;
+        o3 = qs == 3 ? got : o3;
+      }
+      float *dw = wimg + ((((long long)kb * G + gi) * 2 + h) * 32 + 4 * cl + qd) * 4;
+      const f32x4 ww = {o0, o1, o2, o3};
+      asm volatile("global_store_dwordx4 %0, %1, off sc1" ::"v"(dw), "v"(ww) : "memory");
+    }
+  }
+}
+
 __device__ __forceinline__ void pyz_copy_rows(const PrepArgs &g, const int32_t *idx, const int ra, const int rb) {
   const int K = g.K, nt = blockDim.x, t = threadIdx.x;
   if (ra >= rb) return;
@@ -520,6 +569,7 @@
   }
 }
 
+template <bool FRAG = false>
 __device__ __forceinline__ void pyz_prep_rows(const PrepArgs &g, const int32_t *idx, const int nb, const int j, const int cnt,
                                               const int bid) {
   int ra, rb;
@@ -539,11 +589,15 @@
     ra = j * per;
     rb = min(ra + per, nb);
   }
-  pyz_copy_rows(g, idx, ra, rb);
+  if (FRAG) pyz_copy_rows_frag(g, idx, ra, rb, nb);
+  else pyz_copy_rows(g, idx, ra, rb);
 }
 
 __global__ void k_prep_batch(PrepArgs g, const StepCtl *ctl) {
   pyz_prep_rows(g, g.row_idx + ctl->row_off, ctl->batch, (int)blockIdx.x, (int)gridDim.x, (int)blockIdx.x);
+}
+__global__ void k_prep_batch_frag(PrepArgs g, const StepCtl *ctl) {
+  pyz_prep_rows<true>(g, g.row_idx + ctl->row_off, ctl->batch, (int)blockIdx.x, (int)gridDim.x, (int)blockIdx.x);
 }
 
 __global__ void k_run_start(StepCtl *ctl, InlineTabs t, int32_t *tab_bs, float *tab_lr, long long n, long long row_off,
@@ -565,6 +619,27 @@
     }
   }
   pyz_prep_rows(g, g.row_idx + row_off, t.bs[0], (int)blockIdx.x, (int)gridDim.x, (int)blockIdx.x);
+}
+
+__global__ void k_run_start_frag(StepCtl *ctl, InlineTabs t, int32_t *tab_bs, float *tab_lr, long long n, long long row_off,
+                                 int slot0, PrepArgs g) {
+  if (blockIdx.x == 0) {
+    const int e = threadIdx.x;
+    if (e < t.n) {
+      tab_bs[e] = t.bs[e];
+      tab_lr[e] = t.lr[e];
+    }
+    if (e == 0) {
+      ctl->batch = t.bs[0];
+      ctl->lr = t.lr[0];
+      ctl->n = n;
+      ctl->row_off = row_off;
+      ctl->i = 0;
+      ctl->slot0 = slot0;
+      ctl->n_run = t.n - 1;
+    }
+  }
+  pyz_prep_rows<true>(g, g.row_idx + row_off, t.bs[0], (int)blockIdx.x, (int)gridDim.x, (int)blockIdx.x);
 }
 
 __global__ void k_run_start_bc(StepCtl *ctl, InlineTabs t, InlineBc b, int32_t *tab_bs, float *tab_lr, float2 *tab_bc,
@@ -773,7 +848,46 @@
   }
 }
 
-template <int S, bool PLAIN, int MODE>
+template <class H>
+__device__ __forceinline__ void pyz_wgrad_accumulate_frag(f32x16 &acc, const float *ablk, const float *dbase, const int n,
+                                                          const int N, const int batch, const int s, const int se,
+                                                          const int h, const bool is_w, const bool is_b, H hook) {
+  const float bconst = is_b ? 1.0f : 0.0f;
+  const unsigned d_lane = ((unsigned)h * (unsigned)N + (unsigned)n) * 4u;
+  const unsigned d_row2 = 8u * (unsigned)N;
+  const __amdgpu_buffer_rsrc_t rd =
+      __builtin_amdgcn_make_buffer_rsrc(const_cast<float *>(dbase), 0, (int)((unsigned)batch * (unsigned)N * 4u), 0x00020000);
+  const int full = batch >> 1, sf = min(se, full);
+  const int cb = s >> 2, ce = s < sf ? (sf + 3) >> 2 : cb;
+  const int dlast = max(full - 1, 0);
+  pyz_pipe4x<2>(
+      cb, ce,
+      [&](int c, float4 &a4, float4 &d4) {
+        const int cc = PYZ_HOT(c, batch);
+        a4 = *reinterpret_cast<const float4 *>(ablk + 256 * cc);
+        const unsigned s0 = (unsigned)min(4 * cc, dlast), s1 = (unsigned)min(4 * cc + 1, dlast);
+        const unsigned s2 = (unsigned)min(4 * cc + 2, dlast), s3 = (unsigned)min(4 * cc + 3, dlast);
+        d4 = make_float4(pyz_buf_load(rd, d_lane, s0 * d_row2), pyz_buf_load(rd, d_lane, s1 * d_row2),
+                         pyz_buf_load(rd, d_lane, s2 * d_row2), pyz_buf_load(rd, d_lane, s3 * d_row2));
+      },
+      [&](int c, float4 &a4, float4 &d4) {
+        const int st = 4 * c;
+        if (st >= s && st < sf) acc = pyz_mfma(is_w ? a4.x : bconst, d4.x, acc);
+        if (st + 1 >= s && st + 1 < sf) acc = pyz_mfma(is_w ? a4.y : bconst, d4.y, acc);
+        if (st + 2 >= s && st + 2 < sf) acc = pyz_mfma(is_w ? a4.z : bconst, d4.z, acc);
+        if (st + 3 >= s && st + 3 < sf) acc = pyz_mfma(is_w ? a4.w : bconst, d4.w, acc);
+      },
+      hook);
+  if (se > full) {
+    const int b = batch - 1;
+    float a = ablk[256 * (full >> 2) + (full & 3)], d = dbase[(size_t)b * N + n];
+    a = h == 0 ? (is_w ? a : bconst) : 0.0f;
+    d = h == 0 ? d : 0.0f;
+    acc = pyz_mfma(a, d, acc);
+  }
+}
+
+template <int S, bool PLAIN, int MODE, bool FRAG = false>
 __device__ __forceinline__ void pyz_wgrad_tile(const WgradArgs &g, float *red) {
   constexpr int EPT = 16 / S;
   const int w = pyz_wave_id(), l = threadIdx.x & 63;
@@ -853,7 +967,11 @@
   int s = (steps * w) / S;
   const int se = (steps * (w + 1)) / S;
   PYZ_STAMP(2, 1);
-  if (idx) {
+  if (FRAG && li == 0) {
+    const int kb = min(i0, K - 1) >> 5, G = ly.lda >> 3;
+    pyz_wgrad_accumulate_frag(acc, ly.in + ((long long)kb * G * 64 + l) * 4, ly.delta + p * ly.delta_pstride, n, N, batch, s,
+                              se, h, is_w, is_b, prefetch);
+  } else if (idx) {
     prefetch();
     for (int s0 = s; s0 < se; s0 += 32) {
       const int idxv = idx[min(2 * s0 + l, batch - 1)];
@@ -982,6 +1100,35 @@
       case PYZ_UPD_BBB: pyz_wgrad_tile<S, false, PYZ_UPD_BBB>(g, red); break;
       default: pyz_wgrad_tile<S, false, PYZ_UPD_NONE>(g, red); break;
     }
+  }
+}
+
+template <int S>
+__global__ void __launch_bounds__(64 * S) k_wgrad_all_frag(WgradArgs g) {
+  extern __shared__ float red[];
+  PYZ_STAMP(2, 0);
+  const int w = pyz_wave_id(), l = threadIdx.x & 63;
+  asm volatile("; arguments in one trip" ::"s"(g.tiles), "s"(g.mode), "s"(g.ctl), "s"(g.row_idx), "s"(g.tile0[1]),
+               "s"(g.tile0[2]), "s"(g.tile0[3]), "s"(g.tile0[4]), "s"(g.tile0[5]), "s"(g.tile0[6]), "s"(g.tile0[7]),
+               "s"(g.tile0[8]), "s"(g.tile0[9]), "s"(g.tile0[10]), "s"(g.tile0[11]), "s"(g.tile0[12]), "s"(g.tile0[13]),
+               "s"(g.tile0[14]), "s"(g.tile0[15]));
+  if (blockIdx.x >= (unsigned)g.tiles) {
+    if (blockIdx.x == (unsigned)g.tiles && w == 0) pyz_step_duties(g, l);
+    if (blockIdx.x > (unsigned)g.tiles && g.prep.src) {
+      const int i2 = g.ctl->i + 1;
+      if (i2 < g.ctl->n_run)
+        pyz_prep_rows<true>(g.prep, g.prep.row_idx + g.ctl->row_off + g.prep.row_stride, g.prep.tab_bs[i2],
+                            (int)blockIdx.x - g.tiles - 1, (int)gridDim.x - g.tiles - 1, (int)blockIdx.x);
+      PYZ_STAMP(2, 3);
+    }
+    return;
+  }
+  switch (g.mode) {
+    case PYZ_UPD_SGLD: pyz_wgrad_tile<S, false, PYZ_UPD_SGLD, true>(g, red); break;
+    case PYZ_UPD_SGD: pyz_wgrad_tile<S, false, PYZ_UPD_SGD, true>(g, red); break;
+    case PYZ_UPD_SWAG: pyz_wgrad_tile<S, false, PYZ_UPD_SWAG, true>(g, red); break;
+    case PYZ_UPD_BBB: pyz_wgrad_tile<S, false, PYZ_UPD_BBB, true>(g, red); break;
+    default: __builtin_trap();
   }
 }
 
diff --git a/bayesian_inference_for_nn_amd/csrc/pyz_gemm.h b/bayesian_inference_for_nn_amd/csrc/pyz_gemm.h
--- a/bayesian_inference_for_nn_amd/csrc/pyz_gemm.h
+++ b/bayesian_inference_for_nn_amd/csrc/pyz_gemm.h
@@ -213,6 +213,40 @@
   }
 }
 
+template <int G, class L, class B, class H = PyzNoHook>
+__device__ __forceinline__ void pyz_pipe4x(int c, const int ce, L load, B body, H hook = H()) {
+  if (c >= ce) {
+    hook();
+    return;
+  }
+  float4 an[G], bn[G], a[G], b[G];
+  const int last = ce - 1;
+#pragma unroll
+  for (int u = 0; u < G; ++u) load(min(c + u, last), an[u], bn[u]);
+  __builtin_amdgcn_sched_barrier(0);
+  hook();
+  __builtin_amdgcn_sched_barrier(0);
+  for (;;) {
+#pragma unroll
+    for (int u = 0; u < G; ++u) {
+      a[u] = an[u];
+      b[u] = bn[u];
+    }
+    const int cn = c + G;
+    if (cn < ce) {
+#pragma unroll
+      for (int u = 0; u < G; ++u) load(min(cn + u, last), an[u], bn[u]);
+    }
+    __builtin_amdgcn_sched_barrier(0);
+#pragma unroll
+    for (int u = 0; u < G; ++u)
+      if (c + u < ce) body(c + u, a[u], b[u]);
+    __builtin_amdgcn_sched_barrier(0);
+    c = cn;
+    if (c >= ce) break;
+  }
+}
+
 template <class L, class U, class H = PyzNoHook>
 __device__ __forceinline__ void pyz_steps4_all(int c, const int ce, f32x16 &acc, L load, U use, H hook = H()) {
   pyz_pipe4<2>(c, ce, acc, load, use, hook);
@@ -226,7 +260,7 @@
   return __builtin_bit_cast(float, __builtin_amdgcn_raw_buffer_load_b32(rsrc, (int)voff, (int)soff, 0));
 }
 
-template <class H = PyzNoHook>
+template <bool FRAG = false, class H = PyzNoHook>
 __device__ __forceinline__ void pyz_fwd_accumulate(f32x16 &acc, const float *ap, const float *wl, const int n, const int K,
                                                    const int N, const int vec, const int w, const int S, const int h,
                                                    float *gp = nullptr, const int copy_mod = 1, const int copy_rem = 0,
@@ -241,13 +275,13 @@
       0, (c8 - w + S - 1) / S, acc,
       [&](int u, float4 &a4, float4 &b4) {
         const int c = PYZ_HOT(w + S * u, K);
-        a4 = *reinterpret_cast<const float4 *>(ap + 8 * c + 4 * h);
+        a4 = *reinterpret_cast<const float4 *>(FRAG ? ap + 256 * c : ap + 8 * c + 4 * h);
         const unsigned so = 8u * (unsigned)c * N4;
         b4 = make_float4(pyz_buf_load(rw, v0, so), pyz_buf_load(rw, v1, so), pyz_buf_load(rw, v2, so), pyz_buf_load(rw, v3, so));
       },
       [&](int u, const float4 &a4) {
         const int c = w + S * u;
-        if (gp && c % copy_mod == copy_rem) {
+        if (!FRAG && gp && c % copy_mod == copy_rem) {
 #ifdef PYZ_COPY_NT
           typedef float pyz_f4 __attribute__((ext_vector_type(4)));
           pyz_f4 v = {a4.x, a4.y, a4.z, a4.w};
@@ -258,9 +292,9 @@
         }
       },
       hook);
-  const int t0 = 8 * c8, steps = (K - t0 + 1) >> 1;
+  const int t0 = 8 * c8, steps = FRAG ? 0 : (K - t0 + 1) >> 1;
   const unsigned vt = (unsigned)h * N4 + n4;
-  pyz_steps1_all(
+  if (!FRAG) pyz_steps1_all(
       0, (steps - w + S - 1) / S, acc,
       [&](int u, float &a, float &b) {
         const int kb = t0 + 2 * (w + S * u);
@@ -319,6 +353,38 @@
   batch = g.rows_cap > 0 ? __builtin_amdgcn_readfirstlane(batch) : cap;
   PYZ_STAMP(0, 2);
   float *op = g.out + p * g.out_pstride;
+  const int act = g.act, wt = g.wt;
+  pyz_tile_epilogue(acc, red, [&](int ro, int co, float v) {
+    const int mm = m0 + ro, nn = n0 + co;
+    if (mm < batch && nn < N) pyz_st(op + (long long)mm * N + nn, pyz_act(v, act), wt);
+  });
+  PYZ_STAMP(0, 3);
+}
+
+__global__ void k_dense_fwd_frag(DenseArgs g) {
+  extern __shared__ float red[];
+  PYZ_STAMP(0, 0);
+  const int S = blockDim.x >> 6, w = pyz_wave_id(), l = threadIdx.x & 63;
+  const int r = l & 31, h = l >> 5;
+  const int tiles_n = (g.N + 31) >> 5;
+  asm volatile("; arguments in one trip" ::"s"(g.in), "s"(g.theta), "s"(g.w_off), "s"(g.K), "s"(g.N), "s"(g.vec), "s"(g.rows_cap),
+               "s"(g.out), "s"(g.ctl), "s"(g.act), "s"(g.wt), "s"((int)gridDim.x), "s"((int)blockDim.x));
+  const int tile = pyz_xcd_remap(blockIdx.x, gridDim.x);
+  const int m0 = (tile / tiles_n) * 32, n0 = (tile % tiles_n) * 32;
+  if (m0 >= g.rows_cap) return;
+  const int K = g.K, N = g.N;
+  const int n = min(n0 + r, N - 1);
+  const float *ap = g.in + ((long long)(m0 >> 5) * (K >> 3) * 64 + l) * 4;
+  const float *wl = g.theta + g.w_off;
+  f32x16 acc = {0};
+  PYZ_STAMP(0, 1);
+  int batch = 0;
+  const int32_t *ctl_batch = &g.ctl->batch;
+  pyz_fwd_accumulate<true>(acc, ap, wl, n, K, N, g.vec, w, S, h, nullptr, 1, 0,
+                           [&]() { batch = __hip_atomic_load(ctl_batch, __ATOMIC_RELAXED, __HIP_MEMORY_SCOPE_AGENT); });
+  batch = __builtin_amdgcn_readfirstlane(batch);
+  PYZ_STAMP(0, 2);
+  float *op = g.out;
   const int act = g.act, wt = g.wt;
   pyz_tile_epilogue(acc, red, [&](int ro, int co, float v) {
     const int mm = m0 + ro, nn = n0 + co;
@@ -677,6 +743,12 @@
   PYZ_LAUNCH(k_dense_fwd, dim3(pyz_pad8(tiles, P), P), dim3(64 * S), S > 1 ? S * 4096 : 0, st, g);
 }
 
+static inline void pyz_launch_fwd_frag(const DenseArgs &g, int grid_batch, hipStream_t st) {
+  const long long tiles = (long long)((grid_batch + 31) / 32) * ((g.N + 31) / 32);
+  const int S = pyz_pick_waves(tiles, (g.K + 1) / 2 + 1);
+  PYZ_LAUNCH_AS(k_dense_fwd, k_dense_fwd_frag, dim3((unsigned)tiles), dim3(64 * S), S > 1 ? S * 4096 : 0, st, g);
+}
+
 static inline void pyz_launch_bwd_data(const DenseArgs &g, int grid_batch, int P, hipStream_t st) {
   const long long tiles = (long long)((grid_batch + 31) / 32) * ((g.K + 31) / 32);
   const int S = pyz_pick_waves(tiles * P, (g.N + 1) / 2);
diff --git a/bayesian_inference_for_nn_amd/engine.py b/bayesian_inference_for_nn_amd/engine.py
--- a/bayesian_inference_for_nn_amd/engine.py
+++ b/bayesian_inference_for_nn_amd/engine.py
@@ -450,6 +450,11 @@
         n = C.c_int32()
         check(self.lib.pyz_sgld_run_info(self.h, C.byref(n)))
         return n.value
+
+    def run_batch_form(self) -> str:
+        n = C.c_int32()
+        check(self.lib.pyz_run_batch_form(self.h, C.byref(n)))
+        return ("gather", "rows", "images")[n.value]
 
     def check_finite(self):
         check(self.lib.pyz_check_finite(self.h, _stream()))
diff --git a/include/pyz.h b/include/pyz.h
--- a/include/pyz.h
+++ b/include/pyz.h
@@ -136,6 +136,8 @@
                       int32_t *h_graph_launches);
 
 int pyz_sgld_run_info(const pyz_mlp *mlp, int32_t *h_captures);
+
+int pyz_run_batch_form(const pyz_mlp *mlp, int32_t *h_form);
 
 int pyz_check_finite(pyz_mlp *mlp, void *stream);
 
```

New measurement: 44530 grad-steps/s, median of 6. +4.2%, better.
